# LuckyIYI/gsm-renderer

Measured on AMD Instinct MI355X. Metric: frames/sec @ N Gaussians × W×H (1/2/4/8 GPU); sort Gkeys/s; blend HBM GB/s, higher is better.
Workload: dtype fp16

## Files before the change

### gsm-renderer_amd/csrc/gsm_capi.hip

```cpp
#include <hip/hip_runtime.h>

#include <cstring>

#include "../../include/gsm_debug.h"
#include "../../include/gsm_multigpu.h"
#include "../../include/gsm_renderer.h"
#include "gsm_internal.h"
#include "gsm_frame_sort_check.h"
#include "gsm_renderer_impl.h"

namespace gsm {

class FrameSorter {
   public:
    static gsm_status create(uint32_t capacity, uint32_t maxTiles, int device, FrameSorter** out) {
        FrameSorter* f = new (std::nothrow) FrameSorter;
        if (!f) return GSM_ERR_FAILED_TO_ALLOCATE_BUFFER;
        gsm_status st = pick_device(device, &f->dev_);
        if (st == GSM_OK) {
            f->allocs_.setDevice(f->dev_.id);
            f->tuning_ = tuning_from_env(f->dev_.id);
            f->capacity_ = capacity;
            f->maxTiles_ = maxTiles;
            DeviceAllocations& M = f->allocs_;
// ... 358 lines not shown
}

gsm_status gsm_global_transform_from_pose(const float rotation[9], float scale, const float translation[3],
                                          gsm_global_transform_desc* out) {
    return gsm::transform_from_pose(rotation, scale, translation, out);
}

gsm_status gsm_global_transform(gsm_renderer* r, void* stream, const gsm_global_scene* scene,
                                const gsm_global_state* state, const uint32_t keep[8],
                                const gsm_global_transform_desc* desc) {
    if (!r || !r->impl) return GSM_ERR_INVALID_ARGUMENT;
    return r->impl->transform((hipStream_t)stream, scene, state, keep, desc);
}

gsm_status gsm_global_pick_owner(gsm_renderer* r, const uint32_t* items, uint32_t n, uint32_t* object,
                                 uint32_t* gaussian) {
    if (!r || !r->impl || (n > 0 && (!items || !object || !gaussian))) return GSM_ERR_INVALID_ARGUMENT;
    return r->impl->pickOwner(items, n, object, gaussian);
}

gsm_status gsm_global_project_partition(gsm_renderer* r, void* stream, const gsm_gaussian_input* input,
                                        const gsm_camera_params* camera, uint32_t width, uint32_t height,
                                        uint32_t first, uint32_t count, const uint32_t* slab_rows,
                                        uint32_t num_slabs, void* send, uint64_t send_capacity,
                                        uint32_t* send_counts) {
    if (!r || !r->impl || !input || !camera) return GSM_ERR_INVALID_ARGUMENT;
    return r->impl->projectPartition((hipStream_t)stream, *input, *camera, width, height, first, count,
                                     slab_rows, num_slabs, send, send_capacity, send_counts);
}

gsm_status gsm_global_render_records(gsm_renderer* r, void* stream, const void* records, uint32_t count,
                                     uint32_t width, uint32_t height, void* color, size_t color_pitch,
                                     void* depth, size_t depth_pitch) {
    if (!r || !r->impl) return GSM_ERR_INVALID_ARGUMENT;
    return r->impl->renderRecords((hipStream_t)stream, records, count, width, height, color, color_pitch,
                                  depth, depth_pitch);
}

gsm_status gsm_global_render_stereo_sbs(gsm_renderer* r, void* stream, const gsm_gaussian_input* input,
                                        const gsm_camera_params* left, const gsm_camera_params* right,
                                        uint32_t width_per_eye, uint32_t height, void* color, size_t color_pitch,
                                        void* depth, size_t depth_pitch) {
    if (!r || !r->impl || !input || !left || !right) return GSM_ERR_INVALID_ARGUMENT;
    if (!color) return GSM_ERR_MISSING_REQUIRED_BUFFER;
    gsm_status st = r->impl->renderFrame((hipStream_t)stream, *input, *left, width_per_eye, height,
                                         gsm::FrameTargets{color, color_pitch, depth, depth_pitch});
    if (st != GSM_OK) return st;
    char* rc = (char*)color + (size_t)width_per_eye * 8;
    char* rd = depth ? (char*)depth + (size_t)width_per_eye * 2 : nullptr;
    return r->impl->renderFrame((hipStream_t)stream, *input, *right, width_per_eye, height,
                                gsm::FrameTargets{rc, color_pitch, rd, depth_pitch});
}

gsm_status gsm_global_render_stereo(gsm_renderer* r, void*, const gsm_gaussian_input*,
                                    const gsm_camera_params*, const gsm_camera_params*, uint32_t,
                                    uint32_t, void*, size_t, void*, size_t) {
    if (!r) return GSM_ERR_INVALID_ARGUMENT;
    return GSM_ERR_UNSUPPORTED;
}

uint32_t gsm_global_debug_read_total_assignments(gsm_renderer* r) {
    if (!r || !r->impl) return 0;
    gsm_debug_counters c;
    if (r->impl->counters(&c) != GSM_OK) return 0;
    return c.total_assignments;
}

gsm_status gsm_global_last_gpu_time(gsm_renderer* r, double* seconds) {
    if (!r || !r->impl || !seconds) return GSM_ERR_INVALID_ARGUMENT;
    return r->impl->lastGpuTime(seconds);
}

gsm_status gsm_global_debug_counters(gsm_renderer* r, gsm_debug_counters* out) {
    if (!r || !r->impl || !out) return GSM_ERR_INVALID_ARGUMENT;
    return r->impl->counters(out);
}

gsm_status gsm_global_debug_blend_kernel(gsm_renderer* r, int* kind) {
    if (!r || !r->impl || !kind) return GSM_ERR_INVALID_ARGUMENT;
    *kind = r->impl->lastBlendKernel();
    return GSM_OK;
}

gsm_status gsm_global_debug_copy(gsm_renderer* r, int which, void* dst, size_t bytes, size_t* needed) {
    if (!r || !r->impl) return GSM_ERR_INVALID_ARGUMENT;
    return r->impl->debugCopy(which, dst, bytes, needed);
}

gsm_status gsm_global_set_profiling(gsm_renderer* r, int enable) {
    if (!r || !r->impl) return GSM_ERR_INVALID_ARGUMENT;
    return r->impl->setProfiling(enable);
}

gsm_status gsm_global_stage_times(gsm_renderer* r, float* ms, int n) {
    if (!r || !r->impl || !ms) return GSM_ERR_INVALID_ARGUMENT;
    return r->impl->stageTimes(ms, n);
}

gsm_status gsm_global_set_tile_rows(gsm_renderer* r, uint32_t b, uint32_t e) {
    if (!r || !r->impl) return GSM_ERR_INVALID_ARGUMENT;
    return r->impl->setTileRows(b, e);
}

size_t gsm_debug_sort_workspace_bytes(uint32_t capacity) { return gsm::sort_workspace_bytes(capacity); }

gsm_status gsm_debug_sort_plan_fits(uint32_t capacity, uint32_t key_bits, int wide, size_t hist_bytes) {
    if (key_bits == 0 || key_bits > 32) return GSM_ERR_INVALID_ARGUMENT;
    const gsm::SortSpace ws{(uint32_t*)(uintptr_t)16, hist_bytes, (uint32_t*)(uintptr_t)16, gsm::kSortTotalsWords};
    return gsm::sort_bits_plan_fits(capacity, key_bits, wide != 0, ws) ? GSM_OK : GSM_ERR_INVALID_ASSIGNMENT_CAPACITY;
}

gsm_status gsm_sort_pairs_u32(void* keys, void* values, uint32_t n, uint32_t key_bits, void* stream) {
    if ((!keys || !values) && n > 0) return GSM_ERR_INVALID_ARGUMENT;
    if (n == 0) return GSM_OK;
    if (key_bits == 0 || key_bits > 32) key_bits = 32;
    hipStream_t s = (hipStream_t)stream;
    uint32_t *k2 = nullptr, *v2 = nullptr, *hist = nullptr, *bins = nullptr, *np = nullptr;
    gsm_status st = GSM_OK;
    if (hipMalloc(&k2, (size_t)n * 4) != hipSuccess || hipMalloc(&v2, (size_t)n * 4) != hipSuccess ||
        hipMalloc(&hist, gsm::sort_workspace_bytes(n)) != hipSuccess || hipMalloc(&bins, 256 * 4) != hipSuccess ||
        hipMalloc(&np, 4) != hipSuccess) {
        st = GSM_ERR_FAILED_TO_ALLOCATE_BUFFER;
    }
    if (st == GSM_OK) {
        hipMemcpyAsync(np, &n, 4, hipMemcpyHostToDevice, s);
        hipMemsetAsync(hist, 0, gsm::sort_workspace_bytes(n), s);
        uint32_t* kb[2] = {(uint32_t*)keys, k2};
        uint32_t* vb[2] = {(uint32_t*)values, v2};
        const int digits = (int)((key_bits + 7) / 8);
        int dev = 0;
        hipGetDevice(&dev);
        const gsm::Tuning tn = gsm::tuning_from_env(dev);
        const gsm::SortSpace ws{hist, gsm::sort_workspace_bytes(n), bins, 256};
        int res = gsm::radix_sort_pairs(kb, vb, np, n, 0, digits, ws, s, tn.ballotRank, tn.sortScanless);
        if (res == gsm::kSortNoSpace) st = GSM_ERR_INVALID_ASSIGNMENT_CAPACITY;
        if (res == 1) {
            hipMemcpyAsync(keys, k2, (size_t)n * 4, hipMemcpyDeviceToDevice, s);
            hipMemcpyAsync(values, v2, (size_t)n * 4, hipMemcpyDeviceToDevice, s);
        }
        if (hipStreamSynchronize(s) != hipSuccess) st = GSM_ERR_RENDER_FAILED;
    }
    hipFree(k2);
    hipFree(v2);
    hipFree(hist);
    hipFree(bins);
    hipFree(np);
    return st;
}

gsm_status gsm_debug_frame_sort_create(uint32_t capacity, uint32_t max_tiles, int hip_device,
                                       gsm_debug_frame_sort** out) {
    const gsm_status st = gsm::frame_sort_create_check(capacity, max_tiles, out);
    if (st != GSM_OK) return st;
    return gsm_debug_frame_sort::create(out, capacity, max_tiles, hip_device);
}

void gsm_debug_frame_sort_destroy(gsm_debug_frame_sort* f) { gsm_debug_frame_sort::destroy(f); }

gsm_status gsm_debug_frame_sort_run(gsm_debug_frame_sort* f, void* stream, const gsm_debug_frame_sort_desc* desc,
                                    const void* keys, const void* values, uint32_t n, gsm_debug_frame_sort_out* out) {
    if (!f || !f->impl) return GSM_ERR_INVALID_ARGUMENT;
    return f->impl->run((hipStream_t)stream, desc, keys, values, n, out);
}

gsm_status gsm_debug_sort_rank_probe(int hip_device, int* lane_ordered) {
    if (!lane_ordered) return GSM_ERR_INVALID_ARGUMENT;
// ... 43 lines not shown
```

### gsm-renderer_amd/csrc/gsm_internal.h

```cpp
#pragma once
#include <hip/hip_runtime.h>
#include <cstdint>
#include <tuple>

#include "gsm_blend_plan.h"
#include "gsm_frame_plan.h"
#include "gsm_host.h"
#include "gsm_sort_plan.h"
#include "gsm_types.h"

namespace gsm {

struct ProjectArgs {
    CameraUniforms cam;
    TileBinningParams bin;
    uint32_t rowBegin, rowEnd, rowStride;
    uint32_t count;
    uint32_t maxAssignments;
    uint32_t keepRenderData;
    uint32_t schedUnits;
    uint32_t pairBucket;
    float limX, limY, focalX, focalY, maxEig, adjFar, adjDen;
};

struct ViewArgs {
    CameraUniforms cam;
    float limX, limY, focalX, focalY, maxEig, adjFar, adjDen;
    float pad;
};
static_assert(sizeof(ViewArgs) == 240, "ViewArgs: 15 16-B words");
constexpr uint32_t kViewChunk = 16;
struct ViewChunk {
    ViewArgs v[kViewChunk];
};
struct ViewBatch {
    uint32_t views = 0;
    uint32_t blocksPerView = 0;
    uint32_t tilesPerView = 0;
    const ViewArgs* args = nullptr;
};

struct BatchTarget {
    uint8_t* color;
    uint8_t* depth;
    size_t colorPitch, depthPitch;
    uint32_t tileBase, tilesX, tilesY, width, height;
    uint32_t vec;
    uint32_t pad[2];
};
static_assert(sizeof(BatchTarget) == 64, "BatchTarget: one 64-B line");
struct BatchViewArgs {
    CameraUniforms cam;
    float limX, limY, focalX, focalY, maxEig, adjFar, adjDen;
    uint32_t count;
    TileBinningParams bin;
    uint32_t blockBase;
    uint32_t ortho;
    const void* world;
    const void* harm;
    BatchTarget tg;
};
static_assert(sizeof(BatchViewArgs) == 368 && offsetof(BatchViewArgs, tg) % 16 == 0, "BatchViewArgs: 23 16-B words");
constexpr uint32_t kBatchChunk = 10;
struct BatchChunk {
    BatchViewArgs v[kBatchChunk];
};
struct BatchExtras {
    uint8_t* pick;
    size_t pickPitch;
    const uint8_t* occluder;
    size_t occluderPitch;
    const uint8_t* state;
    uint32_t defaultState;
    uint32_t styled;
    uint32_t align;
    uint32_t itemBase;
    uint32_t pad[2];
};
static_assert(sizeof(BatchExtras) == 64, "BatchExtras: one 64-B line");
constexpr uint32_t kExtrasChunk = 32;
struct ExtrasChunk {
    BatchExtras v[kExtrasChunk];
};
struct BatchFrame {
    uint32_t views = 0;
    uint32_t blocks = 0;
    uint32_t tiles = 0;
    const BatchViewArgs* args = nullptr;
    const uint16_t* blockView = nullptr;
    const uint16_t* tileView = nullptr;
    const BatchExtras* extras = nullptr;
};

struct ComposeObjectArgs {
    CameraUniforms cam;
    float limX, limY, focalX, focalY, maxEig, adjFar, adjDen;
    uint32_t count;
    const void* world;
    const void* harm;
    uint32_t blockBase;
    uint32_t defaultState;
    const uint8_t* state;
};
static_assert(sizeof(ComposeObjectArgs) == 272 && sizeof(ComposeObjectArgs) < sizeof(BatchViewArgs) &&
                  offsetof(ComposeObjectArgs, blockBase) == 256,
// ... 79 lines not shown
    asm volatile("s_waitcnt vmcnt(0)" ::: "memory");
    __syncthreads();
    if (threadIdx.x < 64u) mg_arrive_wave(a);
}
constexpr uint32_t kArriveShards = 16, kArriveLineWords = 32;
constexpr uint32_t kArriveWordsPerBarrier = (1 + kArriveShards) * kArriveLineWords;
__device__ __forceinline__ void mg_arrive_unit(const MgArrive& a, uint32_t unit) {
    asm volatile("s_waitcnt vmcnt(0)" ::: "memory");
    const uint32_t sh = unit % kArriveShards;
    const uint32_t shTotal = (a.total - sh + kArriveShards - 1u) / kArriveShards;
    uint32_t* c = a.done + (1u + sh) * kArriveLineWords;
    uint32_t last = 0;
    if ((threadIdx.x & 63u) == 0)
        last = __hip_atomic_fetch_add(c, 1u, __ATOMIC_RELAXED, __HIP_MEMORY_SCOPE_AGENT) == shTotal - 1u ? 1u : 0u;
    if (__builtin_amdgcn_readfirstlane(last)) {
        if ((threadIdx.x & 63u) == 0) __hip_atomic_store(c, 0u, __ATOMIC_RELAXED, __HIP_MEMORY_SCOPE_AGENT);
        mg_arrive_wave(a, a.total < kArriveShards ? a.total : kArriveShards);
    }
}
__device__ __forceinline__ void mg_arrive_block_unit(const MgArrive& a, uint32_t unit) {
    asm volatile("s_waitcnt vmcnt(0)" ::: "memory");
    __syncthreads();
    if (threadIdx.x < 64u) mg_arrive_unit(a, unit);
}
struct CountPublish {
    uint32_t* row[kMaxSlabs];
    MgArrive arrive;
};
constexpr int kSysCoherent = 17;
__device__ __forceinline__ __amdgpu_buffer_rsrc_t sys_rsrc(const void* base, uint32_t bytes) {
    return __builtin_amdgcn_make_buffer_rsrc(const_cast<void*>(base), 0, (int)bytes, 0x00020000);
}
__device__ __forceinline__ uint32_t ld_sys32(const uint32_t* p) {
    return __hip_atomic_load(p, __ATOMIC_RELAXED, __HIP_MEMORY_SCOPE_SYSTEM);
}
__device__ __forceinline__ uint4 ld_sys128(const void* base, uint32_t bytes, uint32_t i) {
    const auto v = __builtin_amdgcn_raw_buffer_load_b128(sys_rsrc(base, bytes), (int)(i * 16u), 0, kSysCoherent);
    return make_uint4(v[0], v[1], v[2], v[3]);
}
__device__ __forceinline__ void st_sys128(void* base, uint32_t bytes, uint32_t i, uint4 v) {
    typedef uint32_t v4u __attribute__((ext_vector_type(4)));
    const v4u w = {v.x, v.y, v.z, v.w};
    __builtin_amdgcn_raw_buffer_store_b128(w, sys_rsrc(base, bytes), (int)(i * 16u), 0, kSysCoherent);
}
__device__ __forceinline__ void st_sys32_at(void* base, uint32_t bytes, uint32_t off, uint32_t v) {
    __builtin_amdgcn_raw_buffer_store_b32(v, sys_rsrc(base, bytes), (int)off, 0, kSysCoherent);
}
__device__ __forceinline__ void st_sys16_at(void* base, uint32_t bytes, uint32_t off, uint16_t v) {
    __builtin_amdgcn_raw_buffer_store_b16(v, sys_rsrc(base, bytes), (int)off, 0, kSysCoherent);
}
__device__ __forceinline__ void st_sys128_at(void* base, uint32_t bytes, uint32_t off, uint4 v) {
    typedef uint32_t v4u __attribute__((ext_vector_type(4)));
    const v4u w = {v.x, v.y, v.z, v.w};
    __builtin_amdgcn_raw_buffer_store_b128(w, sys_rsrc(base, bytes), (int)off, 0, kSysCoherent);
}

struct SortSpace {
    uint32_t* hist = nullptr;
    size_t histBytes = 0;
    uint32_t* binTotals = nullptr;
    size_t binWords = 0;
};
inline bool sort_plan_fits(const SortPlan& plan, const SortSpace& ws, bool haveBuckets = true) {
    return sort_plan_fits(plan, ws.histBytes, ws.binWords, ws.hist != nullptr, ws.binTotals != nullptr, haveBuckets);
}

struct DeviceArena {
    GaussianRenderData* renderData = nullptr;
    short4* bounds = nullptr;
    BlendRecord* rec = nullptr;
    uint32_t* tileCounts = nullptr;
    uint32_t* tileMasks = nullptr;
    uint32_t* blockSums = nullptr;
    TileAssignmentHeader* header = nullptr;
    uint32_t* keys[2] = {nullptr, nullptr};
    uint32_t* vals[2] = {nullptr, nullptr};
    uint32_t* keysKeep = nullptr;
    uint32_t* valsKeep = nullptr;
    unsigned long long* blendTrace = nullptr;
    uint32_t* costMax = nullptr;
    uint32_t* radixHist = nullptr;
    size_t radixHistBytes = 0;
    uint32_t* radixBinTotals = nullptr;
    uint32_t* tileStart = nullptr;
    uint32_t* tileQueue = nullptr;
    uint16_t* unitCost = nullptr;
    uint32_t* unitOrder = nullptr;
    uint32_t* halfVals[2] = {nullptr, nullptr};
    uint32_t* halfCount = nullptr;
    ViewArgs* viewArgs = nullptr;
    BatchViewArgs* batchArgs = nullptr;
    uint16_t* batchBlockView = nullptr;
    uint16_t* batchTileView = nullptr;
    BatchExtras* batchExtras = nullptr;
    ComposeObjectArgs* composeArgs = nullptr;
    uint16_t* composeBlockObject = nullptr;
    uint2* styleTable = nullptr;
    uint32_t* selectBitmap = nullptr;
    uint32_t* extractBlocks = nullptr;
    uint4* boundsPartials = nullptr;
    uint16_t* expTable = nullptr;
    float2* sincosTable = nullptr;
};

struct Tuning {
    bool fullRadix = false;
    bool ballotRank = false;
    bool costOrder = true;
    int blendWaves = 0;
    int blendClaim = 1;
    bool wideSort = true;
    bool sortScanless = true;
    bool blendPairs = true;
    int pairBucket = 128;
    bool fusedScan = true;
};
constexpr uint32_t kFusedScanMaxBlocks = 8192;
Tuning tuning_from_env(int device);
bool sort_lane_ordered_atomics(int device);

constexpr uint32_t kHalfSkipShift = 30;
constexpr uint32_t kGidMask = (1u << kHalfSkipShift) - 1u;
constexpr float kBlendZeroP = 34.65625f;

constexpr uint32_t kSincosEntries = 65536;
inline SortSpace sort_space(const DeviceArena& A) { return SortSpace{A.radixHist, A.radixHistBytes, A.radixBinTotals, kSortTotalsWords}; }

void launch_project(bool halfInput, uint32_t shDegree, const FramePayload& payload, const void* world,
                    const void* harmonics, const ProjectArgs& args, const StyleArgs* style, bool ortho,
                    const DeviceArena& A, hipStream_t stream);
void launch_fill_views(const ViewChunk& chunk, uint32_t first, uint32_t n, ViewArgs* dst, hipStream_t stream);
void launch_fill_batch(const BatchChunk& chunk, uint32_t first, uint32_t n, BatchViewArgs* dst, uint16_t* blockView,
                       uint32_t maxBlocks, uint16_t* tileView, uint32_t maxTiles, hipStream_t stream);
void launch_fill_batch_extras(const ExtrasChunk& chunk, uint32_t first, uint32_t n, BatchExtras* dst,
                              hipStream_t stream);
void launch_fill_compose(const ComposeChunk& chunk, uint32_t first, uint32_t n, ComposeObjectArgs* dst,
                         uint16_t* blockObject, uint32_t maxBlocks, hipStream_t stream);
void launch_fill_styles(const StyleChunk& chunk, uint2* dst, hipStream_t stream);
void launch_select_mask(bool halfInput, const void* world, const ProjectArgs& args, const uint8_t* mask,
                        size_t maskPitch, uint32_t width, uint32_t height, uint8_t* state, const uint2* styleTable,
                        uint32_t andMask, uint32_t xorMask, uint32_t* matched, const DeviceArena& A,
                        hipStream_t stream, bool ortho = false);
void launch_select_pick(const uint8_t* pick, size_t pickPitch, uint32_t width, uint32_t height, const uint8_t* mask,
                        size_t maskPitch, uint32_t base, uint32_t n, uint32_t* bitmap, uint8_t* state,
                        uint32_t andMask, uint32_t xorMask, uint32_t* matched, hipStream_t stream);
struct KeepSet {
    uint32_t w[8];
};
struct ExtractArgs {
    const uint8_t* records;
    const uint8_t* harmonics;
    const uint8_t* state;
    uint32_t defaultState;
    uint32_t count;
    KeepSet keep;
    uint32_t* blockBase;
    uint8_t* outRecords;
    uint8_t* outHarmonics;
    uint8_t* outState;
    uint32_t* outIds;
    uint32_t capacity;
    uint32_t recordBytes;
    uint64_t harmonicsBytes;
};
void launch_extract(const ExtractArgs& args, uint32_t* kept, hipStream_t stream);
void launch_state_histogram(const uint8_t* state, uint32_t count, uint32_t* histogram, hipStream_t stream);
struct SelectWhereArgs {
    float A[12];
    float opacityMin, opacityMax, scaleMin, scaleMax;
    uint32_t shape, outside, opacityOn, scaleOn;
    uint32_t testMask, testValue;
    uint32_t andMask, xorMask;
    uint32_t count;
};
void launch_select_where(bool halfInput, const void* world, const SelectWhereArgs& args, uint8_t* state,
                         const uint2* styleTable, uint32_t* matched, hipStream_t stream);
constexpr size_t kBoundsPartialBytes = 32;
void launch_state_bounds(bool halfInput, const void* world, const uint8_t* state, uint32_t defaultState,
                         uint32_t count, const KeepSet& keep, uint4* partials, uint32_t* bounds, hipStream_t stream);
void launch_transform(bool halfInput, uint32_t shDegree, void* world, void* harmonics, const uint8_t* state,
                      uint32_t defaultState, uint32_t count, const KeepSet& keep, const gsm_global_transform_desc& desc,
                      bool wideRows, hipStream_t stream);
void launch_partition(bool halfInput, uint32_t shDegree, const void* world, const void* harmonics,
                      const ProjectArgs& args, const SlabTable& slabs, const PartitionBuffers& B,
                      const float2* sincos, void* send, uint64_t capacity, uint32_t* sendCounts,
                      hipStream_t stream);
void launch_partition_counts(bool halfInput, uint32_t shDegree, const void* world, const void* harmonics,
                             const ProjectArgs& args, const SlabTable& slabs, const PartitionBuffers& B,
                             const float2* sincos, uint32_t* sendCounts, const DeviceArena& A,
                             const CountPublish& publish, hipStream_t stream);
void launch_partition_push(const ProjectArgs& args, uint32_t world, uint32_t rank, const PartitionBuffers& B,
                           const uint32_t* counts, const SlabPeers& peers, uint32_t* recvCount, const SlabTable& slabs,
                           const MgArrive& arrive, hipStream_t stream, uint32_t gridCap = 0);
void launch_records_in(const void* records, const ProjectArgs& args, const DeviceArena& A,
                       hipStream_t stream, const uint32_t* devCount = nullptr);
void launch_scan_blocks(uint32_t numBlocks, const ProjectArgs& args, const DeviceArena& A,
                        hipStream_t stream, const uint32_t* devCount = nullptr);
void launch_scan_sums(uint32_t* sums, uint32_t nb, uint32_t cap, TileAssignmentHeader* hdr, uint32_t* queue,
                      hipStream_t stream);
void launch_scatter(const ProjectArgs& args, const DeviceArena& A, hipStream_t stream, const FramePayload& payload,
                    const uint32_t* devCount = nullptr, bool fusedScan = false);
void launch_half_lists(const uint32_t* sortedVals, uint32_t tileBegin, uint32_t numTiles, const DeviceArena& A,
                       uint32_t tileCount, hipStream_t stream);
void launch_headers(const uint32_t* sortedKeys, const FrameGeometry& geo, const DeviceArena& A,
                    hipStream_t stream);
struct BlendOptions {
    bool costOrder = false;
    int colorFormat = 0;
    int waves = 0;
    int claim = 1;
    bool pairs = false;
    const MgArrive* arrive = nullptr;
    const PickTarget* pick = nullptr;
    const OccluderSource* occluder = nullptr;
    const uint32_t* sortedVals = nullptr;
    const BatchExtras* batchExtras = nullptr;
    int numCUs = 0;
};
int launch_blend(const FrameGeometry& geo, const DeviceArena& A, const FrameTargets& targets,
                 const BlendOptions& options, hipStream_t stream);
void launch_blend_pw(const FrameGeometry& geo, const DeviceArena& A, const FrameTargets& targets, const BlendPlan& plan,
                     hipStream_t stream);
int blend_pairs_per_lane(uint32_t numTiles, int numCUs);
uint32_t blend_units_per_tile(uint32_t numTiles, int numCUs);
template <class K, class Mid, class Last>
void launch_blend_walk(K kernel, const BlendPlan& plan, int threads, const DeviceArena& A, uint32_t tileCount,
                       const Mid& mid, const Last& last, hipStream_t stream) {
    const uint32_t* order = (plan.flags & kBlendCostSplit) ? A.unitOrder : nullptr;
    std::apply(
        [&](const auto&... args) { hipLaunchKernelGGL(kernel, dim3(plan.grid), dim3(threads), 0, stream, args...); },
        std::tuple_cat(std::make_tuple(A.tileStart, A.rec, A.expTable, A.tileQueue), mid,
                       std::make_tuple(order, A.unitCost, A.blendTrace, A.halfVals[0], A.halfVals[1], A.halfCount,
                                       tileCount, A.costMax),
                       last));
}

int radix_sort_pairs(uint32_t* keys[2], uint32_t* vals[2], const uint32_t* nPtr, uint32_t capacity,
                     int firstDigit, int numDigits, const SortSpace& ws,
                     hipStream_t stream, bool ballot, bool scanless = true);
int radix_sort_bits(uint32_t* keys[2], uint32_t* vals[2], const uint32_t* nPtr, uint32_t capacity,
                    uint32_t shift, uint32_t bits, const SortSpace& ws, hipStream_t stream,
                    bool ballot, bool wide = false, bool scanless = true);
int radix_sort_tiles(uint32_t* keys[2], uint32_t* vals[2], const uint32_t* nPtr, uint32_t capacity, uint32_t shift,
                     const SortSpace& ws, uint32_t* tileStart, uint32_t tileBase, uint32_t numTiles,
                     uint32_t allTiles, hipStream_t stream, bool ballot, bool wide = true, bool scanless = true);
int radix_sort_tiles_wide(uint32_t* keys[2], uint32_t* vals[2], const uint32_t* nPtr, uint32_t capacity,
                          const SortSpace& ws, uint32_t* tileStart, uint32_t* buckets, uint32_t allTiles,
                          hipStream_t stream, bool ballot);
int run_sort_plan(const SortPlan& plan, uint32_t* keys[2], uint32_t* vals[2], const uint32_t* nPtr, const SortSpace& ws,
                  uint32_t* tileStart, uint32_t* buckets, hipStream_t stream, bool ballot);
inline bool sort_tiles_wide_fits(uint32_t capacity, uint32_t allTiles, const SortSpace& ws) {
    return sort_plan_fits(plan_sort_tiles_wide(capacity, allTiles), ws);
}
inline bool sort_bits_plan_fits(uint32_t capacity, uint32_t bits, bool wide, const SortSpace& ws) {
    return sort_plan_fits(plan_sort_bits(capacity, 0u, bits, wide, false), ws);
}
void tile_depth_sort(uint32_t* keysIn, uint32_t* valsIn, uint32_t* keysOut, uint32_t* valsOut,
                     const uint32_t* tileStart, uint32_t tileBegin, uint32_t numTiles, hipStream_t stream,
                     bool ballot, uint32_t* half0, uint32_t* half1, uint32_t* halfCount, uint32_t tileCount,
                     bool full, int numCUs);

__device__ __forceinline__ uint32_t wave_scan_incl(uint32_t v) {
    v += (uint32_t)__builtin_amdgcn_update_dpp(0, (int)v, 0x111, 0xF, 0xF, true);
    v += (uint32_t)__builtin_amdgcn_update_dpp(0, (int)v, 0x112, 0xF, 0xF, true);
    v += (uint32_t)__builtin_amdgcn_update_dpp(0, (int)v, 0x114, 0xF, 0xF, true);
    v += (uint32_t)__builtin_amdgcn_update_dpp(0, (int)v, 0x118, 0xF, 0xF, true);
    v += (uint32_t)__builtin_amdgcn_update_dpp(0, (int)v, 0x142, 0xA, 0xF, false);
    v += (uint32_t)__builtin_amdgcn_update_dpp(0, (int)v, 0x143, 0xC, 0xF, false);
    return v;
}

struct Tail4 {
    uint32_t n4, last4, t[3];
};
__device__ __forceinline__ Tail4 tail4_load(const uint32_t* __restrict__ p, uint32_t n) {
    Tail4 T;
    T.n4 = n & ~3u;
    T.last4 = T.n4 >= 4u ? T.n4 - 4u : 0u;
#pragma unroll
    for (uint32_t j = 0; j < 3; ++j) T.t[j] = p[min(T.n4 + j, n - 1u)];
    return T;
}
__device__ __forceinline__ uint4 load4_clamped(const uint32_t* __restrict__ p, uint32_t i, const Tail4& T) {
    return *(const uint4*)(p + min(i, T.last4));
}
__device__ __forceinline__ uint4 fix4(uint4 q, uint32_t i, const Tail4& T) {
    return i == T.n4 ? make_uint4(T.t[0], T.t[1], T.t[2], 0u) : q;
}

#define GSM_EXP_TABLE_TO_LDS(NTHREADS, expTable, tbl)                                                        \
    do {                                                                                                     \
        constexpr uint32_t kVec_ = 65536u * 2u / 16u, kPer_ = (kVec_ + (NTHREADS) - 1u) / (NTHREADS);        \
        const uint4* src_ = (const uint4*)(expTable);                                                        \
        uint4 t_[kPer_];                                                                                     \
        _Pragma("unroll") for (uint32_t k_ = 0; k_ < kPer_; ++k_)                                            \
            t_[k_] = src_[min((uint32_t)threadIdx.x + k_ * (uint32_t)(NTHREADS), kVec_ - 1u)];                \
        _Pragma("unroll") for (uint32_t k_ = 0; k_ < kPer_; ++k_) {                                          \
            const uint32_t i_ = (uint32_t)threadIdx.x + k_ * (uint32_t)(NTHREADS);                           \
            if (i_ < kVec_) ((uint4*)(tbl))[i_] = t_[k_];                                                    \
        }                                                                                                    \
    } while (0)

constexpr uint32_t kUoBuckets = 256;
constexpr uint32_t kQueueStripes = 8, kQueueStride = 16;
constexpr uint32_t kCostMaxSlots = 64;
template <int NT>
__device__ __forceinline__ void unit_order_block(const uint16_t* __restrict__ cost, uint32_t* __restrict__ order,
                                                 uint32_t n, uint32_t* base, uint32_t* wmax,
                                                 uint32_t* __restrict__ costMax, uint32_t splitBucket = 0) {
    static_assert(NT >= (int)kUoBuckets && NT % 64 == 0, "one thread per bucket");
    constexpr uint32_t UN = 8;
    const uint32_t t = threadIdx.x, lane = t & 63u, w = t >> 6;
    auto load = [&](uint32_t b0, uint32_t (&c)[UN]) {
#pragma unroll
        for (uint32_t k = 0; k < UN; ++k) c[k] = (uint32_t)cost[min(b0 + k * (uint32_t)NT + t, n - 1u)];
    };
    uint32_t m = t < kCostMaxSlots ? costMax[t] : 0u;
    for (int off = 32; off > 0; off >>= 1) m = max(m, (uint32_t)__shfl_xor((int)m, off));
    if (lane == 0) wmax[w] = m;
    if (t < kUoBuckets) base[t] = 0;
    __syncthreads();
    if (t < kCostMaxSlots) costMax[t] = 0;
    uint32_t mx = 0;
    for (uint32_t k = 0; k < (uint32_t)NT / 64u; ++k) mx = max(mx, wmax[k]);
    const float scale = (float)kUoBuckets / (float)(mx + 1u);
    auto bucket = [&](uint32_t c) { return (kUoBuckets - 1u) - min(kUoBuckets - 1u, (uint32_t)((float)c * scale)); };
    for (uint32_t b0 = 0; b0 < n; b0 += (uint32_t)NT * UN) {
        uint32_t c[UN];
        load(b0, c);
#pragma unroll
        for (uint32_t k = 0; k < UN; ++k)
            if (b0 + k * (uint32_t)NT + t < n) atomicAdd(&base[bucket(c[k])], 1u);
    }
    __syncthreads();
    if (w == 0) {
        const uint4 c = *(const uint4*)(base + lane * 4u);
        const uint32_t local = c.x + c.y + c.z + c.w;
        const uint32_t inc = wave_scan_incl(local);
        const uint32_t e = inc - local;
        const uint4 starts = make_uint4(e, e + c.x, e + c.x + c.y, e + c.x + c.y + c.z);
        *(uint4*)(base + lane * 4u) = starts;
        if (splitBucket) {
            if (splitBucket >= kUoBuckets) {
                if (lane == 0) costMax[kCostMaxSlots] = n;
            } else if (lane == splitBucket / 4u) {
                const uint32_t q = splitBucket & 3u;
                costMax[kCostMaxSlots] = q == 0 ? starts.x : q == 1 ? starts.y : q == 2 ? starts.z : starts.w;
            }
        }
    }
    __syncthreads();

// ... 16 lines not shown
```

### gsm-renderer_amd/csrc/gsm_kernels.hip

```cpp
#include <hip/hip_runtime.h>

#include <cstdlib>
#include <tuple>
#include <type_traits>

#include "gsm_device.h"
#include "gsm_detmath.h"
#include "gsm_internal.h"
#include "gsm_types.h"



namespace gsm {

struct ProjOut {
    uint4 rd;
    BlendRecordA ra;
    uint32_t rb;
    short4 bounds;
    float cmx, cmy, w;
    Conic k;
    bool vis, countable;
};

// ... 872 lines not shown
        hdr->paddedCount = ((tot + 1023u) / 1024u) * 1024u;
        hdr->overflow = ovf;
        for (uint32_t q = 0; q < kQueueStripes; ++q) blendQueue[q * kQueueStride] = 0;
    }
}

__device__ __forceinline__ uint32_t half_skip_flags(float mx, float ex, int tx) {
    if (ex < 0.0f) return 0u;
    const int x0 = tx * (int)kTileWidth;
    constexpr int hw = (int)kTileWidth / 2;
    const int m0 = fp16_coord_margin(x0 + hw - 1), m1 = fp16_coord_margin(x0 + 2 * hw - 1);
    const bool l = (float)(x0 - m0) - mx > ex || (float)(x0 + hw - 1 + m0) - mx < -ex;
    const bool r = (float)(x0 + hw - m1) - mx > ex || (float)(x0 + 2 * hw - 1 + m1) - mx < -ex;
    return (l ? 1u : 0u) | (r ? 2u : 0u);
}

__device__ __forceinline__ uint64_t block_sum_prefix(const uint32_t* __restrict__ sums, uint32_t n,
                                                     unsigned long long* lds64) {
    uint64_t v = 0;
    const uint32_t n4 = n & ~3u;
    constexpr uint32_t kStep = kProjectBlock * 4u;
    auto sum_groups = [&](auto ng) {
        constexpr uint32_t NG = decltype(ng)::value, NR = NG < 4u ? NG : 4u;
        const Tail4 T = tail4_load(sums, n);
#pragma unroll
        for (uint32_t r = 0; r < NG; r += NR) {
            uint4 q[NR];
#pragma unroll
            for (uint32_t k = 0; k < NR; ++k) q[k] = load4_clamped(sums, threadIdx.x * 4u + (r + k) * kStep, T);
#pragma unroll
            for (uint32_t k = 0; k < NR; ++k)
                if (threadIdx.x * 4u + (r + k) * kStep < T.n4) v += (uint64_t)q[k].x + q[k].y + q[k].z + q[k].w;
        }
        if (threadIdx.x == 0)
            v += (uint64_t)(T.n4 < n ? T.t[0] : 0u) + (T.n4 + 1u < n ? T.t[1] : 0u) + (T.n4 + 2u < n ? T.t[2] : 0u);
    };
    if (n == 0u) {
    } else if (n <= kStep) {
        sum_groups(std::integral_constant<uint32_t, 1>{});
    } else if (n <= 2u * kStep) {
        sum_groups(std::integral_constant<uint32_t, 2>{});
    } else if (n <= 4u * kStep) {
        sum_groups(std::integral_constant<uint32_t, 4>{});
    } else if (n <= 8u * kStep) {
        sum_groups(std::integral_constant<uint32_t, 8>{});
    } else {
        uint32_t i = threadIdx.x * 4u;
        for (; i + 3u * kStep < n4; i += 4u * kStep) {
            uint4 q[4];
#pragma unroll
            for (uint32_t k = 0; k < 4; ++k) q[k] = *(const uint4*)(sums + i + k * kStep);
#pragma unroll
            for (uint32_t k = 0; k < 4; ++k) v += (uint64_t)q[k].x + q[k].y + q[k].z + q[k].w;
        }
        for (; i < n4; i += kStep) {
            const uint4 q = *(const uint4*)(sums + i);
            v += (uint64_t)q.x + q.y + q.z + q.w;
        }
        if (threadIdx.x < n - n4) v += sums[n4 + threadIdx.x];
    }
    const uint32_t lo = wave_scan_incl((uint32_t)(v & 0x3FFFFFFull)), hi = wave_scan_incl((uint32_t)(v >> 26));
    v = ((uint64_t)hi << 26) + lo;
    if ((threadIdx.x & 63u) == 63u) lds64[threadIdx.x >> 6] = v;
    __syncthreads();
    uint64_t t = 0;
#pragma unroll
    for (int w = 0; w < kProjectBlock / 64; ++w) t += lds64[w];
    __syncthreads();
    return t;
}

#define GSM_VIEWS 0
#include "gsm_scatter_body.h"
#undef GSM_VIEWS
#define GSM_VIEWS 1
#include "gsm_scatter_body.h"
#undef GSM_VIEWS
#define GSM_VIEWS 2
#include "gsm_scatter_body.h"
#undef GSM_VIEWS
#define GSM_VIEWS 3
#include "gsm_scatter_body.h"
#undef GSM_VIEWS

__global__ __launch_bounds__(256) void k_tile_starts(const uint32_t* __restrict__ sortedKeys,
                                                     const TileAssignmentHeader* __restrict__ hdr,
                                                     uint32_t tileBegin, uint32_t tileEnd,
                                                     uint32_t* __restrict__ tileStart) {
    const uint32_t total = hdr->totalAssignments;
    const uint32_t stride = gridDim.x * 256u * 4u;
    for (uint32_t i0 = (blockIdx.x * 256u + threadIdx.x) * 4u; i0 <= total; i0 += stride) {
        uint32_t k[5];
        k[0] = i0 == 0 ? 0u : sortedKeys[i0 - 1];
        if (i0 + 4u <= total) {
            const uint4 q = *(const uint4*)(sortedKeys + i0);
            k[1] = q.x;
            k[2] = q.y;
            k[3] = q.z;
            k[4] = q.w;
        } else {
#pragma unroll
            for (int j = 0; j < 4; ++j) k[j + 1] = i0 + j < total ? sortedKeys[i0 + j] : 0u;
        }
#pragma unroll
        for (uint32_t j = 0; j < 4; ++j) {
            const uint32_t i = i0 + j;
            if (i > total) break;
            const uint32_t prev = i == 0 ? tileBegin - 1u : (k[j] >> 16);
            const uint32_t cur = i == total ? tileEnd : min(k[j + 1] >> 16, tileEnd);
            for (uint32_t t = prev + 1u; t <= cur; ++t) tileStart[t] = i;
        }
    }
}


constexpr uint32_t kHlThreads = 256;
__global__ __launch_bounds__(kHlThreads) void k_half_lists(const uint32_t* __restrict__ tileStart,
                                                           const uint32_t* __restrict__ sortedVals,
                                                           uint32_t tileBegin, uint32_t tileCount,
                                                           uint32_t* __restrict__ half0, uint32_t* __restrict__ half1,
                                                           uint32_t* __restrict__ halfCount) {
    __shared__ uint32_t part[2][kHlThreads / 64];
    const uint32_t t = tileBegin + blockIdx.x;
    const uint32_t start = tileStart[t], n = tileStart[t + 1] - start;
    const uint32_t lane = threadIdx.x & 63u, wave = threadIdx.x >> 6;
    uint32_t base0 = 0, base1 = 0;
    for (uint32_t b = 0; b < n; b += 4 * kHlThreads) {
        const uint32_t i0 = b + threadIdx.x * 4u;
        uint32_t v[4];
        uint32_t k0 = 0, k1 = 0;
#pragma unroll
        for (uint32_t j = 0; j < 4; ++j) {
            v[j] = i0 + j < n ? sortedVals[start + i0 + j] : (3u << kHalfSkipShift);
            k0 += ((v[j] >> kHalfSkipShift) & 1u) ^ 1u;
            k1 += ((v[j] >> (kHalfSkipShift + 1)) & 1u) ^ 1u;
        }
        const uint32_t packed = k0 | (k1 << 16);
        uint32_t inc = wave_scan_incl(packed);
        if (lane == 63) {
            part[0][wave] = inc & 0xFFFFu;
            part[1][wave] = inc >> 16;
        }
        __syncthreads();
        uint32_t off0 = 0, off1 = 0, tot0 = 0, tot1 = 0;
#pragma unroll
        for (uint32_t w = 0; w < kHlThreads / 64; ++w) {
            if (w < wave) {
                off0 += part[0][w];
                off1 += part[1][w];
            }
            tot0 += part[0][w];
            tot1 += part[1][w];
        }
        uint32_t p0 = base0 + off0 + (inc & 0xFFFFu) - k0, p1 = base1 + off1 + (inc >> 16) - k1;
#pragma unroll
        for (uint32_t j = 0; j < 4; ++j) {
            const uint32_t g = v[j] & kGidMask;
            if (!((v[j] >> kHalfSkipShift) & 1u)) half0[start + p0++] = g;
            if (!((v[j] >> (kHalfSkipShift + 1)) & 1u)) half1[start + p1++] = g;
        }
        base0 += tot0;
        base1 += tot1;
        __syncthreads();
    }
    if (threadIdx.x == 0) {
        halfCount[t] = base0;
// ... 151 lines not shown
                       CountPublish{});
    hipLaunchKernelGGL(k_part_copy<false>, dim3(min(blocks, kCopyMaxBlocks)), dim3(kProjectBlock), 0, s, B.runs,
                       B.runStride, blocks, slabs.n, B.blockSlabCounts, sendCounts, 0u, nullptr, SlabPeers{},
                       nullptr, MgArrive{}, (SplatRecord*)send, capacity);
}

void launch_partition_counts(bool halfInput, uint32_t deg, const void* world, const void* harm, const ProjectArgs& a,
                             const SlabTable& slabs, const PartitionBuffers& B, const float2* sincos,
                             uint32_t* sendCounts, const DeviceArena& A, const CountPublish& pub, hipStream_t s) {
    const uint32_t blocks = (a.count + kProjectBlock - 1) / kProjectBlock;
    if (blocks > 0 || a.schedUnits > 0) launch_project_part(halfInput, deg, world, harm, a, slabs, B, sincos, &A, s);
    CountPublish p = pub;
    if (p.arrive.done) p.arrive.total = slabs.n;
    hipLaunchKernelGGL(k_part_scan, dim3(slabs.n), dim3(1024), 0, s, B.blockSlabCounts, blocks, sendCounts, p);
}

void launch_partition_push(const ProjectArgs& a, uint32_t world, uint32_t rank, const PartitionBuffers& B,
                           const uint32_t* counts, const SlabPeers& peers, uint32_t* recvCount, const SlabTable& slabs,
                           const MgArrive& arrive, hipStream_t s, uint32_t gridCap) {
    (void)slabs;
    const uint32_t blocks = (a.count + kProjectBlock - 1) / kProjectBlock;
    uint32_t grid = blocks ? blocks : 1u;
    if (gridCap && grid > gridCap) grid = gridCap;
    MgArrive ar = arrive;
    ar.total = grid;
    hipLaunchKernelGGL(k_part_copy<true>, dim3(grid), dim3(kProjectBlock), 0, s, B.runs, B.runStride, blocks, world,
                       B.blockSlabCounts, nullptr, rank, counts, peers, recvCount, ar, nullptr, 0ull);
}

constexpr uint32_t kRecordsInMaxBlocks = 2048;
void launch_records_in(const void* records, const ProjectArgs& a, const DeviceArena& A, hipStream_t s,
                       const uint32_t* devCount) {
    uint32_t blocks = (a.count + kProjectBlock - 1) / kProjectBlock;
    if (blocks == 0 && a.schedUnits == 0) return;
    if (devCount && blocks > kRecordsInMaxBlocks) blocks = kRecordsInMaxBlocks;
    hipLaunchKernelGGL(k_records_in, dim3(blocks + (a.schedUnits ? 1u : 0u)), dim3(kProjectBlock), 0, s,
                       (const SplatRecord*)records, a, A.renderData, A.bounds, A.rec, A.tileCounts, A.tileMasks,
                       A.blockSums, A.sincosTable, devCount, A.unitCost, A.unitOrder, A.costMax);
}

void launch_scan_sums(uint32_t* sums, uint32_t nb, uint32_t cap, TileAssignmentHeader* hdr, uint32_t* queue,
                      hipStream_t s) {
    hipLaunchKernelGGL(k_scan_blocks, dim3(1), dim3(kScanThreads), 0, s, sums, nb, cap, hdr, queue,
                       (const uint32_t*)nullptr);
}

void launch_scan_blocks(uint32_t nb, const ProjectArgs& a, const DeviceArena& A, hipStream_t s,
                        const uint32_t* devCount) {
    hipLaunchKernelGGL(k_scan_blocks, dim3(1), dim3(kScanThreads), 0, s, A.blockSums, nb,
                       a.maxAssignments, A.header, A.tileQueue, devCount);
}

void launch_scatter(const ProjectArgs& a, const DeviceArena& A, hipStream_t s, const FramePayload& payload,
                    const uint32_t* devCount, bool fusedScan) {
    if (const ComposeFrame* cf = payload.compose()) {
        if (cf->blocks == 0) return;
        hipLaunchKernelGGL(k_scatter_compose, dim3(cf->blocks), dim3(kProjectBlock), 0, s, a, cf->args,
                           cf->blockObject, A.renderData, A.bounds, A.tileCounts, A.tileMasks, A.blockSums, A.keys[0],
                           A.vals[0], A.sincosTable, A.rec, fusedScan ? 1u : 0u, A.header, A.tileQueue);
        return;
    }
    if (const BatchFrame* bf = payload.batch()) {
        if (bf->blocks == 0) return;
        hipLaunchKernelGGL(k_scatter_batch, dim3(bf->blocks), dim3(kProjectBlock), 0, s, a, bf->args, bf->blockView,
                           A.renderData, A.bounds, A.tileCounts, A.tileMasks, A.blockSums, A.keys[0], A.vals[0],
                           A.sincosTable, A.rec, fusedScan ? 1u : 0u, A.header, A.tileQueue);
        return;
    }
    if (const ViewBatch* vb = payload.views()) {
        const uint32_t vblocks = vb->views * vb->blocksPerView;
        if (vblocks == 0) return;
        hipLaunchKernelGGL(k_scatter_views, dim3(vblocks), dim3(kProjectBlock), 0, s, a, vb->blocksPerView,
                           vb->tilesPerView, A.renderData, A.bounds, A.tileCounts, A.tileMasks, A.blockSums, A.keys[0],
                           A.vals[0], A.sincosTable, A.rec, fusedScan ? 1u : 0u, A.header, A.tileQueue);
        return;
    }
    const uint32_t blocks = (a.count + kProjectBlock - 1) / kProjectBlock;
    if (blocks == 0) return;
    hipLaunchKernelGGL(k_scatter, dim3(blocks), dim3(kProjectBlock), 0, s, a, A.renderData, A.bounds,
                       A.tileCounts, A.tileMasks, A.blockSums, A.keys[0], A.vals[0], A.sincosTable, A.rec, devCount,
                       fusedScan ? 1u : 0u, A.header, A.tileQueue);
}

void launch_headers(const uint32_t* sortedKeys, const FrameGeometry& g, const DeviceArena& A,
                    hipStream_t s) {
    const uint32_t t0 = 0, t1 = frame_tiles(g);
    if (t1 <= t0) return;
    uint32_t blocks = (g.maxAssignments + 1u + 1023u) / 1024u;
    if (blocks > 4096u) blocks = 4096u;
    hipLaunchKernelGGL(k_tile_starts, dim3(blocks), dim3(256), 0, s, sortedKeys, A.header, t0, t1,
                       A.tileStart);
}

}
```

### gsm-renderer_amd/csrc/gsm_project_body.h

```cpp
#ifdef GSM_ORTHO
#define GSM_PK(plain, ortho) ortho
#else
#define GSM_PK(plain, ortho) plain
#endif
#if defined(GSM_STYLED) && GSM_VIEWS == 2
template <bool HALF, int DEG>
__global__ __launch_bounds__(kProjectBlock) void GSM_PK(k_project_batch_styled, k_project_batch_ortho_styled)(
    ProjectArgs P, const BatchViewArgs* __restrict__ views, const uint16_t* __restrict__ blockView,
    const BatchExtras* __restrict__ extras, GaussianRenderData* __restrict__ outRD, short4* __restrict__ outBounds,
    BlendRecord* __restrict__ outRec, uint32_t* __restrict__ counts, uint32_t* __restrict__ masks,
    uint32_t* __restrict__ blockSums, const float2* __restrict__ sincos, const uint16_t* __restrict__ unitCost,
    uint32_t* __restrict__ unitOrder, uint32_t* __restrict__ costMax, const uint2* __restrict__ styleTable) {
    const void* __restrict__ world = nullptr;
    const void* __restrict__ harm = nullptr;
    const uint8_t* __restrict__ stateBytes = nullptr;
    uint32_t defaultState = 0, styledView = 0;
#elif defined(GSM_STYLED) && GSM_VIEWS == 3
template <bool HALF, int DEG>
__global__ __launch_bounds__(kProjectBlock) void GSM_PK(k_project_compose_styled, k_project_compose_ortho_styled)(
    ProjectArgs P, const ComposeObjectArgs* __restrict__ objects, const uint16_t* __restrict__ blockObject,
    GaussianRenderData* __restrict__ outRD, short4* __restrict__ outBounds, BlendRecord* __restrict__ outRec,
    uint32_t* __restrict__ counts, uint32_t* __restrict__ masks, uint32_t* __restrict__ blockSums,
    const float2* __restrict__ sincos, const uint16_t* __restrict__ unitCost, uint32_t* __restrict__ unitOrder,
    uint32_t* __restrict__ costMax, const uint2* __restrict__ styleTable) {
// ... 59 lines not shown
    const uint32_t blk = blockIdx.x - (P.schedUnits ? 1u : 0u);
#if GSM_VIEWS == 3
    uint32_t gblk;
    {
        const ComposeObjectArgs& V = objects[__builtin_amdgcn_readfirstlane((uint32_t)blockObject[blk])];
        gblk = blk - V.blockBase;
        world = V.world;
        harm = V.harm;
#ifdef GSM_STYLED
        stateBytes = V.state;
        defaultState = V.defaultState;
#endif
        P.cam = V.cam;
        P.count = V.count;
        P.limX = V.limX;
        P.limY = V.limY;
        P.focalX = V.focalX;
        P.focalY = V.focalY;
        P.maxEig = V.maxEig;
        P.adjFar = V.adjFar;
        P.adjDen = V.adjDen;
    }
#elif GSM_VIEWS == 2
    uint32_t gblk;
#ifdef GSM_ORTHO
    uint32_t orthoView = 0;
#endif
    {
        const BatchViewArgs& V = views[__builtin_amdgcn_readfirstlane((uint32_t)blockView[blk])];
        gblk = blk - V.blockBase;
        world = V.world;
        harm = V.harm;
#ifdef GSM_ORTHO
        orthoView = V.ortho;
#endif
#ifdef GSM_STYLED
        {
            const BatchExtras& E = extras[__builtin_amdgcn_readfirstlane((uint32_t)blockView[blk])];
            stateBytes = E.state;
            defaultState = E.defaultState;
            styledView = E.styled;
        }
#endif
        P.cam = V.cam;
        P.bin = V.bin;
        P.rowBegin = 0;
        P.rowEnd = V.bin.tilesY;
        P.rowStride = 1;
        P.count = V.count;
        P.limX = V.limX;
        P.limY = V.limY;
        P.focalX = V.focalX;
        P.focalY = V.focalY;
        P.maxEig = V.maxEig;
        P.adjFar = V.adjFar;
        P.adjDen = V.adjDen;
    }
#elif GSM_VIEWS
    const uint32_t view = blk / blocksPerView, gblk = blk - view * blocksPerView;
    {
        const ViewArgs& V = views[view];
        P.cam = V.cam;
        P.limX = V.limX;
        P.limY = V.limY;
        P.focalX = V.focalX;
        P.focalY = V.focalY;
        P.maxEig = V.maxEig;
        P.adjFar = V.adjFar;
        P.adjDen = V.adjDen;
    }
#else
    const uint32_t gblk = blk;
#endif
    __shared__ float4 sEll[kProjectBlock];
    __shared__ float2 sEll2[kProjectBlock];
    __shared__ uint32_t sOff[kProjectBlock];
    __shared__ uint32_t sRect[kProjectBlock];
    __shared__ int sTy0[kProjectBlock];
    __shared__ uint32_t sMask[kProjectBlock];
    __shared__ uint32_t sMore[kProjectBlock];
    constexpr uint32_t kCandCap = 4096, kCandRect = 64;
    constexpr uint16_t kSearch = 0xFFFFu;
    __shared__ uint16_t sCand[kCandCap];
    uint4 preW[2];
    preload_world<HALF>(world, gblk * kProjectBlock + threadIdx.x, P.count, preW);
#ifdef GSM_STYLED
    uint32_t stateByte = defaultState;
    if (stateBytes && gblk * kProjectBlock + threadIdx.x < P.count)
        stateByte = stateBytes[gblk * kProjectBlock + threadIdx.x];
#if GSM_VIEWS == 2
    const uint2 style = styledView ? styleTable[stateByte & (kStyleEntries - 1u)] : make_uint2(0u, kStyleIdentityY);
#else
    const uint2 style = styleTable[stateByte & (kStyleEntries - 1u)];
#endif
#endif
    fill_byte_lut(lut, sincos);
    const uint32_t tid = threadIdx.x;
    const uint32_t gid = gblk * kProjectBlock + tid;
#if GSM_VIEWS
    const uint32_t oid = blk * kProjectBlock + tid;
#else
#define oid gid
#endif
    ProjOut o;
    o.vis = false;
    o.countable = false;
    o.bounds = make_short4(0, -1, 0, -1);
    uint32_t area = 0;
    int ty0 = 0;
#ifdef GSM_STYLED
#define GSM_PROJ_MODE kProjStyled
#define GSM_PROJ_STYLE style
#else
#define GSM_PROJ_MODE kProjPlain
#define GSM_PROJ_STYLE make_uint2(0u, kStyleIdentityY)
#endif
    if (gid < P.count) {
#if defined(GSM_ORTHO) && GSM_VIEWS == 2
        o = project_gaussian<HALF, DEG, GSM_PROJ_MODE, kOrthoPerView>(world, harm, gid, P, sincos, lut,
                                                                      HALF ? preW : nullptr, GSM_PROJ_STYLE, orthoView);
#elif defined(GSM_ORTHO)
        o = project_gaussian<HALF, DEG, GSM_PROJ_MODE, kOrthoOn>(world, harm, gid, P, sincos, lut, HALF ? preW : nullptr,
                                                                 GSM_PROJ_STYLE);
#elif defined(GSM_STYLED)
        o = project_gaussian<HALF, DEG, kProjStyled>(world, harm, gid, P, sincos, lut, HALF ? preW : nullptr, style);
#else
        o = project_gaussian<HALF, DEG>(world, harm, gid, P, sincos, lut, HALF ? preW : nullptr);
#endif
        outBounds[oid] = o.bounds;
        if (o.vis) {
            const int ry0 = max((int)o.bounds.z, (int)P.rowBegin), ry1 = min((int)o.bounds.w, (int)P.rowEnd - 1);
            if (P.keepRenderData || (ry1 - ry0 + 1) * ((int)o.bounds.y - (int)o.bounds.x + 1) > kMaskTiles)
                *(uint4*)(outRD + oid) = o.rd;
            if (o.countable && ry1 >= ry0) {
                area = (uint32_t)((ry1 - ry0 + 1) * ((int)o.bounds.y - (int)o.bounds.x + 1));
                ty0 = ry0;
            }
        }
    }
    sEll[tid] = make_float4(o.cmx, o.cmy, o.k.A, o.k.B);
    sEll2[tid] = make_float2(o.k.C, o.w);
    sRect[tid] = ((uint32_t)(int)o.bounds.x & 0xFFFFu) | ((uint32_t)((int)o.bounds.y - (int)o.bounds.x + 1) << 16);
    sTy0[tid] = ty0;
    sMask[tid] = 0;
    sMore[tid] = 0;
    uint32_t total;
    const uint32_t coff = block_exclusive_scan<kProjectBlock>(area, lds, &total);
    sOff[tid] = coff;
    const uint32_t nCand = min(total, kCandCap);
    for (uint32_t i = tid; i < nCand; i += kProjectBlock) sCand[i] = kSearch;
    __syncthreads();
    if (area <= kCandRect)
        for (uint32_t k = 0; k < area && coff + k < kCandCap; ++k) sCand[coff + k] = (uint16_t)((tid << 8) | k);
    __syncthreads();
    for (uint32_t c = tid; c < total; c += kProjectBlock) {
        uint32_t lo, k;
        const uint32_t v = c < kCandCap ? (uint32_t)sCand[c] : (uint32_t)kSearch;
        if (v != kSearch) {
            lo = v >> 8;
            k = v & 0xFFu;
        } else {
            lo = 0;
            uint32_t hi = kProjectBlock - 1;
            while (lo < hi) {
                const uint32_t mid = (lo + hi + 1) >> 1;
                if (sOff[mid] <= c) lo = mid;
                else hi = mid - 1;
            }
            k = c - sOff[lo];
        }
        const uint32_t rect = sRect[lo], rw = rect >> 16;
        uint32_t row = (uint32_t)((float)k * __builtin_amdgcn_rcpf((float)rw));
        if (row * rw > k) row--;
        else if ((row + 1u) * rw <= k) row++;
        const int ty = sTy0[lo] + (int)row, tx = (int)(rect & 0xFFFFu) + (int)(k - row * rw);
        const float4 e = sEll[lo];
        const float2 e2 = sEll2[lo];
        Conic kk;
        kk.A = e.z;
        kk.B = e.w;
        kk.C = e2.x;
        if (intersects_tile(tx, ty, e.x, e.y, kk, e2.y)) {
            if (k < (uint32_t)kMaskTiles) atomicOr(&sMask[lo], 1u << k);
            else atomicAdd(&sMore[lo], 1u);
        }
    }
    __syncthreads();
    uint32_t ntiles = 0;
    if (gid < P.count && o.vis) {
        const uint32_t mask = sMask[tid];
        ntiles = (uint32_t)__builtin_popcount(mask) + sMore[tid];
        masks[oid] = mask;
        const float2 band = ntiles ? band_of(o.ra, o.bounds, rows_of(P)) : make_float2(0.f, -1.f);
        uint4* rp = (uint4*)(outRec + oid);
        rp[0] = make_uint4(o.ra.x, o.ra.y, o.ra.z, o.ra.w);
        rp[1] = make_uint4(o.rb, __float_as_uint(band.x), __float_as_uint(band.y), 0u);
    }
    if (gid < P.count) counts[oid] = ntiles;
    uint32_t s = block_reduce_add<kProjectBlock>(ntiles, lds);
    if (threadIdx.x == 0) blockSums[blk] = s;
}
#if !GSM_VIEWS
#undef oid
#endif
#undef GSM_PROJ_MODE
#undef GSM_PROJ_STYLE
#undef GSM_PK
```

### gsm-renderer_amd/csrc/gsm_renderer.hip

```cpp
#include <hip/hip_runtime.h>

#include <algorithm>
#include <cmath>
#include <cstring>
#include <vector>

#include "../../include/gsm_debug.h"
#include "../../include/gsm_renderer.h"
#include "gsm_detmath.h"
#include "gsm_internal.h"
#include "gsm_renderer_impl.h"

namespace gsm {

gsm_status GlobalRenderer::create(const gsm_renderer_config& cfg, int hipDevice, GlobalRenderer** out) {
    *out = nullptr;
    gsm_status st = check_config(cfg);
    if (st != GSM_OK) return st;
    Device dev;
    if ((st = pick_device(hipDevice, &dev)) != GSM_OK) return st;

    GlobalRenderer* r = new (std::nothrow) GlobalRenderer();
    if (!r) return GSM_ERR_FAILED_TO_ALLOCATE_BUFFER;
    r->dev_ = dev;
    r->allocs_.setDevice(dev.id);
    r->config_ = cfg;
    r->maxGaussians_ = cfg.max_gaussians ? cfg.max_gaussians : 1u;
    r->maxWidth_ = cfg.max_width ? cfg.max_width : 1u;
    r->maxHeight_ = cfg.max_height ? cfg.max_height : 1u;
    r->tilesX_ = tiles_x(r->maxWidth_);
    r->tilesY_ = tiles_y(r->maxHeight_);
    r->tileCount_ = r->tilesX_ * r->tilesY_;
    if (r->tileCount_ > 65536u) {
        delete r;
        return GSM_ERR_INVALID_TILE_COUNT;
    }
    r->rowBegin_ = 0;
    r->rowEnd_ = r->tilesY_;
    const uint64_t cap64 = 4ull * r->maxGaussians_;
    r->maxAssignments_ = (uint32_t)(cap64 > 0xFFFFFFF0ull ? 0xFFFFFFF0ull : cap64);
    r->tuning_ = tuning_from_env(dev.id);

    const size_t G = r->maxGaussians_;
    const size_t cap = r->maxAssignments_;
    const size_t nb = blocks_of(r->maxGaussians_);
    DeviceArena& A = r->arena_;
    DeviceAllocations& M = r->allocs_;
    M.alloc(st, A.renderData, G * sizeof(GaussianRenderData));
    M.alloc(st, A.bounds, G * sizeof(short4));
    M.alloc(st, A.rec, G * sizeof(BlendRecord));
    M.alloc(st, A.tileCounts, G * sizeof(uint32_t));
    M.alloc(st, A.tileMasks, G * sizeof(uint32_t));
    M.alloc(st, A.blockSums, (nb + 1) * sizeof(uint32_t));
    M.alloc(st, A.header, sizeof(TileAssignmentHeader));
    M.alloc(st, A.keys[0], cap * sizeof(uint32_t));
    M.alloc(st, A.keys[1], cap * sizeof(uint32_t));
    M.alloc(st, A.vals[0], cap * sizeof(uint32_t));
    M.alloc(st, A.vals[1], cap * sizeof(uint32_t));
    A.radixHistBytes = sort_workspace_bytes(r->maxAssignments_);
    M.alloc(st, A.radixHist, A.radixHistBytes);
    if (st == GSM_OK && hipMemset(A.radixHist, 0, A.radixHistBytes) != hipSuccess) st = GSM_ERR_FAILED_TO_ALLOCATE_BUFFER;
    M.alloc(st, A.radixBinTotals, kSortTotalsWords * sizeof(uint32_t));
    M.alloc(st, A.tileStart, ((size_t)r->tileCount_ + 1) * sizeof(uint32_t));
    M.alloc(st, A.tileQueue, kQueueStripes * kQueueStride * sizeof(uint32_t));
    M.alloc(st, A.unitCost, (size_t)r->tileCount_ * 4 * sizeof(uint16_t));
    M.alloc(st, A.unitOrder, (size_t)r->tileCount_ * 4 * sizeof(uint32_t));
    M.alloc(st, A.costMax, (kCostMaxSlots + 2) * sizeof(uint32_t));
    M.alloc(st, A.halfVals[0], cap * sizeof(uint32_t));
    M.alloc(st, A.halfVals[1], cap * sizeof(uint32_t));
    M.alloc(st, A.halfCount, (size_t)r->tileCount_ * 2 * sizeof(uint32_t));
    M.alloc(st, A.expTable, 65536 * sizeof(uint16_t));
    M.alloc(st, A.sincosTable, (kSincosEntries + 256) * sizeof(float2));
    if (st != GSM_OK) {
        delete r;
        return st;
    }
    r->sched_[0] = {A.unitCost, A.unitOrder, A.costMax};
    if (upload_table(A.expTable, [](uint32_t i) { return blend_exp_table_entry((uint16_t)i); }) != GSM_OK ||
        upload_table(A.sincosTable, [](uint32_t i) {
            float2 v;
            if (i < kSincosEntries) {
                det_sincos_table_entry(i, &v.x, &v.y);
            } else {
                uint32_t d;
                det_byte_lut_entry(i - kSincosEntries, &v.x, &d);
                std::memcpy(&v.y, &d, 4);
            }
            return v;
        }, kSincosEntries + 256) != GSM_OK ||
        hipMemset(A.header, 0, sizeof(TileAssignmentHeader)) != hipSuccess ||
        hipMemset(A.tileStart, 0, ((size_t)r->tileCount_ + 1) * sizeof(uint32_t)) != hipSuccess ||
        hipMemset(A.unitCost, 0, (size_t)r->tileCount_ * 4 * sizeof(uint16_t)) != hipSuccess ||
        hipMemset(A.costMax, 0, (kCostMaxSlots + 2) * sizeof(uint32_t)) != hipSuccess ||
        hipMemset(A.vals[0], 0, cap * sizeof(uint32_t)) != hipSuccess ||
        hipMemset(A.vals[1], 0, cap * sizeof(uint32_t)) != hipSuccess ||
        hipMemset(A.halfVals[0], 0, cap * sizeof(uint32_t)) != hipSuccess ||
        hipMemset(A.halfVals[1], 0, cap * sizeof(uint32_t)) != hipSuccess) {
        delete r;
        return GSM_ERR_FAILED_TO_ALLOCATE_BUFFER;
    }
    *out = r;
    return GSM_OK;
}

int GlobalRenderer::sortPassCount() const {
    int tileBytes = 1;
    uint32_t remaining = tileCount_ > 0 ? tileCount_ - 1 : 0;
    while (remaining >= 256) {
        tileBytes++;
        remaining >>= 8;
    }
    int p = 2 + tileBytes;
    return p > 4 ? 4 : p;
}

ProjectArgs GlobalRenderer::frameArgs(const gsm_camera_params& camp, uint32_t width, uint32_t height,
                                      uint32_t count, uint32_t shComponents, bool orthographic) const {
    ProjectArgs a;
    std::memset(&a, 0, sizeof(a));
    std::memcpy(a.cam.view, camp.view, sizeof(a.cam.view));
    std::memcpy(a.cam.proj, camp.proj, sizeof(a.cam.proj));
    std::memcpy(a.cam.cameraCenter, camp.position, sizeof(a.cam.cameraCenter));
    a.cam.pixelFactor = 1.0f;
    a.cam.focalX = camp.focal_x;
    a.cam.focalY = camp.focal_y;
    a.cam.width = (float)width;
    a.cam.height = (float)height;
    a.cam.nearPlane = camp.near_plane;
    a.cam.farPlane = camp.far_plane;
    a.cam.shComponents = shComponents;
    a.cam.gaussianCount = count;
    a.cam.inputIsSRGB = config_.gaussian_color_space == GSM_COLOR_SPACE_SRGB ? 1.0f : 0.0f;
    a.bin.gaussianCount = count;
    a.bin.tilesX = tilesX_;
    a.bin.tilesY = tilesY_;
    a.bin.tileWidth = kTileWidth;
    a.bin.tileHeight = kTileHeight;
    a.bin.surfaceWidth = maxWidth_;
    a.bin.surfaceHeight = maxHeight_;
    a.bin.maxCapacity = count;
    a.bin.alphaThreshold = 0.005f;
    a.bin.totalInkThreshold = 2.0f;
    a.rowBegin = rowBegin_;
    a.rowEnd = rowEnd_;
    a.rowStride = rowStride_;
// ... 718 lines not shown
    if (hipGetLastError() != hipSuccess) return GSM_ERR_RENDER_FAILED;
    return GSM_OK;
}

const ScheduleKey& GlobalRenderer::requestKey(const FrameRequest& rq, uint32_t* tiles) {
    const FramePayload& p = rq.payload;
    key_.reset(p.kind == FrameKind::Records ? FrameKind::Single : p.kind);
    *tiles = rowCount() * tilesX_;
    if (const ViewBatch* vb = p.views()) {
        *tiles = vb->views * tiles_of(rq.width, rq.height);
        key_[ScheduleKey::kViewCount] = vb->views;
    } else if (const BatchFrame* bf = p.batch()) {
        *tiles = bf->tiles;
        key_[ScheduleKey::kViewCount] = bf->views;
        for (uint32_t v = 0; v < bf->views; ++v) {
            key_.push(batchHost_[v].tg.width);
            key_.push(batchHost_[v].tg.height);
            key_.push(batchHost_[v].count);
        }
    } else if (const ComposeFrame* cf = p.compose()) {
        key_[ScheduleKey::kViewCount] = cf->objects;
        for (uint32_t o = 0, e = 0; o < cf->objects; ++o) {
            const bool has = e < cf->entries && composeObject_[e] == o;
            key_.push(has ? composeHost_[e].count : 0u);
            e += has ? 1u : 0u;
        }
    }
    key_[ScheduleKey::kPick] = (rq.pick || rq.anyPick) ? 1u : 0u;
    key_[ScheduleKey::kOccluded] = (rq.occluder || rq.anyOccluder) ? 1u : 0u;
    key_[ScheduleKey::kStyled] = rq.style.table ? 1u : 0u;
    key_[ScheduleKey::kUnitsPerTile] = blend_units_per_tile(*tiles, dev_.numCUs);
    key_[ScheduleKey::kWidth] = rq.width;
    key_[ScheduleKey::kHeight] = rq.height;
    key_[ScheduleKey::kRowBegin] = rowBegin_;
    key_[ScheduleKey::kRowEnd] = rowEnd_;
    key_[ScheduleKey::kRowStride] = rowStride_;
    if (rq.orthographic) key_.markOrthographic();
    return key_;
}

uint32_t GlobalRenderer::scheduleUnits(hipStream_t s, const ScheduleKey& key, uint32_t tiles) {
    const uint32_t units = tiles * key[ScheduleKey::kUnitsPerTile];
    if (schedState_.update(key)) {
        for (const ScheduleSet& t : sched_) {
            if (!t.unitCost) continue;
            hipMemsetAsync(t.unitCost, 0, (size_t)units * sizeof(uint16_t), s);
            hipMemsetAsync(t.costMax, 0, (kCostMaxSlots + 2) * sizeof(uint32_t), s);
        }
    }
    return tuning_.costOrder ? units : 0u;
}

gsm_status GlobalRenderer::runFrame(hipStream_t s, const FrameRequest& rq) {
    (void)hipGetLastError();
    const ProjectArgs& a = rq.args;
    const FrameTargets& tg = rq.targets;
    const int profiling = timer_.flags();
    const bool keep = (profiling & 2) != 0;
    const bool capture = (profiling & (2 | 16)) != 0;
    const ViewBatch* views = rq.payload.views();
    const BatchFrame* batch = rq.payload.batch();
    const ComposeFrame* comp = rq.payload.compose();
    const uint32_t nb = comp ? comp->blocks : batch ? batch->blocks : views ? views->views * views->blocksPerView
                                                                            : blocks_of(a.count);
    ProjectArgs fa = a;
    fa.keepRenderData = capture ? 1u : 0u;
    keptRenderData_ = fa.keepRenderData != 0;
    lastCount_ = a.count;
    lastItems_ = comp ? comp->blocks * (uint32_t)kProjectBlock : a.count;
    lastWidth_ = rq.width;
    lastHeight_ = rq.height;
    lastPick_ = rq.pick != nullptr;
    lastPickComposite_ = rq.pick && comp;
    lastPickObjects_ = !rq.pick ? 0u : comp ? comp->objects : 1u;
    uint32_t units = 0;
    if (!rq.preOrdered) {
        uint32_t tiles = 0;
        const ScheduleKey& key = requestKey(rq, &tiles);
        units = scheduleUnits(s, key, tiles);
    }
    const bool costOrder = rq.preOrdered ? tuning_.costOrder : units > 0;
    fa.schedUnits = units;
    fa.pairBucket = tuning_.blendPairs ? (uint32_t)std::max(1, tuning_.pairBucket) : kUoBuckets;

    timer_.beginFrame();
    timer_.record(0, s);
    if (rq.payload.kind == FrameKind::Records)
        launch_records_in(rq.records, fa, arena_, s, rq.devCount);
    else
        launch_project(config_.precision == GSM_PRECISION_FLOAT16, rq.shDegree, rq.payload, rq.world, rq.harm, fa,
                       rq.style.table ? &rq.style : nullptr, rq.orthographic, arena_, s);
    timer_.record(1, s);
    const bool fusedScan = tuning_.fusedScan && nb > 0 && nb <= (rq.devCount ? 4u : 1u) * kFusedScanMaxBlocks;
    if (!fusedScan) launch_scan_blocks(nb, a, arena_, s, rq.devCount);
    timer_.record(2, s);
    launch_scatter(a, arena_, s, rq.payload, rq.devCount, fusedScan);
    if (keep) {
        hipMemcpyAsync(arena_.keysKeep, arena_.keys[0], (size_t)maxAssignments_ * 4, hipMemcpyDeviceToDevice, s);
        hipMemcpyAsync(arena_.valsKeep, arena_.vals[0], (size_t)maxAssignments_ * 4, hipMemcpyDeviceToDevice, s);
    }
    timer_.record(3, s);
    uint32_t* kb[2] = {arena_.keys[0], arena_.keys[1]};
    uint32_t* vb[2] = {arena_.vals[0], arena_.vals[1]};
    FrameGeometry g;
    g.kind = rq.payload.kind;
    g.tilesX = tilesX_;
    g.tilesY = tilesY_;
    g.tileCount = tileCount_;
    g.rowBegin = rowBegin_;
    g.rowEnd = rowEnd_;
    g.rowStride = rowStride_;
    g.rowCount = rowCount();
    g.width = rq.width;
    g.height = rq.height;
    g.maxAssignments = maxAssignments_;
    if (batch) {
        g.rowBegin = 0;
        g.rowStride = 1;
        g.views = batch->views;
        g.batchTiles = batch->tiles;
        g.batchArgs = batch->args;
        g.batchTileView = batch->tileView;
    } else if (views) {
        g.tilesX = a.bin.tilesX;
        g.tilesY = a.bin.tilesY;
        g.rowBegin = 0;
        g.rowEnd = g.rowCount = g.tilesY;
        g.rowStride = 1;
        g.views = views->views;
        g.tilesPerView = views->tilesPerView;
        g.colorViewStride = rq.payload.colorViewStride;
        g.depthViewStride = rq.payload.depthViewStride;
    }
    const bool fullRadix = tuning_.fullRadix;
    const bool unionWalk = batch && batch->extras && (rq.anyPick || rq.anyOccluder);
    const bool keepRuns = rq.occluder || unionWalk;
    const uint32_t* blendRun = nullptr;
    const bool ballot = tuning_.ballotRank;
    if (!fullRadix) {
        const uint32_t localTiles = frame_tiles(g);
        const int res = radix_sort_tiles(kb, vb, &arena_.header->totalAssignments, maxAssignments_, 16,
                                         sort_space(arena_), arena_.tileStart, 0u, localTiles,
                                         tileCount_, s, ballot, tuning_.wideSort, tuning_.sortScanless);
        if (res == kSortNoSpace) return GSM_ERR_INVALID_ASSIGNMENT_CAPACITY;
        tile_depth_sort(kb[res], vb[res], kb[res ^ 1], vb[res ^ 1], arena_.tileStart, 0u, localTiles, s, ballot,
                        arena_.halfVals[0], arena_.halfVals[1],
                        arena_.halfCount, tileCount_, capture || keepRuns, dev_.numCUs);
        sortedKeys_ = capture ? kb[res ^ 1] : nullptr;
        sortedVals_ = capture ? vb[res ^ 1] : nullptr;
        blendRun = keepRuns ? vb[res ^ 1] : nullptr;
    } else {
        const int res = radix_sort_pairs(kb, vb, &arena_.header->totalAssignments, maxAssignments_, 0,
                                         sortPassCount(), sort_space(arena_), s, ballot,
                                         tuning_.sortScanless);
        if (res == kSortNoSpace) return GSM_ERR_INVALID_ASSIGNMENT_CAPACITY;
        sortedKeys_ = kb[res];
        sortedVals_ = vb[res];
        blendRun = vb[res];
    }
    unsortedKeys_ = keep ? arena_.keysKeep : nullptr;
    unsortedVals_ = keep ? arena_.valsKeep : nullptr;
    timer_.record(4, s);
    if (fullRadix) launch_headers(sortedKeys_, g, arena_, s);
    if (fullRadix)
        launch_half_lists(sortedVals_, 0u, frame_tiles(g), arena_, tileCount_, s);
    arena_.blendTrace = (profiling & 4) ? traceBuf_ : nullptr;
    timer_.record(5, s, true);
    BlendOptions bo;
    bo.costOrder = costOrder;
    bo.colorFormat = (int)config_.color_format;
    bo.waves = tuning_.blendWaves;
    bo.claim = tuning_.blendClaim;
    bo.pairs = tuning_.blendPairs;
    bo.arrive = rq.blendArrive;
    bo.pick = rq.pick;
    bo.occluder = rq.occluder;
    bo.sortedVals = blendRun;
    bo.batchExtras = unionWalk ? batch->extras : nullptr;
    bo.numCUs = dev_.numCUs;
    lastBlendKernel_ = launch_blend(g, arena_, tg, bo, s);
    timer_.record(6, s, true);
    timer_.frameDone();
    if (hipGetLastError() != hipSuccess) return GSM_ERR_RENDER_FAILED;
    return GSM_OK;
}

gsm_status GlobalRenderer::counters(gsm_debug_counters* out) {
    hipSetDevice(dev_.id);
    TileAssignmentHeader h;
    if (hipMemcpy(&h, arena_.header, sizeof(h), hipMemcpyDeviceToHost) != hipSuccess)
        return GSM_ERR_RENDER_FAILED;
    out->total_assignments = h.totalAssignments;
    out->max_capacity = h.maxCapacity;
    out->padded_count = h.paddedCount;
    out->overflow = h.overflow;
    out->tiles_x = tilesX_;
    out->tiles_y = tilesY_;
    out->tile_count = tileCount_;
    out->gaussian_count = lastCount_;
    return GSM_OK;
}

gsm_status GlobalRenderer::debugCopy(int which, void* dst, size_t bytes, size_t* needed) {
    hipSetDevice(dev_.id);
    gsm_debug_counters c;
    gsm_status st = counters(&c);
    if (st != GSM_OK) return st;
    const size_t n = lastItems_, tot = c.total_assignments;
    const void* src = nullptr;
    size_t full = 0;
    switch (which) {
        case GSM_BUF_RENDER_DATA:
            if (!keptRenderData_) return GSM_ERR_MISSING_REQUIRED_BUFFER;
            src = arena_.renderData;
            full = n * 16;
            break;
        case GSM_BUF_BOUNDS: full = n * 16; break;
        case GSM_BUF_TILE_COUNTS: src = arena_.tileCounts; full = n * 4; break;
        case GSM_BUF_KEYS: src = unsortedKeys_; full = tot * 4; break;
        case GSM_BUF_VALUES: src = unsortedVals_; full = tot * 4; break;
        case GSM_BUF_SORTED_KEYS:
            if (!sortedKeys_) return GSM_ERR_MISSING_REQUIRED_BUFFER;
            src = sortedKeys_;
            full = tot * 4;
            break;
        case GSM_BUF_SORTED_VALUES:
            if (!sortedVals_) return GSM_ERR_MISSING_REQUIRED_BUFFER;
            src = sortedVals_;
            full = tot * 4;
            break;
        case GSM_BUF_HEADERS: full = (size_t)tileCount_ * 8; break;
        case GSM_BUF_EXP_TABLE: src = arena_.expTable; full = 65536 * 2; break;
        case GSM_BUF_BLEND_TRACE: src = (timer_.flags() & 4) ? traceBuf_ : nullptr; full = (size_t)tileCount_ * 4 * 4 * 8; break;
        default: return GSM_ERR_INVALID_ARGUMENT;
    }
    if (needed) *needed = full;
    if (!dst || bytes == 0) return GSM_OK;
    size_t cpy = bytes < full ? bytes : full;
    if (which == GSM_BUF_BOUNDS) return copy_bounds_int4(arena_.bounds, n, dst, bytes);
    if (which == GSM_BUF_HEADERS) return copy_headers(arena_.tileStart, tileCount_, dst, bytes);
    if (!src) return full == 0 ? GSM_OK : GSM_ERR_MISSING_REQUIRED_BUFFER;
    if (cpy && hipMemcpy(dst, src, cpy, hipMemcpyDeviceToHost) != hipSuccess) return GSM_ERR_RENDER_FAILED;
    if (which == GSM_BUF_VALUES || which == GSM_BUF_SORTED_VALUES) {
        uint32_t* v = (uint32_t*)dst;
        for (size_t i = 0; i < cpy / 4; ++i) v[i] &= kGidMask;
    }
    return GSM_OK;
}

gsm_status GlobalRenderer::setTileRows(uint32_t b, uint32_t e, uint32_t stride) {
    if (b == 0 && e == 0) {
        rowBegin_ = 0;
        rowEnd_ = tilesY_;
        rowStride_ = 1;
        return GSM_OK;
    }
    if (b >= e || e > tilesY_ || stride == 0) return GSM_ERR_INVALID_ARGUMENT;
    rowBegin_ = b;
    rowEnd_ = e;
    rowStride_ = stride;
    return GSM_OK;
}

gsm_status GlobalRenderer::setProfiling(int flags) {
    hipSetDevice(dev_.id);
    if ((flags & 2) && !arena_.keysKeep) {
        gsm_status st = allocs_.alloc((void**)&arena_.keysKeep, (size_t)maxAssignments_ * 4);
        if (st == GSM_OK) st = allocs_.alloc((void**)&arena_.valsKeep, (size_t)maxAssignments_ * 4);
        if (st != GSM_OK) return st;
    }
    if ((flags & 4) && !traceBuf_) {
        gsm_status st = allocs_.alloc((void**)&traceBuf_, (size_t)tileCount_ * 4 * 4 * 8);
        if (st != GSM_OK) return st;
    }
    return timer_.setProfiling(flags);
}
}
```

### gsm-renderer_amd/csrc/gsm_renderer_impl.h

```cpp
#pragma once
#include <hip/hip_runtime.h>

#include <vector>

#include "../../include/gsm_debug.h"
#include "../../include/gsm_renderer.h"
#include "gsm_extract_check.h"
#include "gsm_host.h"
#include "gsm_internal.h"
#include "gsm_schedule_key.h"
#include "gsm_select_check.h"
#include "gsm_transform_check.h"

namespace gsm {

class GlobalRenderer {
   public:
    static gsm_status create(const gsm_renderer_config& cfg, int hipDevice, GlobalRenderer** out);
    ~GlobalRenderer() { hipSetDevice(dev_.id); }

    gsm_status renderFrame(hipStream_t stream, const gsm_gaussian_input& input, const gsm_camera_params& camera,
                           uint32_t width, uint32_t height, const FrameTargets& targets,
                           const FrameExtras& extras = {});
    gsm_status composeFrame(hipStream_t stream, const gsm_global_object* objects, uint32_t objectCount,
                            uint32_t width, uint32_t height, const FrameTargets& targets,
                            const FrameExtras& extras = {});

    gsm_status renderViews(hipStream_t stream, const gsm_gaussian_input& input, const gsm_camera_params* cameras,
                           uint32_t viewCount, uint32_t width, uint32_t height, void* color, size_t colorPitch,
                           size_t colorStride, void* depth, size_t depthPitch, size_t depthStride);

    gsm_status renderBatch(hipStream_t stream, const gsm_global_view* views, uint32_t viewCount);
    gsm_status renderFrames(hipStream_t stream, const gsm_global_frame* frames, uint32_t frameCount);

    gsm_status selectMask(hipStream_t stream, const gsm_gaussian_input* input, const gsm_camera_params* camera,
                          uint32_t width, uint32_t height, const void* mask, size_t maskPitch, uint8_t* state,
                          const gsm_global_style* styles, uint32_t styleCount, uint32_t andMask, uint32_t xorMask,
                          uint32_t* matched, bool orthographic = false);
    gsm_status selectPick(hipStream_t stream, const void* pick, size_t pickPitch, uint32_t width, uint32_t height,
                          const void* mask, size_t maskPitch, uint32_t object, uint8_t* state, uint32_t gaussianCount,
                          uint32_t andMask, uint32_t xorMask, uint32_t* matched);
    gsm_status selectPickIds(hipStream_t stream, const void* pick, size_t pickPitch, uint32_t width, uint32_t height,
                             const void* mask, size_t maskPitch, uint8_t* state, uint32_t gaussianCount,
                             uint32_t andMask, uint32_t xorMask, uint32_t* matched);
    gsm_status extract(hipStream_t stream, const gsm_gaussian_input* input, const gsm_global_state* state,
                       const uint32_t* keep, const gsm_global_extract_out* out, uint32_t* kept);
    gsm_status stateHistogram(hipStream_t stream, const uint8_t* state, uint32_t gaussianCount, uint32_t* histogram);
    gsm_status selectWhere(hipStream_t stream, const gsm_gaussian_input* input, const gsm_global_select_query* query,
                           uint8_t* state, const gsm_global_style* styles, uint32_t styleCount, uint32_t andMask,
                           uint32_t xorMask, uint32_t* matched);
    gsm_status stateBounds(hipStream_t stream, const gsm_gaussian_input* input, const gsm_global_state* state,
                           const uint32_t* keep, gsm_global_bounds* bounds);
    gsm_status transform(hipStream_t stream, const gsm_global_scene* scene, const gsm_global_state* state,
                         const uint32_t* keep, const gsm_global_transform_desc* desc);
    gsm_status pickOwner(const uint32_t* items, uint32_t n, uint32_t* object, uint32_t* gaussian) const;

    gsm_status projectPartition(hipStream_t stream, const gsm_gaussian_input& input,
                                const gsm_camera_params& camera, uint32_t width, uint32_t height,
                                uint32_t first, uint32_t count, const uint32_t* slabRows, uint32_t numSlabs,
                                void* send, uint64_t capacity, uint32_t* sendCounts, bool interleave = false);
    gsm_status partitionCounts(hipStream_t stream, const gsm_gaussian_input& input, const gsm_camera_params& camera,
                               uint32_t width, uint32_t height, uint32_t first, uint32_t count,
                               const uint32_t* slabRows, uint32_t numSlabs, uint32_t* sendCounts,
                               bool orderUnits = false, bool interleave = false, const CountPublish* publish = nullptr);
    gsm_status partitionPush(hipStream_t stream, uint32_t world, uint32_t rank, const uint32_t* counts,
                             const SlabPeers& peers, uint32_t* recvCount, const MgArrive& arrive);
    gsm_status renderRecords(hipStream_t stream, const void* records, uint32_t count, uint32_t width,
                             uint32_t height, void* color, size_t colorPitch, void* depth, size_t depthPitch,
                             const uint32_t* devCount = nullptr, bool preOrdered = false,
                             const MgArrive* blendArrive = nullptr);
    gsm_status validateFrame(uint32_t count, bool inputMissing, uint32_t width, uint32_t height,
                             const void* color, size_t colorPitch, const void* depth, size_t depthPitch) const;
    gsm_status ensurePartitionBuffers(uint32_t numSlabs);
    void selectSchedule(uint32_t parity);
    uint32_t maxGaussians() const { return maxGaussians_; }
    uint32_t tilesY() const { return tilesY_; }
    uint32_t maxWidth() const { return maxWidth_; }
    uint32_t maxHeight() const { return maxHeight_; }
    uint32_t colorBytesPerPixel() const { return color_bytes_per_pixel(config_.color_format); }
    bool halfPrecision() const { return config_.precision == GSM_PRECISION_FLOAT16; }

    gsm_status counters(gsm_debug_counters* out);
    int lastBlendKernel() const { return lastBlendKernel_; }
    gsm_status debugCopy(int which, void* dst, size_t bytes, size_t* needed);
    gsm_status setProfiling(int flags);
    gsm_status stageTimes(float* ms, int n) {
        hipSetDevice(dev_.id);
        return timer_.stageTimes(ms, n, GSM_STAGE_BLEND);
    }
    gsm_status lastGpuTime(double* seconds) {
        hipSetDevice(dev_.id);
        return timer_.lastGpuTime(seconds);
    }
    gsm_status setTileRows(uint32_t begin, uint32_t end, uint32_t stride = 1);
    uint32_t rowCount() const { return rowEnd_ > rowBegin_ ? (rowEnd_ - rowBegin_ + rowStride_ - 1) / rowStride_ : 0u; }
    int device() const { return dev_.id; }

   private:
    GlobalRenderer() = default;
    gsm_status fillStyleTable(hipStream_t s, const gsm_global_style* styles, uint32_t styleCount);
    ProjectArgs frameArgs(const gsm_camera_params& camera, uint32_t width, uint32_t height, uint32_t count,
                          uint32_t shComponents, bool orthographic = false) const;
    struct FrameRequest {
        ProjectArgs args;
        uint32_t width = 0, height = 0;
        FrameTargets targets;
        FramePayload payload;
        const void* world = nullptr;
        const void* harm = nullptr;
        uint32_t shDegree = 0;
        const void* records = nullptr;
        const PickTarget* pick = nullptr;
        const OccluderSource* occluder = nullptr;
        StyleArgs style;
        bool orthographic = false;
        bool anyPick = false, anyOccluder = false;
        const uint32_t* devCount = nullptr;
        bool preOrdered = false;
        const MgArrive* blendArrive = nullptr;
    };
    FrameRequest request(FrameKind kind, const ProjectArgs& args, uint32_t width, uint32_t height,
                         const FrameTargets& targets) const;
    gsm_status runFrame(hipStream_t s, const FrameRequest& rq);
    const ScheduleKey& requestKey(const FrameRequest& rq, uint32_t* tiles);
    uint32_t scheduleUnits(hipStream_t s, const ScheduleKey& key, uint32_t tiles);
    FrameLimits limits() const {
        FrameLimits L;
        L.colorFormat = config_.color_format;
        L.maxGaussians = maxGaussians_;
        L.maxWidth = maxWidth_;
        L.maxHeight = maxHeight_;
        L.tileCount = tileCount_;
        L.tilesY = tilesY_;
        L.rowsRestricted = tileRowsRestricted();
        L.rowStride = rowStride_;
        return L;
    }
    bool tileRowsRestricted() const { return rowBegin_ != 0 || rowEnd_ != tilesY_ || rowStride_ != 1; }
    ProjectArgs batchSharedArgs(const gsm_camera_params& camera0, uint32_t width0, uint32_t height0, uint32_t count,
                                uint32_t shComponents) const;
    gsm_status enqueueBatch(hipStream_t s, const gsm_global_view* views, uint32_t viewCount,
                            const BatchViewOptions* options);
    gsm_status enqueueSelectPick(hipStream_t s, const void* pick, size_t pickPitch, uint32_t width, uint32_t height,
                                 const void* mask, size_t maskPitch, uint32_t base, uint32_t n, uint8_t* state,
                                 uint32_t andMask, uint32_t xorMask, uint32_t* matched);
    PartitionBuffers part_;
    uint32_t partCount_ = 0;
    SlabTable partSlabs_{};
    struct ScheduleSet {
        uint16_t* unitCost = nullptr;
        uint32_t* unitOrder = nullptr;
        uint32_t* costMax = nullptr;
    } sched_[2];
    struct PartitionFrame {
        ProjectArgs a;
        SlabTable slabs;
        const void* world;
        const void* harm;
        uint32_t deg;
        bool half;
    };
    gsm_status preparePartition(const gsm_gaussian_input& in, const gsm_camera_params& camera, uint32_t width,
                                uint32_t height, uint32_t first, uint32_t count, const uint32_t* slabRows,
                                uint32_t numSlabs, bool needSend, const void* send, const uint32_t* sendCounts,
                                PartitionFrame* f, bool interleave = false);
    int sortPassCount() const;

    Device dev_;
    gsm_renderer_config config_{};
    Tuning tuning_{};
    uint32_t maxGaussians_ = 1, maxWidth_ = 1, maxHeight_ = 1;
    uint32_t tilesX_ = 1, tilesY_ = 1, tileCount_ = 1;
    uint32_t rowBegin_ = 0, rowEnd_ = 1, rowStride_ = 1;
    uint32_t maxAssignments_ = 4;
    DeviceArena arena_;
    DeviceAllocations allocs_;
    StageTimer timer_{GSM_STAGE_COUNT, 128};
    int lastBlendKernel_ = 0;
    bool keptRenderData_ = false;
    uint32_t lastCount_ = 0, lastWidth_ = 0, lastHeight_ = 0;
    uint32_t lastItems_ = 0;
    const uint32_t* sortedKeys_ = nullptr;
    const uint32_t* sortedVals_ = nullptr;
    const uint32_t* unsortedKeys_ = nullptr;
    const uint32_t* unsortedVals_ = nullptr;
    unsigned long long* traceBuf_ = nullptr;
    ScheduleKey key_;
    ScheduleState schedState_;
    std::vector<ViewArgs> viewHost_;
    uint32_t maxViews_ = 0;
    std::vector<BatchViewArgs> batchHost_;
    uint32_t maxBatchViews_ = 0;
    std::vector<BatchExtras> extrasHost_;
    std::vector<gsm_global_view> framesViews_;
    std::vector<BatchViewOptions> framesOptions_;
    std::vector<ComposeObjectArgs> composeHost_;
    std::vector<uint32_t> composeObject_;
    bool lastPick_ = false;
    bool lastPickComposite_ = false;
    uint32_t lastPickObjects_ = 0;
};

}

struct gsm_renderer : gsm::Handle<gsm::GlobalRenderer> {};
```

### gsm-renderer_amd/csrc/gsm_sort.hip

```cpp
#include <hip/hip_runtime.h>

#include <algorithm>
#include <cstdlib>
#include <cstring>
#include <mutex>
#include <type_traits>
#include <unordered_map>

#include "gsm_internal.h"

namespace gsm {

constexpr int kWaves = kRadixBlock / 64;

__device__ __forceinline__ void block_range(uint32_t n, uint32_t grid, uint32_t b, uint32_t* begin,
                                            uint32_t* end) {
    uint32_t per = (n + grid - 1) / grid;
    per = (per + kRadixChunk - 1) / kRadixChunk * kRadixChunk;
    uint64_t bb = (uint64_t)per * b;
    uint64_t ee = bb + per;
    if (bb > n) bb = n;
    if (ee > n) ee = n;
    *begin = (uint32_t)bb;
    *end = (uint32_t)ee;
}

template <int BITS>
__device__ __forceinline__ uint64_t match_digit(uint32_t d, bool valid) {
    uint64_t peers = __ballot(valid);
#pragma unroll
    for (int bit = 0; bit < BITS; ++bit) {
        const bool set = (d >> bit) & 1u;
        const uint64_t m = __ballot(set);
        peers &= set ? m : ~m;
    }
    return peers;
}

template <int BITS, bool BALLOT>
__device__ __forceinline__ uint32_t wave_rank(uint32_t* cnt, uint32_t d, bool valid, uint64_t lt) {
    if constexpr (BALLOT) {
        const uint64_t peers = match_digit<BITS>(d, valid);
        const uint32_t before = cnt[d];
        if (valid && (peers & lt) == 0) cnt[d] = before + (uint32_t)__popcll(peers);
        return before + (uint32_t)__popcll(peers & lt);
    } else {
        uint32_t r = 0;
        if (valid) r = atomicAdd(&cnt[d], 1u);
        return r;
    }
}

static_assert(kRadixBlock == 256 && kRadixBlock / 64 == 4, "the scanless base reduction assumes 4 waves");


template <int BITS>
__global__ __launch_bounds__(kRadixBlock) void k_radix_upsweep(const uint32_t* __restrict__ keys,
                                                               const uint32_t* __restrict__ nPtr,
                                                               uint32_t shift,
                                                               uint32_t* __restrict__ hist,
                                                               uint32_t* __restrict__ super,
                                                               uint32_t* __restrict__ superClear) {
    constexpr uint32_t R = 1u << BITS;
    constexpr uint32_t CP = 4, RS = R + (CP > 1 ? 1u : 0u);
    __shared__ uint32_t cnt[kWaves * CP][RS];
    const uint32_t wave = threadIdx.x >> 6;
    const uint32_t row = wave * CP + (threadIdx.x & (CP - 1u));
    for (int i = threadIdx.x; i < (int)(kWaves * CP * RS); i += kRadixBlock) (&cnt[0][0])[i] = 0;
    if (superClear)
        for (uint32_t i = blockIdx.x * kRadixBlock + threadIdx.x; i < (uint32_t)kSuperSetWords; i += gridDim.x * kRadixBlock)
            superClear[i] = 0u;
    __syncthreads();
    uint32_t begin, end;
    block_range(*nPtr, gridDim.x, blockIdx.x, &begin, &end);
    const Tail4 T = tail4_load(keys, end > 0u ? end : 1u);
    auto load_chunk = [&](uint32_t cbase, uint4 (&q)[kRadixItems / 4]) {
#pragma unroll
        for (int i = 0; i < kRadixItems / 4; ++i) q[i] = load4_clamped(keys, cbase + (uint32_t)(i * kRadixBlock + threadIdx.x) * 4u, T);
#pragma unroll
        for (int i = 0; i < kRadixItems / 4; ++i) q[i] = fix4(q[i], cbase + (uint32_t)(i * kRadixBlock + threadIdx.x) * 4u, T);
    };
    uint4 q[kRadixItems / 4];
    if (begin < end) load_chunk(begin, q);
    for (uint32_t cbase = begin; cbase < end; cbase += kRadixChunk) {
        uint4 nq[kRadixItems / 4];
        const bool more = cbase + kRadixChunk < end;
        if (more) load_chunk(cbase + kRadixChunk, nq);
#pragma unroll
        for (int i = 0; i < kRadixItems / 4; ++i) {
            const uint32_t idx = cbase + (uint32_t)(i * kRadixBlock + threadIdx.x) * 4u;
            const uint32_t kk[4] = {q[i].x, q[i].y, q[i].z, q[i].w};
#pragma unroll
            for (int c = 0; c < 4; ++c)
                if (idx + (uint32_t)c < end) atomicAdd(&cnt[row][(kk[c] >> shift) & (R - 1u)], 1u);
        }
        if (more) {
#pragma unroll
            for (int i = 0; i < kRadixItems / 4; ++i) q[i] = nq[i];
        }
    }
    __syncthreads();
    for (uint32_t d = threadIdx.x; d < R; d += kRadixBlock) {
        uint32_t s = 0;
#pragma unroll
        for (uint32_t w = 0; w < kWaves * CP; ++w) s += cnt[w][d];
        hist[(size_t)d * gridDim.x + blockIdx.x] = s;
        if (super && s) atomicAdd(&super[(blockIdx.x / kSuperGroup) * 256u + d], s);
    }
}

__global__ __launch_bounds__(256) void k_radix_scan(uint32_t* __restrict__ hist, uint32_t grid,
                                                    uint32_t* __restrict__ binTotals) {
    __shared__ uint32_t part[4];
    const uint32_t d = blockIdx.x;
    uint32_t* row = hist + (size_t)d * grid;
    const uint32_t b0 = threadIdx.x * 4u;
    uint32_t v[4];
#pragma unroll
    for (int i = 0; i < 4; ++i) v[i] = b0 + i < grid ? row[b0 + i] : 0u;
    const uint32_t local = v[0] + v[1] + v[2] + v[3];
    const uint32_t lane = threadIdx.x & 63, wave = threadIdx.x >> 6;
    uint32_t inc = wave_scan_incl(local);
    if (lane == 63) part[wave] = inc;
    __syncthreads();
    uint32_t off = 0, tot = 0;
#pragma unroll
    for (int w = 0; w < 4; ++w) {
        if ((uint32_t)w < wave) off += part[w];
        tot += part[w];
    }
    uint32_t run = off + inc - local;
#pragma unroll
    for (int i = 0; i < 4; ++i)
        if (b0 + i < grid) {
// ... 420 lines not shown
        __syncthreads();
        {
            uint32_t c[DPT][kWaves], tot[DPT], run = 0;
#pragma unroll
            for (uint32_t i = 0; i < DPT; ++i) {
                tot[i] = 0;
#pragma unroll
                for (int w = 0; w < kWaves; ++w) {
                    c[i][w] = waveCnt[w][wide_pad(d0 + i)];
                    tot[i] += c[i][w];
                }
                run += tot[i];
            }
            uint32_t all;
            uint32_t ls = wide_block_scan(run, part, &all);
#pragma unroll
            for (uint32_t i = 0; i < DPT; ++i) {
                const uint32_t pd = wide_pad(d0 + i);
                adj[pd] = gbase[i] - ls;
                gbase[i] += tot[i];
#pragma unroll
                for (int w = 0; w < kWaves; ++w) {
                    waveCnt[w][pd] = ls;
                    ls += c[i][w];
                }
            }
        }
        __syncthreads();
#pragma unroll
        for (int j = 0; j < kWideItems; ++j) {
            const uint32_t idx = cbase + wave * (64 * kWideItems) + j * 64 + lane;
            if (idx < end) {
                const uint32_t pos = waveCnt[wave][wide_pad(((k[j] >> shift) - base) & (R - 1u))] + rank[j];
                sKeys[pos] = k[j];
                sVals[pos] = v[j];
            }
        }
        __syncthreads();
        zero_counters();
        const uint32_t cn = min((uint32_t)kWideChunk, end - cbase);
        for (uint32_t p = tid; p < cn; p += kRadixBlock) {
            const uint32_t key = sKeys[p];
            const uint32_t dst = adj[wide_pad(((key >> shift) - base) & (R - 1u))] + p;
            keysOut[dst] = key;
            valsOut[dst] = sVals[p];
        }
        __syncthreads();
    }
}

template <class F>
static void dispatch_flags(bool a, bool b, F&& f) {
    auto second = [&](auto A) { b ? f(A, std::true_type{}) : f(A, std::false_type{}); };
    a ? second(std::true_type{}) : second(std::false_type{});
}

template <class F>
static void dispatch_sort_pass(const SortPass& p, bool ballot, F&& f) {
    dispatch_flags(ballot, sort_writes_starts(p.starts), [&](auto BAL, auto ST) {
        auto bits = [&](auto B) { f(B, BAL, ST, std::false_type{}); };
        switch (p.bits) {
            case 4: bits(std::integral_constant<int, 4>{}); break;
            case 5: bits(std::integral_constant<int, 5>{}); break;
            case 6: bits(std::integral_constant<int, 6>{}); break;
            case 7: bits(std::integral_constant<int, 7>{}); break;
            case 8:
                if constexpr (decltype(ST)::value) {
                    if (p.starts == SortStarts::FromBigBuckets) {
                        f(std::integral_constant<int, 8>{}, BAL, ST, std::true_type{});
                        break;
                    }
                }
                bits(std::integral_constant<int, 8>{});
                break;
            case 9: bits(std::integral_constant<int, 9>{}); break;
            case 10: bits(std::integral_constant<int, 10>{}); break;
            default: bits(std::integral_constant<int, 11>{}); break;
        }
    });
}

int run_sort_plan(const SortPlan& plan, uint32_t* keys[2], uint32_t* vals[2], const uint32_t* nPtr, const SortSpace& ws,
                  uint32_t* tileStart, uint32_t* buckets, hipStream_t s, bool ballot) {
    if (!sort_plan_fits(plan, ws, buckets != nullptr)) return kSortNoSpace;
    uint32_t* const hist = ws.hist + kSuperWords;
    for (uint32_t i = 0, cur = 0; i < plan.count; ++i, cur ^= 1u) {
        const SortPass& p = plan.pass[i];
        uint32_t *kin = keys[cur], *vin = vals[cur], *kout = keys[cur ^ 1u], *vout = vals[cur ^ 1u];
        uint32_t* binTotals = ws.binTotals + p.totalsAt;
        const dim3 grid(p.grid), block(kRadixBlock);
        dispatch_sort_pass(p, ballot, [&](auto BITS, auto BAL, auto ST, auto BIGL) {
            constexpr int kBits = decltype(BITS)::value;
            constexpr bool kBallot = decltype(BAL)::value, kStarts = decltype(ST)::value;
            if constexpr (kBits > 8) {
                uint32_t* starts = p.starts == SortStarts::WideTiles     ? tileStart
                                   : p.starts == SortStarts::WideBuckets ? buckets
                                                                         : nullptr;
                hipLaunchKernelGGL(k_wide_upsweep<kBits>, grid, block, 0, s, kin, nPtr, p.shift, p.base, hist);
                hipLaunchKernelGGL(k_wide_scan<kBits>, dim3((1u << kBits) / kWideScanDigits), dim3(256), 0, s, hist,
                                   p.grid, nPtr, binTotals);
                hipLaunchKernelGGL((k_wide_downsweep<kBits, kBallot, kStarts>), grid, block, 0, s, kin, vin, kout, vout,
                                   nPtr, p.shift, p.base, hist, binTotals, starts, p.numTiles, p.allTiles);
            } else {
                TileStarts ts{};
                if (p.starts == SortStarts::FromBuckets) ts.bucketStart = ws.binTotals + kSortBucketsAt;
                if (p.starts == SortStarts::FromBigBuckets) ts.bucketStart = buckets;
                if (p.starts == SortStarts::BucketsOut) ts.bucketStartOut = ws.binTotals + kSortBucketsAt;
                ts.lowBits = p.lowBits;
                ts.numTiles = p.allTiles;
                ts.tileStart = kStarts ? tileStart : nullptr;
                uint32_t* super = p.superSet >= 0 ? ws.hist + (size_t)p.superSet * kSuperSetWords : nullptr;
                uint32_t* superClear = p.superSet >= 0 ? ws.hist + (size_t)(p.superSet ^ 1) * kSuperSetWords : nullptr;
                hipLaunchKernelGGL(k_radix_upsweep<kBits>, grid, block, 0, s, kin, nPtr, p.shift, hist, super, superClear);
                if (!super) hipLaunchKernelGGL(k_radix_scan, dim3(1u << kBits), dim3(256), 0, s, hist, p.grid, binTotals);
                hipLaunchKernelGGL((k_radix_downsweep<kBits, kBallot, kStarts, decltype(BIGL)::value>), grid, block,
                                   p.ldsBytes, s, kin, vin, kout, vout, nPtr, p.shift, hist, binTotals, ts, super);
            }
        });
    }
    return plan.result;
}

int radix_sort_pairs(uint32_t* keys[2], uint32_t* vals[2], const uint32_t* nPtr, uint32_t capacity,
                     int firstDigit, int numDigits, const SortSpace& ws, hipStream_t s, bool ballot, bool scanless) {
    return run_sort_plan(plan_sort_pairs(capacity, firstDigit, numDigits, scanless), keys, vals, nPtr, ws, nullptr, nullptr,
                         s, ballot);
}

int radix_sort_bits(uint32_t* keys[2], uint32_t* vals[2], const uint32_t* nPtr, uint32_t capacity,
                    uint32_t shift, uint32_t bits, const SortSpace& ws, hipStream_t s,
                    bool ballot, bool wide, bool scanless) {
    return run_sort_plan(plan_sort_bits(capacity, shift, bits, wide, scanless), keys, vals, nPtr, ws, nullptr, nullptr, s,
                         ballot);
}

int radix_sort_tiles(uint32_t* keys[2], uint32_t* vals[2], const uint32_t* nPtr, uint32_t capacity, uint32_t shift,
                     const SortSpace& ws, uint32_t* tileStart, uint32_t tileBase, uint32_t numTiles,
                     uint32_t allTiles, hipStream_t s, bool ballot, bool wide, bool scanless) {
    return run_sort_plan(plan_sort_tiles(capacity, shift, tileBase, numTiles, allTiles, wide, scanless), keys, vals, nPtr,
                         ws, tileStart, nullptr, s, ballot);
}

int radix_sort_tiles_wide(uint32_t* keys[2], uint32_t* vals[2], const uint32_t* nPtr, uint32_t capacity,
                          const SortSpace& ws, uint32_t* tileStart, uint32_t* buckets, uint32_t allTiles,
                          hipStream_t s, bool ballot) {
    return run_sort_plan(plan_sort_tiles_wide(capacity, allTiles), keys, vals, nPtr, ws, tileStart, buckets, s, ballot);
}

}

namespace gsm {

constexpr uint32_t kTsThreads = 256;
constexpr uint32_t kTsItems = 8;
constexpr uint32_t kTsCap = kTsThreads * kTsItems;

__device__ __forceinline__ void wave_sync() {
    __builtin_amdgcn_fence(__ATOMIC_RELEASE, "wavefront");
    __builtin_amdgcn_wave_barrier();
    __builtin_amdgcn_fence(__ATOMIC_ACQUIRE, "wavefront");
}

__device__ __forceinline__ void ts_offsets(uint32_t (*wcnt)[256], uint32_t* part) {
    const uint32_t tid = threadIdx.x, lane = tid & 63u, wave = tid >> 6;
    const uint32_t c0 = wcnt[0][tid], c1 = wcnt[1][tid], c2 = wcnt[2][tid], c3 = wcnt[3][tid];
    const uint32_t tot = c0 + c1 + c2 + c3;
    uint32_t inc = wave_scan_incl(tot);
    if (lane == 63) part[wave] = inc;
    __syncthreads();
// ... 248 lines not shown
                     bool ballot, uint32_t* half0, uint32_t* half1, uint32_t* halfCount, uint32_t tileCount,
                     bool full, int numCUs) {
    if (numTiles == 0) return;
    (void)numCUs;
    dispatch_flags(ballot, full, [&](auto BAL, auto FULL) {
        hipLaunchKernelGGL((k_tile_sort<decltype(BAL)::value, decltype(FULL)::value>), dim3(numTiles), dim3(kTsThreads), 0,
                           s, keysIn, valsIn, keysOut, valsOut, tileStart, tileBegin, half0, half1, halfCount, tileCount);
    });
}

__global__ __launch_bounds__(256) void k_rank_probe(uint32_t* __restrict__ mismatches) {
    __shared__ uint32_t cnt[4][64];
    const uint32_t lane = threadIdx.x & 63u, wave = threadIdx.x >> 6;
    const uint64_t lt = (lane == 0) ? 0ull : (~0ull >> (64 - lane));
    uint32_t bad = 0;
    for (uint32_t round = 0; round < 64; ++round) {
        cnt[wave][lane] = 0;
        wave_sync();
        uint32_t h = (blockIdx.x * 0x9E3779B1u) ^ (round * 0x85EBCA6Bu) ^ (wave * 0xC2B2AE35u) ^ (lane * 0x27D4EB2Fu);
        h ^= h >> 15;
        h *= 0x2C1B3C6Du;
        h ^= h >> 12;
        const uint32_t mask = (round & 3u) == 0 ? 0u : ((round & 3u) == 1 ? 1u : ((round & 3u) == 2 ? 7u : 63u));
        const uint32_t d = h & mask;
        const uint32_t got = atomicAdd(&cnt[wave][d], 1u);
        const uint64_t peers = match_digit<6>(d, true);
        if (got != (uint32_t)__popcll(peers & lt)) bad++;
        wave_sync();
    }
    if (bad) atomicAdd(mismatches, bad);
}

bool sort_lane_ordered_atomics(int device) {
    static std::mutex mu;
    static std::unordered_map<int, bool> cache;
    std::lock_guard<std::mutex> lk(mu);
    auto it = cache.find(device);
    if (it != cache.end()) return it->second;
    bool ok = false;
    uint32_t* d = nullptr;
    int prev = 0;
    hipGetDevice(&prev);
    hipStream_t ps = nullptr;
    if (hipSetDevice(device) == hipSuccess && hipStreamCreateWithFlags(&ps, hipStreamNonBlocking) == hipSuccess &&
        hipMalloc(&d, 4) == hipSuccess) {
        uint32_t h = 1;
        if (hipMemsetAsync(d, 0, 4, ps) == hipSuccess) {
            hipLaunchKernelGGL(k_rank_probe, dim3(64), dim3(256), 0, ps, d);
            if (hipMemcpyAsync(&h, d, 4, hipMemcpyDeviceToHost, ps) == hipSuccess && hipStreamSynchronize(ps) == hipSuccess)
                ok = h == 0;
        }
    }
    if (d) hipFree(d);
    if (ps) hipStreamDestroy(ps);
    (void)hipGetLastError();
    hipSetDevice(prev);
    cache[device] = ok;
    return ok;
}

Tuning tuning_from_env(int device) {
    Tuning t;
    const char* sv = getenv("GSM_SORT");
    t.fullRadix = sv && std::strcmp(sv, "radix4") == 0;
    const char* rv = getenv("GSM_SORT_RANK");
    t.ballotRank = (rv && std::strcmp(rv, "ballot") == 0) || !sort_lane_ordered_atomics(device);
    const char* bv = getenv("GSM_BLEND_SCHED");
    t.costOrder = !(bv && bv[0] == '0');
    const char* wv = getenv("GSM_BLEND_WAVES");
    const int w = wv ? atoi(wv) : 0;
    t.blendWaves = (w == 8 || w == 12 || w == 16) ? w : 0;
    const char* cv = getenv("GSM_BLEND_CLAIM");
    t.blendClaim = !cv ? 1 : std::strcmp(cv, "early") == 0 ? 0 : std::strcmp(cv, "auto") == 0 ? 2 : 1;
    const char* ws = getenv("GSM_SORT_WIDE");
    t.wideSort = !(ws && ws[0] == '0');
    const char* sc = getenv("GSM_SORT_SCAN");
    t.sortScanless = !(sc && std::strcmp(sc, "kernel") == 0);
    const char* bp = getenv("GSM_BLEND_PAIRS");
    t.blendPairs = !(bp && bp[0] == '0');
    const char* ps = getenv("GSM_BLEND_PAIR_SPLIT");
    if (ps) t.pairBucket = std::min(256, std::max(0, atoi(ps)));
    const char* fs = getenv("GSM_SCAN_FUSED");
    t.fusedScan = !(fs && fs[0] == '0');
    return t;
}

}
```

### gsm-renderer_amd/csrc/gsm_sort_plan.h

```cpp
#pragma once
#include <cstddef>
#include <cstdint>

#include "../../include/gsm_debug.h"

namespace gsm {

constexpr int kRadixBlock = 256;
constexpr int kRadixItems = 16;
constexpr int kRadixChunk = kRadixBlock * kRadixItems;
constexpr uint32_t kWideMaxBits = 11, kWideBins = 1u << kWideMaxBits;
constexpr int kWideItems = 16;
constexpr int kWideChunk = kRadixBlock * kWideItems;
static_assert(kWideItems % 4 == 0 && kWideItems <= kRadixItems, "wide chunks: 16-B loads, <= the narrow chunk");
constexpr uint32_t kWideRowPad = 64;
constexpr uint32_t kSuperGroup = 32;
constexpr uint32_t kSuperRows = 1024 / kSuperGroup;
constexpr size_t kSuperSetWords = (size_t)kSuperRows * 256;
constexpr size_t kSuperWords = 2 * kSuperSetWords;
constexpr size_t kSortTotalsWords = kWideBins;
constexpr uint32_t kSortFirstTotalsAt = 256, kSortBucketsAt = 512, kSortTwoNarrowWords = 768;
constexpr uint32_t kTilesWideMaxBits = kWideMaxBits + 8u;
constexpr int kSortNoSpace = -1;

inline uint32_t radix_grid_for_capacity(uint32_t capacity) {
    uint32_t g = (capacity + kRadixChunk - 1) / kRadixChunk;
    return g > 1024 ? 1024 : g < 1 ? 1 : g;
}
inline uint32_t wide_grid_for_capacity(uint32_t capacity) {
    uint32_t g = (capacity + kWideChunk - 1) / kWideChunk;
    return g > 1024 ? 1024 : g < 1 ? 1 : g;
}
inline size_t sort_pass_hist_words(bool wide, uint32_t bits, uint32_t grid) {
    const size_t rows = wide ? ((size_t)1 << bits) + kWideRowPad : ((size_t)1 << bits);
    return kSuperWords + rows * grid;
}
inline size_t sort_workspace_bytes(uint32_t capacity) {
    const size_t narrow = sort_pass_hist_words(false, 8, radix_grid_for_capacity(capacity));
    const size_t wide = sort_pass_hist_words(true, kWideMaxBits, wide_grid_for_capacity(capacity));
    return (narrow > wide ? narrow : wide) * sizeof(uint32_t);
}

enum class SortStarts : uint32_t {
    None,
    BucketsOut,
    FromOneBucket,
    FromBuckets,
    WideTiles,
    WideBuckets,
    FromBigBuckets,
};
inline bool sort_writes_starts(SortStarts s) { return s != SortStarts::None && s != SortStarts::BucketsOut; }
inline bool sort_uses_buckets(SortStarts s) { return s == SortStarts::WideBuckets || s == SortStarts::FromBigBuckets; }

struct SortPass {
    bool wide = false;
    uint32_t bits = 0, shift = 0;
    uint32_t base = 0;
    uint32_t grid = 0;
    int superSet = -1;
    uint32_t ldsBytes = 0;
    uint32_t totalsAt = 0;
    SortStarts starts = SortStarts::None;
    uint32_t lowBits = 0;
    uint32_t numTiles = 0, allTiles = 0;
    size_t histWords = 0, binWords = 0;
};

struct SortPlan {
    SortPass pass[4];
    uint32_t count = 0;
    int result = 0;
    uint32_t kind = 0;
    bool valid = true;
    void add(const SortPass& p) {
        if (count == 4) {
            valid = false;
            return;
        }
        pass[count++] = p;
        result = (int)(count & 1u);
    }
};

inline SortPass sort_narrow_pass(uint32_t capacity, uint32_t shift, uint32_t bits, int superSet, SortStarts starts,
                                 size_t binWords) {
    SortPass p;
    p.bits = bits, p.shift = shift, p.grid = radix_grid_for_capacity(capacity), p.superSet = superSet, p.starts = starts;
    p.ldsBytes = sort_writes_starts(starts) ? 0u : 1024u;
    p.histWords = sort_pass_hist_words(false, bits, p.grid), p.binWords = binWords;
    return p;
}
inline SortPass sort_wide_pass(uint32_t capacity, uint32_t shift, uint32_t bits, uint32_t base, SortStarts starts,
                               uint32_t numTiles, uint32_t allTiles) {
    SortPass p;
    p.wide = true, p.bits = bits, p.shift = shift, p.base = base, p.grid = wide_grid_for_capacity(capacity);
    p.starts = starts, p.numTiles = numTiles, p.allTiles = allTiles;
    p.histWords = sort_pass_hist_words(true, bits, p.grid), p.binWords = (size_t)1 << bits;
    return p;
}

inline uint32_t sort_bits_for(uint32_t tiles, uint32_t from, uint32_t to) {
    uint32_t b = from;
    while (b < to && ((tiles - 1u) >> b)) b++;
    return b;
}
inline uint32_t sort_digit_width(uint32_t bitsLeft, uint32_t passesLeft, uint32_t least) {
    const uint32_t b = (bitsLeft + passesLeft - 1) / passesLeft;
    return b < least ? least : b;
}

inline SortPlan plan_sort_bits(uint32_t capacity, uint32_t shift, uint32_t bits, bool wide, bool scanless) {
    const uint32_t narrowPasses = (bits + 7) / 8, widePasses = (bits + kWideMaxBits - 1) / kWideMaxBits;
    const bool useWide = wide && widePasses < narrowPasses;
    const uint32_t passes = useWide ? widePasses : narrowPasses;
    const bool sets = !useWide && scanless && passes % 2 == 0;
    SortPlan plan;
    for (uint32_t p = 0, done = 0; p < passes; ++p) {
        const uint32_t b = sort_digit_width(bits - done, passes - p, useWide ? 9u : 4u);
        if (useWide) plan.add(sort_wide_pass(capacity, shift + done, b, 0u, SortStarts::None, 0u, 0u));
        else
            plan.add(sort_narrow_pass(capacity, shift + done, b, sets ? (int)(p & 1u) : -1, SortStarts::None,
                                      (size_t)1 << b));
        done += b;
    }
    return plan;
}

inline SortPlan plan_sort_pairs(uint32_t capacity, int firstDigit, int numDigits, bool scanless) {
    return plan_sort_bits(capacity, (uint32_t)firstDigit * 8u, (uint32_t)numDigits * 8u, false, scanless);
}

inline SortPlan plan_sort_tiles(uint32_t capacity, uint32_t shift, uint32_t tileBase, uint32_t numTiles,
                                uint32_t allTiles, bool wide, bool scanless) {
    const uint32_t bits = sort_bits_for(allTiles, 1, 16), localBits = sort_bits_for(numTiles, 1, 16);
    SortPlan plan;
    if (wide && bits > 8 && localBits <= kWideMaxBits) {
        plan.kind = GSM_FRAME_SORT_ONE_WIDE;
        plan.add(sort_wide_pass(capacity, shift, sort_digit_width(localBits, 1, 9), tileBase, SortStarts::WideTiles,
                                numTiles, allTiles));
    } else if (bits <= 8) {
        plan.kind = GSM_FRAME_SORT_ONE_NARROW;
        plan.add(sort_narrow_pass(capacity, shift, sort_digit_width(bits, 1, 4), -1, SortStarts::FromOneBucket, 256));
    } else {
        plan.kind = GSM_FRAME_SORT_TWO_NARROW;
        const uint32_t lo = sort_digit_width(bits, 2, 4), hi = sort_digit_width(bits - lo, 1, 4);
        plan.add(sort_narrow_pass(capacity, shift, lo, scanless ? 0 : -1, SortStarts::BucketsOut, kSortTwoNarrowWords));
        plan.pass[0].totalsAt = kSortFirstTotalsAt;
        plan.add(sort_narrow_pass(capacity, shift + lo, hi, scanless ? 1 : -1, SortStarts::FromBuckets,
                                  kSortTwoNarrowWords));
        plan.pass[1].lowBits = lo;
    }
    plan.pass[plan.count - 1].allTiles = allTiles;
    return plan;
}

inline SortPlan plan_sort_tiles_wide(uint32_t capacity, uint32_t allTiles) {
    const uint32_t bits = sort_bits_for(allTiles, 17, 32);
    SortPlan plan;
    plan.kind = GSM_FRAME_SORT_WIDE_THEN_NARROW;
    if (bits > kTilesWideMaxBits) {
        plan.valid = false;
        return plan;
    }
    const uint32_t lo = bits - 8u;
    plan.add(sort_wide_pass(capacity, 0u, lo, 0u, SortStarts::WideBuckets, 1u << lo, 1u << lo));
    plan.add(sort_narrow_pass(capacity, lo, 8, -1, SortStarts::FromBigBuckets, 256));
    plan.pass[1].lowBits = lo, plan.pass[1].allTiles = allTiles;
    return plan;
}

inline bool sort_plan_fits(const SortPlan& plan, size_t histBytes, size_t binWords, bool haveHist, bool haveBins,
                           bool haveBuckets = true) {
    if (!plan.valid) return false;
    for (uint32_t i = 0; i < plan.count; ++i) {
        const SortPass& p = plan.pass[i];
        if (!haveHist || !haveBins || (sort_uses_buckets(p.starts) && !haveBuckets)) return false;
        if (p.histWords * sizeof(uint32_t) > histBytes || p.binWords > binWords) return false;
        if (!p.wide && p.grid > kSuperRows * kSuperGroup) return false;
    }
    return true;
}

}
```

### gsm-renderer_amd/gsm_amd/__init__.py

```python
from __future__ import annotations

import ctypes as C
import enum
import os
from dataclasses import dataclass, field
from typing import Optional

import numpy as np

try:
    import torch
except Exception:
    torch = None

from .types import PROJECTED, RENDER_DATA, WORLD16, WORLD32

_PKG_DIR = os.path.dirname(os.path.abspath(__file__))
LIB_PATH = os.environ.get("GSM_AMD_LIB") or os.path.join(os.path.dirname(_PKG_DIR), "lib", "libgsm_amd.so")
INCLUDE_DIR = os.path.join(os.path.dirname(os.path.dirname(_PKG_DIR)), "include")


class Status(enum.IntEnum):
    OK = 0
    DEVICE_NOT_AVAILABLE = 1
    FAILED_TO_CREATE_LIBRARY = 2
    FAILED_TO_CREATE_PIPELINE = 3
    FAILED_TO_ALLOCATE_BUFFER = 4
    FAILED_TO_ALLOCATE_TEXTURE = 5
    INVALID_GAUSSIAN_COUNT = 6
    INVALID_DIMENSIONS = 7
    INVALID_BUFFER_SIZE = 8
    INVALID_TILE_COUNT = 9
    INVALID_ASSIGNMENT_CAPACITY = 10
    RENDER_FAILED = 11
    ENCODER_CREATION_FAILED = 12
    MISSING_REQUIRED_BUFFER = 13
    INVALID_ARGUMENT = 14
    UNSUPPORTED = 15
    PHASE_ORDER = 16


class RendererError(RuntimeError):
    def __init__(self, status: int, what: str = ""):
        self.status = Status(status)
        msg = _lib().gsm_status_string(int(status)).decode() if _LIB is not None else self.status.name
        super().__init__(f"{self.status.name}: {msg}{(' (' + what + ')') if what else ''}")


class RenderPrecision(enum.IntEnum):
    FLOAT32 = 0
    FLOAT16 = 1


class GaussianColorSpace(enum.IntEnum):
    LINEAR = 0
    SRGB = 1


class ColorFormat(enum.IntEnum):
    RGBA16F = 0
    RGBA32F = 1
    RGBA8_UNORM = 2
    RGBA8_UNORM_SRGB = 3
    BGRA8_UNORM = 4
    BGRA8_UNORM_SRGB = 5

    @property
    def bytes_per_pixel(self) -> int:
        return 8 if self == ColorFormat.RGBA16F else (16 if self == ColorFormat.RGBA32F else 4)


class BufferId(enum.IntEnum):
    RENDER_DATA = 0
    BOUNDS = 1
    TILE_COUNTS = 2
    KEYS = 3
    VALUES = 4
    SORTED_KEYS = 5
    SORTED_VALUES = 6
    HEADERS = 7
    EXP_TABLE = 8
    BLEND_TRACE = 9


STAGES = ("project", "scan", "scatter", "sort", "headers", "blend")
BLEND_KERNELS = {0: None, 1: "k_blend_px", 2: "k_blend_px", 3: "k_blend_pw"}


@dataclass
class RendererConfig:
    max_gaussians: int = 6_000_000
    max_width: int = 1920
    max_height: int = 1080
    precision: RenderPrecision = RenderPrecision.FLOAT16
    color_format: int = 0
    gaussian_color_space: GaussianColorSpace = GaussianColorSpace.SRGB
    back_to_front: bool = False


@dataclass
class GaussianInput:
    gaussians: "torch.Tensor"
    harmonics: "torch.Tensor"
    gaussian_count: int
    shComponents: int = 0

    @property
    def sh_components(self) -> int:
        return self.shComponents


@dataclass
class CameraParams:
    view: np.ndarray
    proj: np.ndarray
    position: np.ndarray = field(default_factory=lambda: np.zeros(3, np.float32))
    focal_x: float = 0.0
    focal_y: float = 0.0
    near: float = 0.1
    far: float = 10.0

    @staticmethod
    def from_dict(d: dict) -> "CameraParams":
        return CameraParams(np.asarray(d["view"], np.float32).reshape(16),
                            np.asarray(d["proj"], np.float32).reshape(16),
                            np.asarray(d.get("position", np.zeros(3)), np.float32).reshape(3),
                            float(d.get("focal_x", 0.0)), float(d.get("focal_y", 0.0)),
                            float(d.get("near", 0.1)), float(d.get("far", 10.0)))

    def to_dict(self) -> dict:
        return {"view": np.asarray(self.view, np.float32), "proj": np.asarray(self.proj, np.float32),
                "position": np.asarray(self.position, np.float32), "focal_x": self.focal_x,
                "focal_y": self.focal_y, "near": self.near, "far": self.far}


@dataclass
class BatchView:
    input: GaussianInput
    camera: CameraParams
    width: int
    height: int
    color: "torch.Tensor"
    depth: Optional["torch.Tensor"] = None
    color_pitch: Optional[int] = None
    depth_pitch: Optional[int] = None


@dataclass
class SceneObject:
    input: GaussianInput
    camera: CameraParams


@dataclass
class Frame:
    objects: object
    width: int
    height: int
    color: "torch.Tensor"
    depth: Optional["torch.Tensor"] = None
    pick: Optional["torch.Tensor"] = None
    occluder: Optional["torch.Tensor"] = None
    states: object = None
    styles: object = None
    color_pitch: Optional[int] = None
# ... 150 lines not shown
                ("tiles_y", C.c_uint32), ("tile_count", C.c_uint32), ("active_tiles", C.c_uint32),
                ("total_entries", C.c_uint32), ("max_tile_count", C.c_uint32), ("max_per_tile", C.c_uint32),
                ("overflow", C.c_uint32)]


PICK_NONE = 0xFFFFFFFF
FRAME_ORTHOGRAPHIC = 2

_LIB = None

_SIGNATURES = {
    "gsm_abi_version": ([], C.c_int),
    "gsm_status_string": ([C.c_int], C.c_char_p),
    "gsm_renderer_config_default": ([C.POINTER(_Config)], None),
    "gsm_camera_params_init": ([C.POINTER(_Camera), C.c_void_p, C.c_void_p, C.c_void_p, C.c_float,
                                C.c_float], None),
    "gsm_global_create": ([C.POINTER(_Config), C.c_int, C.POINTER(C.c_void_p)], C.c_int),
    "gsm_global_destroy": ([C.c_void_p], None),
    "gsm_global_render": ([C.c_void_p, C.c_void_p, C.POINTER(_Input), C.POINTER(_Camera), C.c_uint32,
                           C.c_uint32, C.c_void_p, C.c_size_t, C.c_void_p, C.c_size_t], C.c_int),
    "gsm_global_render_views": ([C.c_void_p, C.c_void_p, C.POINTER(_Input), C.POINTER(_Camera), C.c_uint32,
                                 C.c_uint32, C.c_uint32, C.c_void_p, C.c_size_t, C.c_size_t, C.c_void_p,
                                 C.c_size_t, C.c_size_t], C.c_int),
    "gsm_global_render_batch": ([C.c_void_p, C.c_void_p, C.POINTER(_GlobalView), C.c_uint32], C.c_int),
    "gsm_global_render_composite": ([C.c_void_p, C.c_void_p, C.POINTER(_GlobalObject), C.c_uint32, C.c_uint32,
                                     C.c_uint32, C.c_void_p, C.c_size_t, C.c_void_p, C.c_size_t], C.c_int),
    "gsm_global_render_pick": ([C.c_void_p, C.c_void_p, C.POINTER(_Input), C.POINTER(_Camera), C.c_uint32,
                                C.c_uint32, C.c_void_p, C.c_size_t, C.c_void_p, C.c_size_t, C.c_void_p,
                                C.c_size_t], C.c_int),
    "gsm_global_render_composite_pick": ([C.c_void_p, C.c_void_p, C.POINTER(_GlobalObject), C.c_uint32, C.c_uint32,
                                          C.c_uint32, C.c_void_p, C.c_size_t, C.c_void_p, C.c_size_t, C.c_void_p,
                                          C.c_size_t], C.c_int),
    "gsm_global_render_occluded": ([C.c_void_p, C.c_void_p, C.POINTER(_Input), C.POINTER(_Camera), C.c_uint32,
                                    C.c_uint32, C.c_void_p, C.c_size_t, C.c_void_p, C.c_size_t, C.c_void_p,
                                    C.c_size_t], C.c_int),
    "gsm_global_render_composite_occluded": ([C.c_void_p, C.c_void_p, C.POINTER(_GlobalObject), C.c_uint32,
                                              C.c_uint32, C.c_uint32, C.c_void_p, C.c_size_t, C.c_void_p,
                                              C.c_size_t, C.c_void_p, C.c_size_t], C.c_int),
    "gsm_global_pick_owner": ([C.c_void_p, C.c_void_p, C.c_uint32, C.c_void_p, C.c_void_p], C.c_int),
    "gsm_global_render_styled": ([C.c_void_p, C.c_void_p, C.POINTER(_Input), C.POINTER(_Camera), C.c_uint32,
                                  C.c_uint32, C.c_void_p, C.c_size_t, C.c_void_p, C.c_size_t, C.c_void_p, C.c_size_t,
                                  C.POINTER(_State), C.POINTER(_Style), C.c_uint32], C.c_int),
    "gsm_global_render_composite_styled": ([C.c_void_p, C.c_void_p, C.POINTER(_GlobalObject), C.c_uint32, C.c_uint32,
                                            C.c_uint32, C.c_void_p, C.c_size_t, C.c_void_p, C.c_size_t, C.c_void_p,
                                            C.c_size_t, C.POINTER(_State), C.POINTER(_Style), C.c_uint32], C.c_int),
    "gsm_global_select_mask": ([C.c_void_p, C.c_void_p, C.POINTER(_Input), C.POINTER(_Camera), C.c_uint32,
                                C.c_uint32, C.c_void_p, C.c_size_t, C.c_void_p, C.POINTER(_Style), C.c_uint32,
                                C.c_uint32, C.c_uint32, C.c_void_p], C.c_int),
    "gsm_global_select_mask_ortho": ([C.c_void_p, C.c_void_p, C.POINTER(_Input), C.POINTER(_Camera), C.c_uint32,
                                      C.c_uint32, C.c_void_p, C.c_size_t, C.c_void_p, C.POINTER(_Style), C.c_uint32,
                                      C.c_uint32, C.c_uint32, C.c_void_p], C.c_int),
    "gsm_global_render_frame": ([C.c_void_p, C.c_void_p, C.POINTER(_GlobalFrame)], C.c_int),
    "gsm_global_select_pick": ([C.c_void_p, C.c_void_p, C.c_void_p, C.c_size_t, C.c_uint32, C.c_uint32, C.c_void_p,
                                C.c_size_t, C.c_uint32, C.c_void_p, C.c_uint32, C.c_uint32, C.c_uint32, C.c_void_p],
                               C.c_int),
    "gsm_global_render_frames": ([C.c_void_p, C.c_void_p, C.POINTER(_GlobalFrame), C.c_uint32], C.c_int),
    "gsm_global_select_pick_ids": ([C.c_void_p, C.c_void_p, C.c_void_p, C.c_size_t, C.c_uint32, C.c_uint32,
                                    C.c_void_p, C.c_size_t, C.c_void_p, C.c_uint32, C.c_uint32, C.c_uint32,
                                    C.c_void_p], C.c_int),
    "gsm_global_keep_visible": ([C.POINTER(_Style), C.c_uint32, C.POINTER(C.c_uint32)], None),
    "gsm_global_keep_masked": ([C.c_uint32, C.c_uint32, C.POINTER(C.c_uint32)], None),
    "gsm_global_extract": ([C.c_void_p, C.c_void_p, C.POINTER(_Input), C.POINTER(_State), C.POINTER(C.c_uint32),
                            C.POINTER(_ExtractOut), C.c_void_p], C.c_int),
    "gsm_global_state_histogram": ([C.c_void_p, C.c_void_p, C.c_void_p, C.c_uint32, C.c_void_p], C.c_int),
    "gsm_global_select_query_default": ([C.POINTER(_SelectQuery)], None),
    "gsm_global_select_where": ([C.c_void_p, C.c_void_p, C.POINTER(_Input), C.POINTER(_SelectQuery), C.c_void_p,
                                 C.POINTER(_Style), C.c_uint32, C.c_uint32, C.c_uint32, C.c_void_p], C.c_int),
    "gsm_global_state_bounds": ([C.c_void_p, C.c_void_p, C.POINTER(_Input), C.POINTER(_State),
                                 C.POINTER(C.c_uint32), C.c_void_p], C.c_int),
    "gsm_global_transform_from_pose": ([C.POINTER(C.c_float), C.c_float, C.POINTER(C.c_float),
                                        C.POINTER(_TransformDesc)], C.c_int),
    "gsm_global_transform": ([C.c_void_p, C.c_void_p, C.POINTER(_Scene), C.POINTER(_State), C.POINTER(C.c_uint32),
                              C.POINTER(_TransformDesc)], C.c_int),
    "gsm_global_render_stereo": ([C.c_void_p, C.c_void_p, C.POINTER(_Input), C.POINTER(_Camera),
                                  C.POINTER(_Camera), C.c_uint32, C.c_uint32, C.c_void_p, C.c_size_t,
                                  C.c_void_p, C.c_size_t], C.c_int),
    "gsm_global_render_stereo_sbs": ([C.c_void_p, C.c_void_p, C.POINTER(_Input), C.POINTER(_Camera),
                                      C.POINTER(_Camera), C.c_uint32, C.c_uint32, C.c_void_p, C.c_size_t,
                                      C.c_void_p, C.c_size_t], C.c_int),
    "gsm_global_debug_read_total_assignments": ([C.c_void_p], C.c_uint32),
    "gsm_global_last_gpu_time": ([C.c_void_p, C.POINTER(C.c_double)], C.c_int),
    "gsm_global_debug_counters": ([C.c_void_p, C.POINTER(_Counters)], C.c_int),
    "gsm_global_debug_blend_kernel": ([C.c_void_p, C.POINTER(C.c_int)], C.c_int),
    "gsm_debug_sort_workspace_bytes": ([C.c_uint32], C.c_size_t),
    "gsm_debug_sort_plan_fits": ([C.c_uint32, C.c_uint32, C.c_int, C.c_size_t], C.c_int),
    "gsm_global_debug_copy": ([C.c_void_p, C.c_int, C.c_void_p, C.c_size_t, C.POINTER(C.c_size_t)],
                              C.c_int),
    "gsm_global_set_profiling": ([C.c_void_p, C.c_int], C.c_int),
    "gsm_global_stage_times": ([C.c_void_p, C.POINTER(C.c_float), C.c_int], C.c_int),
    "gsm_global_set_tile_rows": ([C.c_void_p, C.c_uint32, C.c_uint32], C.c_int),
    "gsm_sort_pairs_u32": ([C.c_void_p, C.c_void_p, C.c_uint32, C.c_uint32, C.c_void_p], C.c_int),
    "gsm_debug_frame_sort_create": ([C.c_uint32, C.c_uint32, C.c_int, C.POINTER(C.c_void_p)], C.c_int),
    "gsm_debug_frame_sort_destroy": ([C.c_void_p], None),
    "gsm_debug_frame_sort_run": ([C.c_void_p, C.c_void_p, C.POINTER(_FrameSortDesc), C.c_void_p, C.c_void_p,
                                  C.c_uint32, C.POINTER(_FrameSortOut)], C.c_int),
    "gsm_global_project_partition": ([C.c_void_p, C.c_void_p, C.POINTER(_Input), C.POINTER(_Camera),
                                      C.c_uint32, C.c_uint32, C.c_uint32, C.c_uint32,
                                      C.POINTER(C.c_uint32), C.c_uint32, C.c_void_p, C.c_uint64,
                                      C.c_void_p], C.c_int),
    "gsm_global_render_records": ([C.c_void_p, C.c_void_p, C.c_void_p, C.c_uint32, C.c_uint32, C.c_uint32,
                                   C.c_void_p, C.c_size_t, C.c_void_p, C.c_size_t], C.c_int),
    "gsm_depthfirst_create": ([C.POINTER(_Config), C.c_int, C.POINTER(C.c_void_p)], C.c_int),
    "gsm_depthfirst_default_options": ([C.POINTER(_DfOptions)], None),
    "gsm_depthfirst_create_with_options": ([C.POINTER(_Config), C.c_int, C.POINTER(_DfOptions),
                                            C.POINTER(C.c_void_p)], C.c_int),
    "gsm_depthfirst_get_options": ([C.c_void_p, C.POINTER(_DfOptions)], C.c_int),
    "gsm_depthfirst_destroy": ([C.c_void_p], None),
    "gsm_depthfirst_render_stereo_sbs": ([C.c_void_p, C.c_void_p, C.POINTER(_Input), C.POINTER(_Camera),
                                          C.POINTER(_Camera), C.c_void_p, C.c_uint32, C.c_uint32, C.c_void_p,
                                          C.c_size_t], C.c_int),
    "gsm_depthfirst_render": ([C.c_void_p, C.c_void_p, C.POINTER(_Input), C.POINTER(_Camera), C.c_uint32,
                               C.c_uint32, C.c_void_p, C.c_size_t, C.c_void_p, C.c_size_t], C.c_int),
    "gsm_depthfirst_debug_counters": ([C.c_void_p, C.POINTER(_DfCounters)], C.c_int),
    "gsm_depthfirst_debug_copy": ([C.c_void_p, C.c_int, C.c_void_p, C.c_size_t, C.POINTER(C.c_size_t)],
                                  C.c_int),
    "gsm_depthfirst_set_profiling": ([C.c_void_p, C.c_int], C.c_int),
    "gsm_depthfirst_stage_times": ([C.c_void_p, C.POINTER(C.c_float), C.c_int], C.c_int),
    "gsm_depthfirst_last_gpu_time": ([C.c_void_p, C.POINTER(C.c_double)], C.c_int),
    "gsm_debug_sort_rank_probe": ([C.c_int, C.POINTER(C.c_int)], C.c_int),
    "gsm_debug_partition_counts": ([C.c_void_p, C.c_void_p, C.POINTER(_Input), C.POINTER(_Camera), C.c_uint32,
                                    C.c_uint32, C.c_uint32, C.c_uint32, C.POINTER(C.c_uint32), C.c_uint32,
                                    C.c_void_p], C.c_int),
    "gsm_debug_partition_push": ([C.c_void_p, C.c_void_p, C.c_uint32, C.c_uint32, C.c_void_p,
                                  C.POINTER(C.c_void_p), C.c_void_p], C.c_int),
    "gsm_debug_render_records_device_count": ([C.c_void_p, C.c_void_p, C.c_void_p, C.c_uint32, C.c_void_p,
                                               C.c_uint32, C.c_uint32, C.c_void_p, C.c_size_t, C.c_void_p,
                                               C.c_size_t], C.c_int),
    "gsm_multigpu_create": ([C.c_void_p, C.c_void_p, C.c_int, C.c_int, C.POINTER(C.c_void_p)], C.c_int),
    "gsm_multigpu_default_options": ([C.c_void_p], None),
    "gsm_multigpu_prepare_with_options": ([C.c_void_p, C.c_int, C.c_int, C.c_void_p, C.POINTER(C.c_void_p),
                                           C.c_void_p], C.c_int),
    "gsm_multigpu_create_with_options": ([C.c_void_p, C.c_void_p, C.c_int, C.c_int, C.c_void_p,
                                          C.POINTER(C.c_void_p)], C.c_int),
    "gsm_multigpu_destroy": ([C.c_void_p], None),
    "gsm_multigpu_render": ([C.c_void_p, C.c_void_p, C.POINTER(_Input), C.POINTER(_Camera), C.c_uint32,
                             C.c_uint32, C.c_void_p, C.c_size_t, C.c_void_p, C.c_size_t, C.c_void_p], C.c_int),
    "gsm_multigpu_debug_counts": ([C.c_void_p, C.POINTER(C.c_uint32)], C.c_int),
    "gsm_multigpu_prepare": ([C.c_void_p, C.c_int, C.c_int, C.POINTER(C.c_void_p), C.c_void_p], C.c_int),
    "gsm_multigpu_connect": ([C.c_void_p, C.c_void_p], C.c_int),
    "gsm_multigpu_render_phase": ([C.c_void_p, C.c_int, C.c_void_p, C.POINTER(_Input), C.POINTER(_Camera),
                                   C.c_uint32, C.c_uint32, C.c_void_p, C.c_size_t, C.c_void_p, C.c_size_t,
                                   C.c_void_p], C.c_int),
    "gsm_multigpu_frame": ([C.c_void_p, C.POINTER(C.c_void_p), C.POINTER(C.c_size_t)], C.c_int),
    "gsm_multigpu_status": ([C.c_void_p, C.POINTER(C.c_uint32), C.c_int], C.c_int),
    "gsm_multigpu_set_timeout_ms": ([C.c_void_p, C.c_uint32], C.c_int),
    "gsm_multigpu_debug_copy_exchange": ([C.c_void_p, C.c_void_p, C.c_size_t], C.c_int),
    "gsm_multigpu_debug_copy_frame": ([C.c_void_p, C.c_void_p, C.c_size_t, C.c_uint32, C.c_uint32], C.c_int),
    "gsm_multigpu_debug_copy_depth": ([C.c_void_p, C.c_void_p, C.c_size_t, C.c_uint32, C.c_uint32], C.c_int),
    "gsm_multigpu_frame_depth": ([C.c_void_p, C.POINTER(C.c_void_p), C.POINTER(C.c_size_t)], C.c_int),
    "gsm_multigpu_errors": ([C.c_void_p, C.POINTER(C.c_uint32), C.POINTER(C.c_uint32), C.c_int], C.c_int),
    "gsm_multigpu_finish_frame": ([C.c_void_p, C.c_void_p], C.c_int),
    "gsm_multigpu_wait_event": ([C.c_void_p, C.c_void_p], C.c_int),
    "gsm_multigpu_debug_set_epoch": ([C.c_void_p, C.c_uint32], C.c_int),
}

_LOCAL_SIGNATURES = {
    "gsm_local_create": ([C.POINTER(_Config), C.c_int, C.POINTER(C.c_void_p)], C.c_int),
    "gsm_local_destroy": ([C.c_void_p], None),
    "gsm_local_render": ([C.c_void_p, C.c_void_p, C.POINTER(_Input), C.POINTER(_Camera), C.c_uint32,
                          C.c_uint32, C.c_void_p, C.c_size_t, C.c_void_p, C.c_size_t], C.c_int),
    "gsm_local_debug_counters": ([C.c_void_p, C.POINTER(_LocalCounters)], C.c_int),
    "gsm_local_debug_copy": ([C.c_void_p, C.c_int, C.c_void_p, C.c_size_t, C.POINTER(C.c_size_t)], C.c_int),
    "gsm_local_debug_sort_tiles": ([C.c_void_p, C.c_void_p, C.c_void_p, C.c_void_p, C.c_uint32, C.c_uint32,
                                    C.c_void_p], C.c_int),
    "gsm_local_set_profiling": ([C.c_void_p, C.c_int], C.c_int),
    "gsm_local_stage_times": ([C.c_void_p, C.POINTER(C.c_float), C.c_int], C.c_int),
# ... 451 lines not shown
        rows = (C.c_uint32 * len(slab_rows))(*[int(x) for x in slab_rows])
        st = _lib().gsm_global_project_partition(self._h, _stream_handle(stream), C.byref(inp), C.byref(cam),
                                                 int(width), int(height), int(first), int(count), rows,
                                                 len(slab_rows) - 1, _ptr(send), int(send_capacity),
                                                 _ptr(send_counts))
        _check(st, "gsm_global_project_partition")

    def render_records(self, color_texture, depth_texture, records, count: int, width: int, height: int,
                       stream=None, color_pitch: Optional[int] = None, depth_pitch: Optional[int] = None):
        cp = color_pitch if color_pitch is not None else int(width) * self._bpp
        dp = depth_pitch if depth_pitch is not None else int(width) * 2
        st = _lib().gsm_global_render_records(self._h, _stream_handle(stream), _ptr(records), int(count),
                                              int(width), int(height), _ptr(color_texture), cp,
                                              _ptr(depth_texture), dp)
        _check(st, "gsm_global_render_records")

    def debug_partition_counts(self, input: GaussianInput, camera: CameraParams, width: int, height: int,
                               first: int, count: int, slab_rows, send_counts, stream=None):
        inp = _Input(_ptr(input.gaussians), _ptr(input.harmonics), int(input.gaussian_count),
                     int(input.sh_components))
        cam = _camera_struct(camera)
        rows = (C.c_uint32 * len(slab_rows))(*[int(x) for x in slab_rows])
        _check(_lib().gsm_debug_partition_counts(self._h, _stream_handle(stream), C.byref(inp), C.byref(cam),
                                                 int(width), int(height), int(first), int(count), rows,
                                                 len(slab_rows) - 1, _ptr(send_counts)),
               "gsm_debug_partition_counts")

    def debug_partition_push(self, world: int, rank: int, counts, recv_buffers, recv_count, stream=None):
        bufs = (C.c_void_p * len(recv_buffers))(*[_ptr(b) for b in recv_buffers])
        _check(_lib().gsm_debug_partition_push(self._h, _stream_handle(stream), int(world), int(rank),
                                               _ptr(counts), bufs, _ptr(recv_count)),
               "gsm_debug_partition_push")

    def debug_render_records_device_count(self, color_texture, depth_texture, records, capacity: int, count,
                                          width: int, height: int, stream=None):
        _check(_lib().gsm_debug_render_records_device_count(self._h, _stream_handle(stream), _ptr(records),
                                                            int(capacity), _ptr(count), int(width), int(height),
                                                            _ptr(color_texture), int(width) * self._bpp,
                                                            _ptr(depth_texture), int(width) * 2),
               "gsm_debug_render_records_device_count")

    def render_stereo(self, color_texture, depth_texture, input: GaussianInput, left: CameraParams,
                      right: CameraParams, width: int, height: int, stream=None):
        inp = _Input(_ptr(input.gaussians), _ptr(input.harmonics), int(input.gaussian_count),
                     int(input.sh_components))
        cl, cr = _camera_struct(left), _camera_struct(right)
        st = _lib().gsm_global_render_stereo(self._h, _stream_handle(stream), C.byref(inp), C.byref(cl),
                                             C.byref(cr), int(width), int(height), _ptr(color_texture),
                                             int(width) * 16, _ptr(depth_texture), int(width) * 4)
        _check(st, "gsm_global_render_stereo")

    def render_stereo_sbs(self, color_texture, depth_texture, input: GaussianInput, left: CameraParams,
                          right: CameraParams, width_per_eye: int, height: int, stream=None,
                          color_pitch: Optional[int] = None, depth_pitch: Optional[int] = None):
        inp = _Input(_ptr(input.gaussians), _ptr(input.harmonics), int(input.gaussian_count),
                     int(input.sh_components))
        cl, cr = _camera_struct(left), _camera_struct(right)
        cp = color_pitch if color_pitch is not None else 2 * int(width_per_eye) * self._bpp
        dp = depth_pitch if depth_pitch is not None else 2 * int(width_per_eye) * 2
        st = _lib().gsm_global_render_stereo_sbs(self._h, _stream_handle(stream), C.byref(inp), C.byref(cl),
                                                 C.byref(cr), int(width_per_eye), int(height),
                                                 _ptr(color_texture), cp, _ptr(depth_texture), dp)
        _check(st, "gsm_global_render_stereo_sbs")

    def debug_read_total_assignments(self) -> int:
        return int(_lib().gsm_global_debug_read_total_assignments(self._h))

    def set_profiling(self, stage_events: bool = True, keep_unsorted: bool = False,
                      blend_trace: bool = False, blend_events: bool = False, blend_event_period: int = 1,
                      capture: bool = False):
        flags = (1 if stage_events else 0) | (2 if keep_unsorted else 0) | (4 if blend_trace else 0) | \
            (8 if blend_events else 0) | (16 if capture else 0) | \
            ((max(1, min(255, int(blend_event_period))) & 0xFF) << 8)
        _check(_lib().gsm_global_set_profiling(self._h, flags), "gsm_global_set_profiling")

    def set_tile_rows(self, begin: int, end: int):
        _check(_lib().gsm_global_set_tile_rows(self._h, int(begin), int(end)), "gsm_global_set_tile_rows")

    def blend_kernel(self) -> str:
        k = C.c_int(0)
        _check(_lib().gsm_global_debug_blend_kernel(self._h, C.byref(k)), "gsm_global_debug_blend_kernel")
        return BLEND_KERNELS[k.value]

    def blend_kernel_kind(self) -> int:
        k = C.c_int(0)
        _check(_lib().gsm_global_debug_blend_kernel(self._h, C.byref(k)), "gsm_global_debug_blend_kernel")
        return k.value

    def copy_buffer(self, which: BufferId) -> np.ndarray:
        raw = self._debug_copy(which)
        if which == BufferId.RENDER_DATA:
            return raw.view(RENDER_DATA)
        if which == BufferId.BOUNDS:
            return raw.view(np.int32).reshape(-1, 4)
        if which in (BufferId.TILE_COUNTS, BufferId.KEYS, BufferId.SORTED_KEYS):
            return raw.view(np.uint32)
        if which in (BufferId.VALUES, BufferId.SORTED_VALUES):
            return raw.view(np.int32)
        if which == BufferId.HEADERS:
            return raw.view(np.uint32).reshape(-1, 2)
        if which == BufferId.BLEND_TRACE:
            return raw.view(np.uint64).reshape(-1, 4)
        if which == BufferId.EXP_TABLE:
            return raw.view(np.uint16)
        return raw


class DepthFirstBuffer(enum.IntEnum):
    RENDER_DATA = 0
    BOUNDS = 1
    TOUCHED = 2
    DEPTH_KEYS = 3
    DEPTH_ORDER = 4
    INSTANCE_TILES = 5
    INSTANCE_GAUSSIANS = 6
    HEADERS = 7
    BLEND_STATS = 8
    SORTED_DEPTH_KEYS = 9


DF_STAGES = ("project", "depth_sort", "instances", "tile_sort", "blend")

STEREO_RENDER_DATA = np.dtype([(f, "<u2") for f in (
    "leftMeanX", "leftMeanY", "leftCxx", "leftCyy", "leftCxy2", "leftDepth",
    "rightMeanX", "rightMeanY", "rightCxx", "rightCyy", "rightCxy2", "rightDepth")] +
    [("colorR", "u1"), ("colorG", "u1"), ("colorB", "u1"), ("opacity", "u1"),
     ("centerDepth", "<u2"), ("pad0", "<u2")])


class DepthFirstRenderer(_Renderer):
    _PREFIX, _STAGE_NAMES, _COUNTERS = "gsm_depthfirst", DF_STAGES, _DfCounters

    def __init__(self, device: Optional[int] = None, config: RendererConfig = RendererConfig(),
                 depth_key_bits: int = 32, tile_id_bits: int = 16):
        opt = _DfOptions(C.sizeof(_DfOptions), int(depth_key_bits), int(tile_id_bits), 0)
        self._open(device, config, "create_with_options", C.byref(opt))
        self._last_mono = False

    @property
    def options(self) -> dict:
        o = _DfOptions()
        _check(_lib().gsm_depthfirst_get_options(self._h, C.byref(o)), "gsm_depthfirst_get_options")
        return {"depth_key_bits": int(o.depth_key_bits), "tile_id_bits": int(o.tile_id_bits)}

    def render(self, color_texture, depth_texture, input: GaussianInput, camera: CameraParams,
               width: int, height: int, stream=None, color_pitch: Optional[int] = None,
               depth_pitch: Optional[int] = None):
        inp = _Input(_ptr(input.gaussians), _ptr(input.harmonics), int(input.gaussian_count),
                     int(input.sh_components))
        cam = _camera_struct(camera)
        cp = color_pitch if color_pitch is not None else int(width) * self._bpp
        dp = depth_pitch if depth_pitch is not None else int(width) * 2
        st = _lib().gsm_depthfirst_render(self._h, _stream_handle(stream), C.byref(inp), C.byref(cam),
                                          int(width), int(height), _ptr(color_texture), cp,
                                          _ptr(depth_texture), dp)
        _check(st, "gsm_depthfirst_render")
        self._last_mono = True

    def render_stereo_sbs(self, color_texture, input: GaussianInput, left: CameraParams, right: CameraParams,
                          width_per_eye: int, height: int, scene_transform=None, stream=None,
                          color_pitch: Optional[int] = None):
        inp = _Input(_ptr(input.gaussians), _ptr(input.harmonics), int(input.gaussian_count),
                     int(input.sh_components))
        cl, cr = _camera_struct(left), _camera_struct(right)
        st_arr = None
        if scene_transform is not None:
# ... 416 lines not shown
```

### include/gsm_debug.h

```cpp
#ifndef GSM_DEBUG_H
#define GSM_DEBUG_H

#include "gsm_renderer.h"

#ifdef __cplusplus
extern "C" {
#endif

typedef struct {
    uint32_t total_assignments;
    uint32_t max_capacity;
    uint32_t padded_count;
    uint32_t overflow;
    uint32_t tiles_x, tiles_y, tile_count;
    uint32_t gaussian_count;
} gsm_debug_counters;

typedef enum {
    GSM_BUF_RENDER_DATA = 0,
    GSM_BUF_BOUNDS = 1,
    GSM_BUF_TILE_COUNTS = 2,
    GSM_BUF_KEYS = 3,
    GSM_BUF_VALUES = 4,
    GSM_BUF_SORTED_KEYS = 5,
    GSM_BUF_SORTED_VALUES = 6,
    GSM_BUF_HEADERS = 7,
    GSM_BUF_EXP_TABLE = 8,
    GSM_BUF_BLEND_TRACE = 9
} gsm_buffer_id;

gsm_status gsm_global_debug_counters(gsm_renderer *renderer, gsm_debug_counters *out);

typedef enum {
    GSM_BLEND_KERNEL_NONE = 0,
    GSM_BLEND_KERNEL_QUADRANT = 1,
    GSM_BLEND_KERNEL_HALF_TILE = 2,
    GSM_BLEND_KERNEL_PAIR_WALK = 3
} gsm_blend_kernel;
gsm_status gsm_global_debug_blend_kernel(gsm_renderer *renderer, int *kind);
gsm_status gsm_global_debug_copy(gsm_renderer *renderer, int which, void *host_dst, size_t bytes,
                                 size_t *needed);
gsm_status gsm_global_set_profiling(gsm_renderer *renderer, int enable);

enum {
    GSM_STAGE_PROJECT = 0,
    GSM_STAGE_SCAN = 1,
    GSM_STAGE_SCATTER = 2,
    GSM_STAGE_SORT = 3,
    GSM_STAGE_HEADERS = 4,
    GSM_STAGE_BLEND = 5,
    GSM_STAGE_COUNT = 6
};
gsm_status gsm_global_stage_times(gsm_renderer *renderer, float *ms, int n);

gsm_status gsm_global_set_tile_rows(gsm_renderer *renderer, uint32_t row_begin, uint32_t row_end);

gsm_status gsm_sort_pairs_u32(void *keys, void *values, uint32_t n, uint32_t key_bits, void *stream);

gsm_status gsm_debug_sort_rank_probe(int hip_device, int *lane_ordered);

size_t gsm_debug_sort_workspace_bytes(uint32_t capacity);
gsm_status gsm_debug_sort_plan_fits(uint32_t capacity, uint32_t key_bits, int wide, size_t hist_bytes);

typedef struct gsm_debug_frame_sort gsm_debug_frame_sort;

typedef struct {
    uint32_t shift;
    uint32_t num_tiles;
    uint32_t all_tiles;
    uint32_t depth_sort;
    uint32_t full;
    uint32_t reserved;
} gsm_debug_frame_sort_desc;

typedef enum {
    GSM_FRAME_SORT_ONE_NARROW = 1,
    GSM_FRAME_SORT_TWO_NARROW = 2,
    GSM_FRAME_SORT_ONE_WIDE = 3,
    GSM_FRAME_SORT_WIDE_THEN_NARROW = 4
} gsm_frame_sort_plan;

typedef struct {
    uint32_t *sorted_keys;
    uint32_t *sorted_values;
    uint32_t *tile_start;
    uint32_t *half0, *half1;
    uint32_t *half_count;
    uint32_t plan;
    uint32_t reserved;
} gsm_debug_frame_sort_out;

gsm_status gsm_debug_frame_sort_create(uint32_t capacity, uint32_t max_tiles, int hip_device,
                                       gsm_debug_frame_sort **out);
void gsm_debug_frame_sort_destroy(gsm_debug_frame_sort *sorter);
gsm_status gsm_debug_frame_sort_run(gsm_debug_frame_sort *sorter, void *stream,
                                    const gsm_debug_frame_sort_desc *desc, const void *keys, const void *values,
                                    uint32_t n, gsm_debug_frame_sort_out *out);

gsm_status gsm_debug_partition_counts(gsm_renderer *renderer, void *stream, const gsm_gaussian_input *input,
                                      const gsm_camera_params *camera, uint32_t width, uint32_t height,
                                      uint32_t first, uint32_t count, const uint32_t *slab_rows,
                                      uint32_t num_slabs, uint32_t *d_send_counts);
gsm_status gsm_debug_partition_push(gsm_renderer *renderer, void *stream, uint32_t world, uint32_t rank,
                                    const uint32_t *d_counts, void *const *recv_buffers, uint32_t *d_recv_count);
gsm_status gsm_debug_render_records_device_count(gsm_renderer *renderer, void *stream, const void *records,
                                                 uint32_t capacity, const uint32_t *d_count, uint32_t width,
                                                 uint32_t height, void *color, size_t color_pitch, void *depth,
                                                 size_t depth_pitch);

#ifdef __cplusplus
}
#endif
#endif
```

Measured before the change: 4389.

## Fuse first radix sort pass into scatter via per-block digit histograms

Projection now also counts, per block, how many tile hits fall into each low-bit tile digit. A new bases kernel prefix-sums these counts into per-group scatter offsets, and a sorted scatter kernel writes keys directly in first-pass digit order using ballot or atomic ranking. The sort then starts at the second pass. This is meant to remove one full read-write pass over the key/value arrays and the separate scan launch, in exchange for extra LDS atomics in projection, a serial fixup kernel and more workspace memory.

```diff
diff --git a/gsm-renderer_amd/csrc/gsm_capi.hip b/gsm-renderer_amd/csrc/gsm_capi.hip
--- a/gsm-renderer_amd/csrc/gsm_capi.hip
+++ b/gsm-renderer_amd/csrc/gsm_capi.hip
@@ -464,6 +464,12 @@
     return GSM_OK;
 }
 
+gsm_status gsm_global_debug_scatter_sorted(gsm_renderer* r, int* taken) {
+    if (!r || !r->impl || !taken) return GSM_ERR_INVALID_ARGUMENT;
+    *taken = r->impl->lastScatterSorted() ? 1 : 0;
+    return GSM_OK;
+}
+
 gsm_status gsm_global_debug_copy(gsm_renderer* r, int which, void* dst, size_t bytes, size_t* needed) {
     if (!r || !r->impl) return GSM_ERR_INVALID_ARGUMENT;
     return r->impl->debugCopy(which, dst, bytes, needed);
diff --git a/gsm-renderer_amd/csrc/gsm_internal.h b/gsm-renderer_amd/csrc/gsm_internal.h
--- a/gsm-renderer_amd/csrc/gsm_internal.h
+++ b/gsm-renderer_amd/csrc/gsm_internal.h
@@ -21,6 +21,8 @@
     uint32_t schedUnits;
     uint32_t pairBucket;
     float limX, limY, focalX, focalY, maxEig, adjFar, adjDen;
+    uint32_t sortLowBits;
+    uint32_t* digitCounts;
 };
 
 struct ViewArgs {
@@ -266,6 +268,9 @@
     uint32_t* radixHist = nullptr;
     size_t radixHistBytes = 0;
     uint32_t* radixBinTotals = nullptr;
+    uint32_t* digitCounts = nullptr;
+    uint32_t* scatterBases = nullptr;
+    size_t digitCountWords = 0, scatterBaseWords = 0;
     uint32_t* tileStart = nullptr;
     uint32_t* tileQueue = nullptr;
     uint16_t* unitCost = nullptr;
@@ -298,6 +303,7 @@
     bool blendPairs = true;
     int pairBucket = 128;
     bool fusedScan = true;
+    bool scatterSorted = true;
 };
 constexpr uint32_t kFusedScanMaxBlocks = 8192;
 Tuning tuning_from_env(int device);
@@ -309,6 +315,10 @@
 
 constexpr uint32_t kSincosEntries = 65536;
 inline SortSpace sort_space(const DeviceArena& A) { return SortSpace{A.radixHist, A.radixHistBytes, A.radixBinTotals, kSortTotalsWords}; }
+inline bool sort_plan_fits(const SortPlan& plan, const DeviceArena& A) {
+    return sort_plan_fits(plan, A.radixHistBytes, kSortTotalsWords, A.radixHist != nullptr, A.radixBinTotals != nullptr,
+                          true, A.digitCounts ? A.digitCountWords : 0, A.scatterBases ? A.scatterBaseWords : 0);
+}
 
 void launch_project(bool halfInput, uint32_t shDegree, const FramePayload& payload, const void* world,
                     const void* harmonics, const ProjectArgs& args, const StyleArgs* style, bool ortho,
@@ -384,6 +394,8 @@
                       hipStream_t stream);
 void launch_scatter(const ProjectArgs& args, const DeviceArena& A, hipStream_t stream, const FramePayload& payload,
                     const uint32_t* devCount = nullptr, bool fusedScan = false);
+void launch_scatter_sorted(const ProjectArgs& args, const DeviceArena& A, const SortPlan& plan, uint32_t* superClear,
+                           bool ballot, hipStream_t stream);
 void launch_half_lists(const uint32_t* sortedVals, uint32_t tileBegin, uint32_t numTiles, const DeviceArena& A,
                        uint32_t tileCount, hipStream_t stream);
 void launch_headers(const uint32_t* sortedKeys, const FrameGeometry& geo, const DeviceArena& A,
@@ -452,6 +464,32 @@
     v += (uint32_t)__builtin_amdgcn_update_dpp(0, (int)v, 0x142, 0xA, 0xF, false);
     v += (uint32_t)__builtin_amdgcn_update_dpp(0, (int)v, 0x143, 0xC, 0xF, false);
     return v;
+}
+
+template <int BITS>
+__device__ __forceinline__ uint64_t match_digit(uint32_t d, bool valid) {
+    uint64_t peers = __ballot(valid);
+#pragma unroll
+    for (int bit = 0; bit < BITS; ++bit) {
+        const bool set = (d >> bit) & 1u;
+        const uint64_t m = __ballot(set);
+        peers &= set ? m : ~m;
+    }
+    return peers;
+}
+
+template <int BITS, bool BALLOT>
+__device__ __forceinline__ uint32_t wave_rank(uint32_t* cnt, uint32_t d, bool valid, uint64_t lt) {
+    if constexpr (BALLOT) {
+        const uint64_t peers = match_digit<BITS>(d, valid);
+        const uint32_t before = cnt[d];
+        if (valid && (peers & lt) == 0) cnt[d] = before + (uint32_t)__popcll(peers);
+        return before + (uint32_t)__popcll(peers & lt);
+    } else {
+        uint32_t r = 0;
+        if (valid) r = atomicAdd(&cnt[d], 1u);
+        return r;
+    }
 }
 
 struct Tail4 {
diff --git a/gsm-renderer_amd/csrc/gsm_kernels.hip b/gsm-renderer_amd/csrc/gsm_kernels.hip
--- a/gsm-renderer_amd/csrc/gsm_kernels.hip
+++ b/gsm-renderer_amd/csrc/gsm_kernels.hip
@@ -978,6 +978,7 @@
 #define GSM_VIEWS 3
 #include "gsm_scatter_body.h"
 #undef GSM_VIEWS
+#include "gsm_scatter_sorted.h"
 
 __global__ __launch_bounds__(256) void k_tile_starts(const uint32_t* __restrict__ sortedKeys,
                                                      const TileAssignmentHeader* __restrict__ hdr,
@@ -1295,6 +1296,21 @@
                        fusedScan ? 1u : 0u, A.header, A.tileQueue);
 }
 
+void launch_scatter_sorted(const ProjectArgs& a, const DeviceArena& A, const SortPlan& plan, uint32_t* superClear,
+                           bool ballot, hipStream_t s) {
+    const uint32_t blocks = (a.count + kProjectBlock - 1) / kProjectBlock;
+    const uint32_t lo = plan.scatterBits;
+    hipLaunchKernelGGL(k_scatter_bases, dim3(1u << lo), dim3(kProjectBlock), 0, s, A.digitCounts, blocks,
+                       plan.groupBlocks, plan.groups, lo, A.scatterBases, A.radixBinTotals + kSortFirstTotalsAt,
+                       A.blockSums, a.maxAssignments, A.header, A.tileQueue, superClear);
+    hipLaunchKernelGGL(ballot ? k_scatter_sorted<true> : k_scatter_sorted<false>, dim3(plan.groups),
+                       dim3(kProjectBlock), 0, s, a, A.renderData, A.bounds, A.tileCounts, A.tileMasks, A.blockSums,
+                       A.keys[0], A.vals[0], A.keys[1], A.vals[1], A.sincosTable, A.rec, A.header, A.scatterBases,
+                       A.radixBinTotals, plan.groupBlocks, plan.groups);
+    hipLaunchKernelGGL(k_first_pass_serial, dim3(1), dim3(kProjectBlock), 0, s, A.header, A.keys[0], A.vals[0],
+                       A.keys[1], A.vals[1], lo, a.maxAssignments, A.radixBinTotals);
+}
+
 void launch_headers(const uint32_t* sortedKeys, const FrameGeometry& g, const DeviceArena& A,
                     hipStream_t s) {
     const uint32_t t0 = 0, t1 = frame_tiles(g);
diff --git a/gsm-renderer_amd/csrc/gsm_project_body.h b/gsm-renderer_amd/csrc/gsm_project_body.h
--- a/gsm-renderer_amd/csrc/gsm_project_body.h
+++ b/gsm-renderer_amd/csrc/gsm_project_body.h
@@ -165,6 +165,10 @@
     constexpr uint32_t kCandCap = 4096, kCandRect = 64;
     constexpr uint16_t kSearch = 0xFFFFu;
     __shared__ uint16_t sCand[kCandCap];
+#if !GSM_VIEWS
+    __shared__ uint32_t sDig[1u << kScatterMaxBits];
+    const uint32_t digMask = (1u << P.sortLowBits) - 1u;
+#endif
     uint4 preW[2];
     preload_world<HALF>(world, gblk * kProjectBlock + threadIdx.x, P.count, preW);
 #ifdef GSM_STYLED
@@ -227,6 +231,9 @@
     sTy0[tid] = ty0;
     sMask[tid] = 0;
     sMore[tid] = 0;
+#if !GSM_VIEWS
+    if (P.sortLowBits && tid <= digMask) sDig[tid] = 0;
+#endif
     uint32_t total;
     const uint32_t coff = block_exclusive_scan<kProjectBlock>(area, lds, &total);
     sOff[tid] = coff;
@@ -266,6 +273,10 @@
         if (intersects_tile(tx, ty, e.x, e.y, kk, e2.y)) {
             if (k < (uint32_t)kMaskTiles) atomicOr(&sMask[lo], 1u << k);
             else atomicAdd(&sMore[lo], 1u);
+#if !GSM_VIEWS
+            if (P.sortLowBits)
+                atomicAdd(&sDig[((uint32_t)(ty - (int)P.rowBegin) * P.bin.tilesX + (uint32_t)tx) & digMask], 1u);
+#endif
         }
     }
     __syncthreads();
@@ -280,6 +291,9 @@
         rp[1] = make_uint4(o.rb, __float_as_uint(band.x), __float_as_uint(band.y), 0u);
     }
     if (gid < P.count) counts[oid] = ntiles;
+#if !GSM_VIEWS
+    if (P.sortLowBits && tid <= digMask) P.digitCounts[((size_t)blk << P.sortLowBits) + tid] = sDig[tid];
+#endif
     uint32_t s = block_reduce_add<kProjectBlock>(ntiles, lds);
     if (threadIdx.x == 0) blockSums[blk] = s;
 }
diff --git a/gsm-renderer_amd/csrc/gsm_renderer.hip b/gsm-renderer_amd/csrc/gsm_renderer.hip
--- a/gsm-renderer_amd/csrc/gsm_renderer.hip
+++ b/gsm-renderer_amd/csrc/gsm_renderer.hip
@@ -61,6 +61,16 @@
     M.alloc(st, A.radixHist, A.radixHistBytes);
     if (st == GSM_OK && hipMemset(A.radixHist, 0, A.radixHistBytes) != hipSuccess) st = GSM_ERR_FAILED_TO_ALLOCATE_BUFFER;
     M.alloc(st, A.radixBinTotals, kSortTotalsWords * sizeof(uint32_t));
+    if (r->tuning_.scatterSorted && nb > 0) {
+        const SortPlan sp = plan_sort_tiles_scattered(r->maxAssignments_, 16, r->tileCount_, r->tileCount_,
+                                                      r->tuning_.wideSort, r->tuning_.sortScanless, (uint32_t)nb);
+        if (sp.scatterBits) {
+            A.digitCountWords = sp.countWords;
+            A.scatterBaseWords = (size_t)kScatterMaxGroups << sp.scatterBits;
+            M.alloc(st, A.digitCounts, A.digitCountWords * sizeof(uint32_t));
+            M.alloc(st, A.scatterBases, A.scatterBaseWords * sizeof(uint32_t));
+        }
+    }
     M.alloc(st, A.tileStart, ((size_t)r->tileCount_ + 1) * sizeof(uint32_t));
     M.alloc(st, A.tileQueue, kQueueStripes * kQueueStride * sizeof(uint32_t));
     M.alloc(st, A.unitCost, (size_t)r->tileCount_ * 4 * sizeof(uint16_t));
@@ -945,6 +955,17 @@
     const bool costOrder = rq.preOrdered ? tuning_.costOrder : units > 0;
     fa.schedUnits = units;
     fa.pairBucket = tuning_.blendPairs ? (uint32_t)std::max(1, tuning_.pairBucket) : kUoBuckets;
+    SortPlan scattered;
+    if (tuning_.scatterSorted && !tuning_.fullRadix && rq.payload.kind == FrameKind::Single && !rq.devCount &&
+        !capture && !tileRowsRestricted() && nb > 0) {
+        const SortPlan sp = plan_sort_tiles_scattered(maxAssignments_, 16, rowCount() * tilesX_, tileCount_,
+                                                      tuning_.wideSort, tuning_.sortScanless, nb);
+        if (sp.scatterBits && sort_plan_fits(sp, arena_)) scattered = sp;
+    }
+    const bool scatterSorted = scattered.scatterBits != 0;
+    lastScatterSorted_ = scatterSorted;
+    fa.sortLowBits = scattered.scatterBits;
+    fa.digitCounts = scatterSorted ? arena_.digitCounts : nullptr;
 
     timer_.beginFrame();
     timer_.record(0, s);
@@ -955,9 +976,15 @@
                        rq.style.table ? &rq.style : nullptr, rq.orthographic, arena_, s);
     timer_.record(1, s);
     const bool fusedScan = tuning_.fusedScan && nb > 0 && nb <= (rq.devCount ? 4u : 1u) * kFusedScanMaxBlocks;
-    if (!fusedScan) launch_scan_blocks(nb, a, arena_, s, rq.devCount);
+    if (!scatterSorted && !fusedScan) launch_scan_blocks(nb, a, arena_, s, rq.devCount);
     timer_.record(2, s);
-    launch_scatter(a, arena_, s, rq.payload, rq.devCount, fusedScan);
+    if (scatterSorted) {
+        const int set = scattered.pass[0].superSet;
+        launch_scatter_sorted(fa, arena_, scattered, set >= 0 ? arena_.radixHist + (size_t)set * kSuperSetWords : nullptr,
+                              tuning_.ballotRank, s);
+    } else {
+        launch_scatter(a, arena_, s, rq.payload, rq.devCount, fusedScan);
+    }
     if (keep) {
         hipMemcpyAsync(arena_.keysKeep, arena_.keys[0], (size_t)maxAssignments_ * 4, hipMemcpyDeviceToDevice, s);
         hipMemcpyAsync(arena_.valsKeep, arena_.vals[0], (size_t)maxAssignments_ * 4, hipMemcpyDeviceToDevice, s);
@@ -1002,9 +1029,12 @@
     const bool ballot = tuning_.ballotRank;
     if (!fullRadix) {
         const uint32_t localTiles = frame_tiles(g);
-        const int res = radix_sort_tiles(kb, vb, &arena_.header->totalAssignments, maxAssignments_, 16,
-                                         sort_space(arena_), arena_.tileStart, 0u, localTiles,
-                                         tileCount_, s, ballot, tuning_.wideSort, tuning_.sortScanless);
+        const int res = scatterSorted
+                            ? run_sort_plan(scattered, kb, vb, &arena_.header->totalAssignments, sort_space(arena_),
+                                            arena_.tileStart, nullptr, s, ballot)
+                            : radix_sort_tiles(kb, vb, &arena_.header->totalAssignments, maxAssignments_, 16,
+                                               sort_space(arena_), arena_.tileStart, 0u, localTiles, tileCount_, s,
+                                               ballot, tuning_.wideSort, tuning_.sortScanless);
         if (res == kSortNoSpace) return GSM_ERR_INVALID_ASSIGNMENT_CAPACITY;
         tile_depth_sort(kb[res], vb[res], kb[res ^ 1], vb[res ^ 1], arena_.tileStart, 0u, localTiles, s, ballot,
                         arena_.halfVals[0], arena_.halfVals[1],
@@ -1094,6 +1124,9 @@
             break;
         case GSM_BUF_HEADERS: full = (size_t)tileCount_ * 8; break;
         case GSM_BUF_EXP_TABLE: src = arena_.expTable; full = 65536 * 2; break;
+        case GSM_BUF_HALF_LIST_0: src = arena_.halfVals[0]; full = tot * 4; break;
+        case GSM_BUF_HALF_LIST_1: src = arena_.halfVals[1]; full = tot * 4; break;
+        case GSM_BUF_HALF_COUNTS: src = arena_.halfCount; full = (size_t)tileCount_ * 2 * 4; break;
         case GSM_BUF_BLEND_TRACE: src = (timer_.flags() & 4) ? traceBuf_ : nullptr; full = (size_t)tileCount_ * 4 * 4 * 8; break;
         default: return GSM_ERR_INVALID_ARGUMENT;
     }
diff --git a/gsm-renderer_amd/csrc/gsm_renderer_impl.h b/gsm-renderer_amd/csrc/gsm_renderer_impl.h
--- a/gsm-renderer_amd/csrc/gsm_renderer_impl.h
+++ b/gsm-renderer_amd/csrc/gsm_renderer_impl.h
@@ -82,6 +82,7 @@
 
     gsm_status counters(gsm_debug_counters* out);
     int lastBlendKernel() const { return lastBlendKernel_; }
+    bool lastScatterSorted() const { return lastScatterSorted_; }
     gsm_status debugCopy(int which, void* dst, size_t bytes, size_t* needed);
     gsm_status setProfiling(int flags);
     gsm_status stageTimes(float* ms, int n) {
@@ -176,6 +177,7 @@
     DeviceArena arena_;
     DeviceAllocations allocs_;
     StageTimer timer_{GSM_STAGE_COUNT, 128};
+    bool lastScatterSorted_ = false;
     int lastBlendKernel_ = 0;
     bool keptRenderData_ = false;
     uint32_t lastCount_ = 0, lastWidth_ = 0, lastHeight_ = 0;
diff --git a/gsm-renderer_amd/csrc/gsm_scatter_sorted.h b/gsm-renderer_amd/csrc/gsm_scatter_sorted.h
--- /dev/null
+++ b/gsm-renderer_amd/csrc/gsm_scatter_sorted.h
@@ -0,0 +1,314 @@
+constexpr uint32_t kScatterDigits = 1u << kScatterMaxBits;
+constexpr uint32_t kScatterWindow = 4096;
+static_assert(kProjectBlock == 256 && kScatterDigits <= kProjectBlock, "one thread per digit, 4 waves");
+
+__device__ __forceinline__ void scatter_wave_sync() {
+    __builtin_amdgcn_fence(__ATOMIC_RELEASE, "wavefront");
+    __builtin_amdgcn_wave_barrier();
+    __builtin_amdgcn_fence(__ATOMIC_ACQUIRE, "wavefront");
+}
+
+__device__ __forceinline__ uint32_t scatter_block_scan(uint32_t x, uint32_t* part) {
+    const uint32_t lane = threadIdx.x & 63u, wave = threadIdx.x >> 6;
+    const uint32_t inc = wave_scan_incl(x);
+    __syncthreads();
+    if (lane == 63) part[wave] = inc;
+    __syncthreads();
+    uint32_t off = 0;
+#pragma unroll
+    for (uint32_t w = 0; w < 4; ++w)
+        if (w < wave) off += part[w];
+    return off + inc - x;
+}
+
+__global__ __launch_bounds__(kProjectBlock) void k_scatter_bases(
+    const uint32_t* __restrict__ digitCounts, uint32_t blocks, uint32_t groupBlocks, uint32_t groups, uint32_t lo,
+    uint32_t* __restrict__ bases, uint32_t* __restrict__ firstTotals, const uint32_t* __restrict__ blockSums,
+    uint32_t maxAssignments, TileAssignmentHeader* __restrict__ hdr, uint32_t* __restrict__ blendQueue,
+    uint32_t* __restrict__ superClear) {
+    __shared__ uint32_t part[4];
+    __shared__ unsigned long long lds64[kProjectBlock / 64];
+    const uint32_t d = blockIdx.x, tid = threadIdx.x;
+    if (superClear)
+        for (uint32_t i = blockIdx.x * kProjectBlock + tid; i < (uint32_t)kSuperSetWords; i += gridDim.x * kProjectBlock)
+            superClear[i] = 0u;
+    uint32_t v[4];
+#pragma unroll
+    for (uint32_t i = 0; i < 4; ++i) {
+        const uint32_t g = tid * 4u + i;
+        uint32_t sum = 0;
+        if (g < groups) {
+            const uint32_t b0 = g * groupBlocks, b1 = min(b0 + groupBlocks, blocks);
+            for (uint32_t b = b0; b < b1; ++b) sum += digitCounts[((size_t)b << lo) + d];
+        }
+        v[i] = sum;
+    }
+    const uint32_t local = v[0] + v[1] + v[2] + v[3];
+    uint32_t run = scatter_block_scan(local, part);
+#pragma unroll
+    for (uint32_t i = 0; i < 4; ++i) {
+        const uint32_t g = tid * 4u + i;
+        if (g < groups) bases[(size_t)d * groups + g] = run;
+        run += v[i];
+    }
+    if (tid == kProjectBlock - 1) firstTotals[d] = run;
+    if (blockIdx.x == 0) {
+        const uint64_t all = block_sum_prefix(blockSums, blocks, lds64);
+        if (tid == 0) {
+            uint32_t tot = all > 0xFFFFFFFFull ? 0xFFFFFFFFu : (uint32_t)all;
+            uint32_t ovf = 0;
+            if (tot > maxAssignments) {
+                tot = maxAssignments;
+                ovf = 1;
+            }
+            hdr->totalAssignments = tot;
+            hdr->maxCapacity = maxAssignments;
+            hdr->paddedCount = ((tot + 1023u) / 1024u) * 1024u;
+            hdr->overflow = ovf;
+            for (uint32_t q = 0; q < kQueueStripes; ++q) blendQueue[q * kQueueStride] = 0;
+        }
+    }
+}
+
+template <bool BALLOT>
+__global__ __launch_bounds__(kProjectBlock) void k_scatter_sorted(
+    ProjectArgs P, const GaussianRenderData* __restrict__ rd, const short4* __restrict__ bounds,
+    const uint32_t* __restrict__ counts, const uint32_t* __restrict__ masks, const uint32_t* __restrict__ blockSums,
+    uint32_t* __restrict__ keys0, uint32_t* __restrict__ vals0, uint32_t* __restrict__ keys1,
+    uint32_t* __restrict__ vals1, const float2* __restrict__ sincos, const BlendRecord* __restrict__ rec,
+    const TileAssignmentHeader* __restrict__ hdr, const uint32_t* __restrict__ bases, uint32_t* __restrict__ binTotals,
+    uint32_t groupBlocks, uint32_t groups) {
+    constexpr uint32_t C = kScatterWindow, D = kScatterDigits, kItems = C / kProjectBlock;
+    __shared__ uint32_t sK[C];
+    __shared__ uint32_t sV[C];
+    __shared__ uint32_t binBase[D];
+    __shared__ uint32_t waveCnt[4][D];
+    __shared__ uint32_t localStart[D];
+    __shared__ uint32_t chunkTotal[D];
+    __shared__ uint32_t lds[kProjectBlock / 64];
+    __shared__ unsigned long long lds64[kProjectBlock / 64];
+    __shared__ uint32_t part[4];
+    const uint32_t tid = threadIdx.x, lane = tid & 63u, wave = tid >> 6;
+    const uint32_t g = blockIdx.x, lo = P.sortLowBits, R = 1u << lo;
+    const uint32_t blocks = (P.count + kProjectBlock - 1u) / kProjectBlock;
+    const bool ovf = hdr->overflow != 0u;
+    uint64_t origin = 0;
+    if (ovf) origin = g ? block_sum_prefix(blockSums, g * groupBlocks, lds64) : 0ull;
+    {
+        const uint32_t t = tid < R ? binTotals[kSortFirstTotalsAt + tid] : 0u;
+        const uint32_t start = scatter_block_scan(t, part);
+        if (tid < D) {
+            binBase[tid] = tid < R ? start + bases[(size_t)tid * groups + g] : 0u;
+#pragma unroll
+            for (uint32_t w = 0; w < 4; ++w) waveCnt[w][tid] = 0;
+        }
+        if (g == 0 && !ovf && tid < R) binTotals[kSortBucketsAt + tid] = start;
+    }
+    __syncthreads();
+
+    const uint64_t lt = (lane == 0) ? 0ull : (~0ull >> (64 - lane));
+    auto flush = [&](uint32_t winBase, uint32_t cn) {
+        if (ovf) {
+            for (uint32_t p = tid; p < cn; p += kProjectBlock) {
+                const uint64_t wp = origin + winBase + p;
+                if (wp < P.maxAssignments) {
+                    keys0[wp] = sK[p];
+                    vals0[wp] = sV[p];
+                }
+            }
+            __syncthreads();
+            return;
+        }
+        uint32_t k[kItems], v[kItems], rank[kItems];
+#pragma unroll
+        for (uint32_t j = 0; j < kItems; ++j) {
+            const uint32_t idx = wave * (64u * kItems) + j * 64u + lane;
+            const bool valid = idx < cn;
+            k[j] = valid ? sK[idx] : 0u;
+            v[j] = valid ? sV[idx] : 0u;
+        }
+#pragma unroll
+        for (uint32_t j = 0; j < kItems; ++j) {
+            const uint32_t idx = wave * (64u * kItems) + j * 64u + lane;
+            rank[j] = wave_rank<(int)kScatterMaxBits, BALLOT>(waveCnt[wave], (k[j] >> 16) & (R - 1u), idx < cn, lt);
+            if constexpr (BALLOT) scatter_wave_sync();
+        }
+        __syncthreads();
+        uint32_t tot = 0;
+        if (tid < D) {
+#pragma unroll
+            for (uint32_t w = 0; w < 4; ++w) {
+                const uint32_t c = waveCnt[w][tid];
+                waveCnt[w][tid] = tot;
+                tot += c;
+            }
+            chunkTotal[tid] = tot;
+        }
+        const uint32_t ls = scatter_block_scan(tot, part);
+        if (tid < D) localStart[tid] = ls;
+        __syncthreads();
+#pragma unroll
+        for (uint32_t j = 0; j < kItems; ++j) {
+            const uint32_t idx = wave * (64u * kItems) + j * 64u + lane;
+            if (idx < cn) {
+                const uint32_t d = (k[j] >> 16) & (R - 1u);
+                const uint32_t pos = localStart[d] + waveCnt[wave][d] + rank[j];
+                sK[pos] = k[j];
+                sV[pos] = v[j];
+            }
+        }
+        __syncthreads();
+        for (uint32_t p = tid; p < cn; p += kProjectBlock) {
+            const uint32_t key = sK[p];
+            const uint32_t d = (key >> 16) & (R - 1u);
+            const uint32_t dst = binBase[d] + (p - localStart[d]);
+            if (dst < P.maxAssignments) {
+                keys1[dst] = key;
+                vals1[dst] = sV[p];
+            }
+        }
+        __syncthreads();
+        if (tid < D) {
+            binBase[tid] += chunkTotal[tid];
+#pragma unroll
+            for (uint32_t w = 0; w < 4; ++w) waveCnt[w][tid] = 0;
+        }
+        __syncthreads();
+    };
+
+    typedef unsigned u32x4 __attribute__((ext_vector_type(4)));
+    const RowSet RS = rows_of(P);
+    uint32_t winBase = 0;
+    uint32_t pos = 0;
+    const uint32_t b0 = g * groupBlocks, b1 = min(b0 + groupBlocks, blocks);
+    for (uint32_t blk = b0; blk < b1; ++blk) {
+        const uint32_t gid = blk * kProjectBlock + tid;
+        uint32_t c = 0u, mw = 0u;
+        unsigned long long rb = 0ull;
+        u32x4 r1v = {0u, 0u, 0u, 0u};
+        if (gid < P.count) {
+            c = __builtin_nontemporal_load(counts + gid);
+            rb = __builtin_nontemporal_load((const unsigned long long*)(bounds + gid));
+            r1v = __builtin_nontemporal_load((const u32x4*)(rec + gid) + 1);
+            mw = __builtin_nontemporal_load(masks + gid);
+        }
+        uint32_t total;
+        const uint32_t off = block_exclusive_scan<kProjectBlock>(c, lds, &total);
+        bool large = false;
+        short4 r = make_short4(0, -1, 0, -1);
+        uint32_t dbits = 0, rw = 1, inv = 0;
+        int ty0 = 0, ty1 = -1;
+        float2 band = make_float2(0.0f, -1.0f);
+        if (c != 0) {
+            r = __builtin_bit_cast(short4, rb);
+            band = make_float2(__uint_as_float(r1v.y), __uint_as_float(r1v.z));
+            dbits = ((r1v.x >> 16) ^ 0x8000u) & 0xFFFFu;
+            rows_within(RS, (int)r.z, (int)r.w, &ty0, &ty1);
+            rw = (uint32_t)((int)r.y - (int)r.x + 1);
+            large = (ty1 - ty0 + 1) * (int)rw > kMaskTiles;
+            inv = (uint32_t)__builtin_ceilf(65536.0f * __builtin_amdgcn_rcpf((float)rw));
+        }
+        const uint32_t blockEnd = pos + total;
+        const uint32_t my0 = pos + off;
+        uint4 rdw = make_uint4(0u, 0u, 0u, 0u);
+        if (large) rdw = *(const uint4*)(rd + gid);
+        if (ovf && origin + winBase >= P.maxAssignments) break;
+        for (;;) {
+            const uint32_t winEnd = winBase + C;
+            if (c != 0 && my0 < winEnd && my0 + c > winBase) {
+                if (!large) {
+                    uint32_t m = mw;
+                    for (uint32_t sp = my0; m != 0 && sp < winEnd; ++sp, m &= m - 1u) {
+                        if (sp < winBase) continue;
+                        const uint32_t bit = (uint32_t)__builtin_ctz(m);
+                        const uint32_t row = (bit * inv) >> 16;
+                        const int kr = ty0 + (int)row, tx = (int)r.x + (int)(bit - row * rw);
+                        sK[sp - winBase] = ((uint32_t)(kr * (int)P.bin.tilesX + tx) << 16) | dbits;
+                        sV[sp - winBase] = gid | (half_skip_flags(band.x, band.y, tx) << kHalfSkipShift);
+                    }
+                } else {
+                    const uint16_t hmx = (uint16_t)(rdw.x & 0xFFFFu), hmy = (uint16_t)(rdw.x >> 16);
+                    const uint16_t thq = (uint16_t)(rdw.y & 0xFFFFu), hs1 = (uint16_t)(rdw.y >> 16);
+                    const uint16_t hs2 = (uint16_t)(rdw.z & 0xFFFFu);
+                    const uint32_t opac = rdw.w >> 24;
+                    const float cx = hbits_to_f(hmx), cy = hbits_to_f(hmy);
+                    const Conic kq = conic_from_quant(sincos, thq, hbits_to_f(hs1), hbits_to_f(hs2));
+                    const float w = 2.0f * compute_power((float)opac);
+                    uint32_t sp = my0;
+                    for (int kr = ty0; kr <= ty1 && sp < winEnd; ++kr)
+                        for (int tx = (int)r.x, ty = RS.b + kr * RS.s; tx <= (int)r.y && sp < winEnd; ++tx)
+                            if (intersects_tile(tx, ty, cx, cy, kq, w)) {
+                                if (sp >= winBase && sp < my0 + c) {
+                                    sK[sp - winBase] = ((uint32_t)(kr * (int)P.bin.tilesX + tx) << 16) | dbits;
+                                    sV[sp - winBase] = gid | (half_skip_flags(band.x, band.y, tx) << kHalfSkipShift);
+                                }
+                                sp++;
+                            }
+                }
+            }
+            if (blockEnd <= winEnd) break;
+            __syncthreads();
+            flush(winBase, C);
+            winBase += C;
+            if (ovf && origin + winBase >= P.maxAssignments) break;
+        }
+        pos = blockEnd;
+    }
+    __syncthreads();
+    if (pos > winBase) flush(winBase, pos - winBase);
+}
+
+__global__ __launch_bounds__(kProjectBlock) void k_first_pass_serial(
+    const TileAssignmentHeader* __restrict__ hdr, const uint32_t* __restrict__ keys0,
+    const uint32_t* __restrict__ vals0, uint32_t* __restrict__ keys1, uint32_t* __restrict__ vals1, uint32_t lo,
+    uint32_t capacity, uint32_t* __restrict__ binTotals) {
+    constexpr uint32_t D = kScatterDigits;
+    if (hdr->overflow == 0u) return;
+    __shared__ uint32_t cnt[D];
+    __shared__ uint32_t carry[D];
+    __shared__ uint32_t wcnt[4][D];
+    __shared__ uint32_t part[4];
+    const uint32_t tid = threadIdx.x, lane = tid & 63u, wave = tid >> 6;
+    const uint32_t R = 1u << lo, n = min(hdr->totalAssignments, capacity);
+    const uint64_t lt = (lane == 0) ? 0ull : (~0ull >> (64 - lane));
+    if (tid < D) cnt[tid] = 0;
+    __syncthreads();
+    for (uint32_t i = tid; i < n; i += kProjectBlock) atomicAdd(&cnt[(keys0[i] >> 16) & (R - 1u)], 1u);
+    __syncthreads();
+    {
+        const uint32_t t = tid < D ? cnt[tid] : 0u;
+        const uint32_t start = scatter_block_scan(t, part);
+        if (tid < D) carry[tid] = start;
+        if (tid < R) {
+            binTotals[kSortFirstTotalsAt + tid] = t;
+            binTotals[kSortBucketsAt + tid] = start;
+        }
+    }
+    __syncthreads();
+    for (uint32_t b = 0; b < n; b += kProjectBlock) {
+        const uint32_t i = b + tid;
+        const bool valid = i < n;
+        const uint32_t k = valid ? keys0[i] : 0u, v = valid ? vals0[i] : 0u;
+        const uint32_t d = (k >> 16) & (R - 1u);
+        if (tid < D) {
+#pragma unroll
+            for (uint32_t w = 0; w < 4; ++w) wcnt[w][tid] = 0;
+        }
+        __syncthreads();
+        const uint64_t peers = match_digit<(int)kScatterMaxBits>(d, valid);
+        if (valid && (peers & lt) == 0) wcnt[wave][d] = (uint32_t)__popcll(peers);
+        __syncthreads();
+        if (valid) {
+            uint32_t before = carry[d];
+            for (uint32_t w = 0; w < wave; ++w) before += wcnt[w][d];
+            const uint32_t p = before + (uint32_t)__popcll(peers & lt);
+            if (p < capacity) {
+                keys1[p] = k;
+                vals1[p] = v;
+            }
+        }
+        __syncthreads();
+        if (tid < D) carry[tid] += wcnt[0][tid] + wcnt[1][tid] + wcnt[2][tid] + wcnt[3][tid];
+        __syncthreads();
+    }
+}
diff --git a/gsm-renderer_amd/csrc/gsm_sort.hip b/gsm-renderer_amd/csrc/gsm_sort.hip
--- a/gsm-renderer_amd/csrc/gsm_sort.hip
+++ b/gsm-renderer_amd/csrc/gsm_sort.hip
@@ -25,31 +25,6 @@
     *end = (uint32_t)ee;
 }
 
-template <int BITS>
-__device__ __forceinline__ uint64_t match_digit(uint32_t d, bool valid) {
-    uint64_t peers = __ballot(valid);
-#pragma unroll
-    for (int bit = 0; bit < BITS; ++bit) {
-        const bool set = (d >> bit) & 1u;
-        const uint64_t m = __ballot(set);
-        peers &= set ? m : ~m;
-    }
-    return peers;
-}
-
-template <int BITS, bool BALLOT>
-__device__ __forceinline__ uint32_t wave_rank(uint32_t* cnt, uint32_t d, bool valid, uint64_t lt) {
-    if constexpr (BALLOT) {
-        const uint64_t peers = match_digit<BITS>(d, valid);
-        const uint32_t before = cnt[d];
-        if (valid && (peers & lt) == 0) cnt[d] = before + (uint32_t)__popcll(peers);
-        return before + (uint32_t)__popcll(peers & lt);
-    } else {
-        uint32_t r = 0;
-        if (valid) r = atomicAdd(&cnt[d], 1u);
-        return r;
-    }
-}
 
 static_assert(kRadixBlock == 256 && kRadixBlock / 64 == 4, "the scanless base reduction assumes 4 waves");
 
@@ -636,9 +611,11 @@
 
 int run_sort_plan(const SortPlan& plan, uint32_t* keys[2], uint32_t* vals[2], const uint32_t* nPtr, const SortSpace& ws,
                   uint32_t* tileStart, uint32_t* buckets, hipStream_t s, bool ballot) {
-    if (!sort_plan_fits(plan, ws, buckets != nullptr)) return kSortNoSpace;
+    SortPlan passes = plan;
+    passes.countWords = passes.baseWords = 0;
+    if (!sort_plan_fits(passes, ws, buckets != nullptr)) return kSortNoSpace;
     uint32_t* const hist = ws.hist + kSuperWords;
-    for (uint32_t i = 0, cur = 0; i < plan.count; ++i, cur ^= 1u) {
+    for (uint32_t i = 0, cur = plan.start; i < plan.count; ++i, cur ^= 1u) {
         const SortPass& p = plan.pass[i];
         uint32_t *kin = keys[cur], *vin = vals[cur], *kout = keys[cur ^ 1u], *vout = vals[cur ^ 1u];
         uint32_t* binTotals = ws.binTotals + p.totalsAt;
@@ -1053,6 +1030,8 @@
     if (ps) t.pairBucket = std::min(256, std::max(0, atoi(ps)));
     const char* fs = getenv("GSM_SCAN_FUSED");
     t.fusedScan = !(fs && fs[0] == '0');
+    const char* ss = getenv("GSM_SCATTER_SORTED");
+    t.scatterSorted = !(ss && ss[0] == '0');
     return t;
 }
 
diff --git a/gsm-renderer_amd/csrc/gsm_sort_plan.h b/gsm-renderer_amd/csrc/gsm_sort_plan.h
--- a/gsm-renderer_amd/csrc/gsm_sort_plan.h
+++ b/gsm-renderer_amd/csrc/gsm_sort_plan.h
@@ -22,6 +22,15 @@
 constexpr uint32_t kSortFirstTotalsAt = 256, kSortBucketsAt = 512, kSortTwoNarrowWords = 768;
 constexpr uint32_t kTilesWideMaxBits = kWideMaxBits + 8u;
 constexpr int kSortNoSpace = -1;
+constexpr uint32_t kScatterMaxBits = 7, kScatterMaxGroups = 1024, kScatterMinGroupBlocks = 4;
+inline uint32_t scatter_group_blocks(uint32_t blocks) {
+    const uint32_t g = (blocks + kScatterMaxGroups - 1) / kScatterMaxGroups;
+    return g < kScatterMinGroupBlocks ? kScatterMinGroupBlocks : g;
+}
+inline uint32_t scatter_groups(uint32_t blocks) {
+    const uint32_t g = scatter_group_blocks(blocks);
+    return (blocks + g - 1) / g;
+}
 
 inline uint32_t radix_grid_for_capacity(uint32_t capacity) {
     uint32_t g = (capacity + kRadixChunk - 1) / kRadixChunk;
@@ -73,13 +82,15 @@
     int result = 0;
     uint32_t kind = 0;
     bool valid = true;
+    uint32_t start = 0, scatterBits = 0, groupBlocks = 0, groups = 0;
+    size_t countWords = 0, baseWords = 0;
     void add(const SortPass& p) {
         if (count == 4) {
             valid = false;
             return;
         }
         pass[count++] = p;
-        result = (int)(count & 1u);
+        result = (int)((start + count) & 1u);
     }
 };
 
@@ -155,6 +166,22 @@
     return plan;
 }
 
+inline SortPlan plan_sort_tiles_scattered(uint32_t capacity, uint32_t shift, uint32_t numTiles, uint32_t allTiles,
+                                          bool wide, bool scanless, uint32_t blocks) {
+    const SortPlan two = plan_sort_tiles(capacity, shift, 0u, numTiles, allTiles, wide, scanless);
+    if (two.kind != GSM_FRAME_SORT_TWO_NARROW || two.pass[0].bits > kScatterMaxBits || blocks == 0) return two;
+    SortPlan plan;
+    plan.kind = two.kind;
+    plan.start = 1;
+    plan.scatterBits = two.pass[0].bits;
+    plan.groupBlocks = scatter_group_blocks(blocks);
+    plan.groups = scatter_groups(blocks);
+    plan.countWords = (size_t)blocks << plan.scatterBits;
+    plan.baseWords = (size_t)plan.groups << plan.scatterBits;
+    plan.add(two.pass[1]);
+    return plan;
+}
+
 inline SortPlan plan_sort_tiles_wide(uint32_t capacity, uint32_t allTiles) {
     const uint32_t bits = sort_bits_for(allTiles, 17, 32);
     SortPlan plan;
@@ -171,8 +198,9 @@
 }
 
 inline bool sort_plan_fits(const SortPlan& plan, size_t histBytes, size_t binWords, bool haveHist, bool haveBins,
-                           bool haveBuckets = true) {
+                           bool haveBuckets = true, size_t countWords = 0, size_t baseWords = 0) {
     if (!plan.valid) return false;
+    if (plan.countWords > countWords || plan.baseWords > baseWords || plan.groups > kScatterMaxGroups) return false;
     for (uint32_t i = 0; i < plan.count; ++i) {
         const SortPass& p = plan.pass[i];
         if (!haveHist || !haveBins || (sort_uses_buckets(p.starts) && !haveBuckets)) return false;
diff --git a/gsm-renderer_amd/gsm_amd/__init__.py b/gsm-renderer_amd/gsm_amd/__init__.py
--- a/gsm-renderer_amd/gsm_amd/__init__.py
+++ b/gsm-renderer_amd/gsm_amd/__init__.py
@@ -81,6 +81,9 @@
     HEADERS = 7
     EXP_TABLE = 8
     BLEND_TRACE = 9
+    HALF_LIST_0 = 10
+    HALF_LIST_1 = 11
+    HALF_COUNTS = 12
 
 
 STAGES = ("project", "scan", "scatter", "sort", "headers", "blend")
@@ -397,6 +400,7 @@
     "gsm_global_last_gpu_time": ([C.c_void_p, C.POINTER(C.c_double)], C.c_int),
     "gsm_global_debug_counters": ([C.c_void_p, C.POINTER(_Counters)], C.c_int),
     "gsm_global_debug_blend_kernel": ([C.c_void_p, C.POINTER(C.c_int)], C.c_int),
+    "gsm_global_debug_scatter_sorted": ([C.c_void_p, C.POINTER(C.c_int)], C.c_int),
     "gsm_debug_sort_workspace_bytes": ([C.c_uint32], C.c_size_t),
     "gsm_debug_sort_plan_fits": ([C.c_uint32, C.c_uint32, C.c_int, C.c_size_t], C.c_int),
     "gsm_global_debug_copy": ([C.c_void_p, C.c_int, C.c_void_p, C.c_size_t, C.POINTER(C.c_size_t)],
@@ -1014,6 +1018,11 @@
         _check(_lib().gsm_global_debug_blend_kernel(self._h, C.byref(k)), "gsm_global_debug_blend_kernel")
         return BLEND_KERNELS[k.value]
 
+    def scatter_sorted(self) -> bool:
+        k = C.c_int(0)
+        _check(_lib().gsm_global_debug_scatter_sorted(self._h, C.byref(k)), "gsm_global_debug_scatter_sorted")
+        return bool(k.value)
+
     def blend_kernel_kind(self) -> int:
         k = C.c_int(0)
         _check(_lib().gsm_global_debug_blend_kernel(self._h, C.byref(k)), "gsm_global_debug_blend_kernel")
diff --git a/include/gsm_debug.h b/include/gsm_debug.h
--- a/include/gsm_debug.h
+++ b/include/gsm_debug.h
@@ -26,7 +26,10 @@
     GSM_BUF_SORTED_VALUES = 6,
     GSM_BUF_HEADERS = 7,
     GSM_BUF_EXP_TABLE = 8,
-    GSM_BUF_BLEND_TRACE = 9
+    GSM_BUF_BLEND_TRACE = 9,
+    GSM_BUF_HALF_LIST_0 = 10,
+    GSM_BUF_HALF_LIST_1 = 11,
+    GSM_BUF_HALF_COUNTS = 12
 } gsm_buffer_id;
 
 gsm_status gsm_global_debug_counters(gsm_renderer *renderer, gsm_debug_counters *out);
@@ -38,6 +41,7 @@
     GSM_BLEND_KERNEL_PAIR_WALK = 3
 } gsm_blend_kernel;
 gsm_status gsm_global_debug_blend_kernel(gsm_renderer *renderer, int *kind);
+gsm_status gsm_global_debug_scatter_sorted(gsm_renderer *renderer, int *taken);
 gsm_status gsm_global_debug_copy(gsm_renderer *renderer, int which, void *host_dst, size_t bytes,
                                  size_t *needed);
 gsm_status gsm_global_set_profiling(gsm_renderer *renderer, int enable);
```

After: 4310. 0.982x the previous value.
